# joyecnu/STTODE

Measured on AMD Instinct MI355X. Metric: predicted-trajectories/sec (20-sample best-of-K), higher is better.
Workload: dtype f32

## Files before the change

### include/sttode_hip.h

```cpp
#ifndef STTODE_HIP_H
#define STTODE_HIP_H
#ifdef __cplusplus
extern "C" {
#endif

#define STTODE_ABI_VERSION 15
int sttode_abi_version(void);
const char* sttode_last_error(void);

int sttode_rotate_scene(float* past, float* fut, int n, int Tp, int Tf, float c, float s, void* stream);

int sttode_frontend_scenes(const float* past, const int* scene_ptr, int n, int S, int Tp, int TPX, int vel_from_norm,
                           float* scene_orig, int* agent_scene, float* xpad, float* enc_in, float* cur, float* orig,
                           int* last_flag, void* stream);

int sttode_frontend_nba(const float* past, int n, int N, int Tp, int TPX, float* xpad, float* enc_in, float* cur, float* orig,
                        int* last_flag, void* stream);

int sttode_frontend_future(const float* future, const float* past_last, int n, int Tf, int mode, int nba_N,
                           const float* scene_orig, const int* agent_scene, const int* scene_ptr, float* enc_in, void* stream);

int sttode_embed_qkv(const float* fc1P, const float* fc1b, const float* posP, const float* peb, const float* fc2P,
                     const float* fc2b, const float* fc3P, const float* fc3b, const float* fc3last, const float* inP,
                     const float* inb, const float* enc_in, const int* last_flag, float* g, float* qkv, int n, int Tlen,
// ... 260 lines not shown
                             double* gc_ws, float* gc, void* stream);
int sttode_pmath_matvec_bwd_c(const float* m, const float* x, const float* g, float* mx_ws, float* gmx_ws, float* gxn_ws, float* gx, float* gm,
                              int rows, int d, int O, const float* c_dev, double* gc_ws, float* gc, void* stream);
int sttode_pmath_dist_matrix_bwd_c(const float* x, const float* y, const float* g, float* gx, float* gy, int P, int R, int d,
                                   const float* c_dev, double* gc_ws, float* gc, void* stream);
int sttode_pmath_hsoftmax_bwd_c(const float* X, const float* A, const float* P, const float* g, double* coef_ws, float* gX, float* gA,
                                float* gP, int B, int C, int d, const float* c_dev, double* gc_ws, float* gc, void* stream);
int sttode_oblique_dist(const float* p1, const float* p2, float* out, int nb, int n1, int n2, int d, void* stream);
int sttode_pmath_mean_seg(const float* x, float* yl_ws, float* lam_ws, float* out, float* klein, float* lsum, int outer, int R, int inner,
                          int d, float c, const float* c_dev, void* stream);
int sttode_pmath_mean_bwd(const float* x, const float* g, double* gS_ws, double* gL_ws, float* gx, int outer, int R, int inner, int d, float c,
                          void* stream);
int sttode_pmath_mean_bwd_c(const float* x, const float* g, double* gS_ws, double* gL_ws, float* gx, int outer, int R, int inner, int d,
                            const float* c_dev, double* gc_ws, float* gc, void* stream);
int sttode_oblique_proj_bwd(const float* p, const float* g, float* gp, int rows, int d, void* stream);
int sttode_oblique_dist_bwd(const float* p1, const float* p2, const float* g, float* gp1, float* gp2, int nb, int n1, int n2, int d,
                            void* stream);

enum SttodeManifold { STT_MF_EUCLIDEAN = 0, STT_MF_OBLIQUE, STT_MF_POINCARE, STT_MF_COUNT };
enum SttodeManifoldOp { STT_MOP_PROJ_TAN = 0, STT_MOP_EXPMAP, STT_MOP_PTRANSP, STT_MOP_INNER, STT_MOP_RETR, STT_MOP_RETR_TRANSP, STT_MOP_COUNT };
enum SttodeRiemannianRule { STT_RULE_ADAM = 0, STT_RULE_SGD, STT_RULE_COUNT };
int sttode_manifold_rowop(int op, int manifold, const float* a, const float* b, const float* w, float* out, float* out2, int rows, int d,
                          float c, void* stream);
int sttode_manifold_rowop_bwd(int op, int manifold, const float* a, const float* b, const float* w, const float* g, const float* g2, float* ga,
                              float* gb, float* gw, int rows, int d, float c, void* stream);
#define STTODE_RIEMANNIAN_ITEM_WORDS 10
int sttode_riemannian_step(int rule, const void* table, int nrows_table, long total_slots, double lr, double beta1, double beta2,
                           double eps, double weight_decay, double momentum, long t, void* tstate, void* stream);

int sttode_delta_dist(const float* X, int rows, int d, const int* idx, int T, int n, float* dist, long dist_floats, float* diam, void* stream);
int sttode_delta_workspace(int T, int n, long* floats);
int sttode_delta_hyp(const float* dist, int T, int n, long dist_floats, int symmetric, float* ws, long ws_floats, float* delta, void* stream);

int sttode_reduce_samples(const float* pred, int n, int R, int K_in, int Tf, int K, int iters, int from_frame, int init_mode,
                          const float* init, float* centroids, int* labels, int* counts, void* stream);

int sttode_reduce_scenes(const float* pred, int n, int R, int K_in, int Tf, int K, int iters, int from_frame, int init_mode,
                         const float* init, const int* seg_ptr, int S, float* centroids, int* labels, int* counts, void* stream);
long long int sttode_large_select_ws(int n, int M);
int sttode_large_select(const float* pred, const float* gt, int n, int R, int K_in, int Tf, float scale, float miss_threshold, const int* ks,
                        int nk, const int* seg_ptr, int S, void* ws, long ws_bytes, float* ade, float* fde, int* best_ade_idx,
                        int* best_fde_idx, unsigned char* miss, float* ade_at, float* fde_at, float* seg_jade, float* seg_jfde,
                        int* seg_jade_idx, int* seg_jfde_idx, void* stream);
int sttode_large_kde_nll(const float* pred, const float* gt, int n, int R, int K_in, int Tf, float scale, double* nll, void* stream);
long long int sttode_large_spread_ws(int n, int M);
int sttode_large_spread(const float* pred, const float* gt, int n, int R, int K_in, int Tf, float scale, double div_scale, void* ws,
                        long ws_bytes, double* apd, double* fpd, double* pade, double* dlow, double* es_ade, double* es_fde, void* stream);

typedef struct SttodeModel SttodeModel;

enum SttodeWeight {
    STT_W_FC1P, STT_W_FC1B, STT_W_POSP, STT_W_PEB, STT_W_FC2P, STT_W_FC2B, STT_W_FC3P, STT_W_FC3B, STT_W_FC3LAST, STT_W_INP,
    STT_W_INB, STT_W_OUTP, STT_W_OUTB, STT_W_INFOP, STT_W_INFOB, STT_W_GATEP, STT_W_GATEB, STT_W_LN1W, STT_W_LN1B, STT_W_L1P,
    STT_W_L1B, STT_W_L2P, STT_W_L2B, STT_W_LN2W, STT_W_LN2B,
    STT_W_B0_CONVP, STT_W_B0_CONVB, STT_W_B0_WIHP, STT_W_B0_WHHP, STT_W_B0_GBIAS, STT_W_B0_XWA, STT_W_B0_XB1, STT_W_B0_YWA,
    STT_W_B0_YB1, STT_W_B0_STREAM,
    STT_W_B1_CONVP, STT_W_B1_CONVB, STT_W_B1_WIHP, STT_W_B1_WHHP, STT_W_B1_GBIAS, STT_W_B1_YWA, STT_W_B1_YB1, STT_W_B1_STREAM,
    STT_W_CHAIN_POOL, STT_W_CHAIN_PROG, STT_W_CHAIN_CONSTS, STT_W_G0_POOL, STT_W_G0_PROG, STT_W_G0_CONSTS,
    STT_W_CHAINB3_POOL, STT_W_CHAINB3_PROG,
    STT_W_ROLE32_POOL, STT_W_ROLE32_PROG_SCENES, STT_W_ROLE32_PROG_NBA, STT_W_ROLE32_CONSTS_SCENES,
    STT_W_ROLE32_CONSTS_NBA,
    STT_W_COUNT
};

enum SttodeBuffer {
    STT_B_SCENE_ORIG, STT_B_AGENT_SCENE, STT_B_XPAD, STT_B_ENC_IN, STT_B_CUR, STT_B_ORIG, STT_B_LAST, STT_B_G, STT_B_QKV,
    STT_B_ATTN, STT_B_PF, STT_B_STATE0, STT_B_A0X, STT_B_A0Y, STT_B_A1Y, STT_B_DBUF, STT_B_YBUF, STT_B_STATE1, STT_B_QUEUE, STT_B_FLAGS ,
    STT_B_ODE , STT_B_COUNT
};

enum SttodeStage {
    STT_STAGE_FRONTEND, STT_STAGE_EMBED, STT_STAGE_ATTN, STT_STAGE_POST, STT_STAGE_GRU0, STT_STAGE_LINEAR, STT_STAGE_MLP0,
    STT_STAGE_GRU1, STT_STAGE_MLP1, STT_STAGE_CHAIN, STT_STAGE_AGENTS ,
    STT_STAGE_FUSED , STT_STAGE_COUNT
};

int sttode_model_create(SttodeModel** out, const void* const* weights, int count, int Tp, int Tf, int K, int n_chunks0,
                        int n_chunks1);
int sttode_model_set_weight(SttodeModel* m, int index, const void* ptr);
int sttode_model_destroy(SttodeModel* m);
int sttode_workspace_layout(const SttodeModel* m, int n, int S, long* offsets , long* total_floats);
int sttode_workspace_init(SttodeModel* m, float* workspace, int n, int S, void* stream);
int sttode_set_chain(SttodeModel* m, int mode);
int sttode_set_fused(SttodeModel* m, int mode);
int sttode_set_mfma_mode(SttodeModel* m, int mode);
int sttode_debug_drop_role_flag(SttodeModel* m, int tile);
int sttode_stage_scene(const float* pre, const float* fut, int N, int Tp, int Tf, float* dev, void* stream);
int sttode_stage_rows(const float* a, long na, const float* b, long nb, float* dev, void* stream);
int sttode_async_next_stream(SttodeModel* m, int n, void** stream);
int sttode_async_best_of_k(SttodeModel* m, int slot, const float* pred, const float* gt, int n, int K, int Tf, float scale, float* ade,
                           float* fde);
int sttode_set_scene_launch(SttodeModel* m, int max_tiles);
int sttode_set_ode(SttodeModel* m, int method, int steps);
int sttode_timing_enable(SttodeModel* m, int every);
int sttode_timing_read(SttodeModel* m, double* total_ms , int* launches ,
                       double* busy_ms );

int sttode_inference_scenes(SttodeModel* m, const float* past, const int* scene_ptr, int n, int S, const float* z,
                            float* workspace, float* pred, void* stream);
int sttode_inference_nba(SttodeModel* m, const float* past, int B, int N, const float* z, float* workspace, float* pred,
                         void* stream);
int sttode_inference_nba_groups(SttodeModel* m, const float* past, int G, int B, int N, const float* z, float* workspace, float* pred,
                                void* stream);

int sttode_set_lagged(SttodeModel* m, int streams );
typedef struct SttodeSamplerPlan {
    const float* pool;
    const int* prog;
    int prog_len;
    const float* biases;
    int K;
    int nz;
    int h1;
    int h2;
    int eps_mode;
    const float* eps;
} SttodeSamplerPlan;
typedef struct SttodeAsyncOpts {
    int device_latents;
    unsigned long long zkey;
    const float* metrics_gt;
    float* ade;
    float* fde;
    float metrics_scale;
    int nba_groups;
    const SttodeSamplerPlan* sampler;
} SttodeAsyncOpts;
int sttode_sampler_qnet(const SttodeSamplerPlan* plan, const float* pf, int n, float* z, void* stream);
int sttode_clock_probe(long long* out, void* stream);
int sttode_copy_to_host(void* dst, const void* src, long bytes, int wgs, void* stream);
int sttode_async_enqueue(SttodeModel* m, int slot);
int sttode_async_flush(SttodeModel* m);
int sttode_inference_scenes_async(SttodeModel* m, const float* past, const int* scene_ptr, int n, int S, const float* z,
                                  float* workspace, float* pred, int slot, const SttodeAsyncOpts* opts, void* stream);
int sttode_inference_nba_async(SttodeModel* m, const float* past, int B, int N, const float* z, float* workspace, float* pred,
                               int slot, const SttodeAsyncOpts* opts, void* stream);
int sttode_async_horizon_metrics(SttodeModel* m, int slot, const float* pred, const float* gt, int n, int K, int Tf, float scale, float* out);
int sttode_async_best_of_k_select(SttodeModel* m, int slot, const float* pred, const float* gt, int n, int K, int Tf, float scale,
                                  float miss_threshold, const int* seg_ptr, int S, float* ade, float* fde, int* best_ade_idx, int* best_fde_idx,
                                  unsigned char* miss, float* best, float* seg_ade, float* seg_fde, int* seg_miss);
int sttode_async_joint_select(SttodeModel* m, int slot, const float* pred, const float* gt, int n, int K, int Tf, float scale,
                              const int* seg_ptr, int S, float radius, float* seg_jade, float* seg_jfde, int* seg_jade_idx, int* seg_jfde_idx,
                              int* seg_col, int* seg_gt_col);
int sttode_async_kde_nll(SttodeModel* m, int slot, const float* pred, const float* gt, int n, int K, int Tf, float scale, double* nll);
int sttode_async_sample_spread(SttodeModel* m, int slot, const float* pred, const float* gt, int n, int K, int Tf, float scale,
                               double div_scale, double* apd, double* fpd, double* pade, double* dlow, double* es_ade, double* es_fde,
                               float* ade_at_k, float* fde_at_k);
int sttode_wait(SttodeModel* m, int slot, void* stream);
int sttode_async_is_lagged(SttodeModel* m, int n);
int sttode_wait_host(SttodeModel* m, int slot);
int sttode_timeout_word(SttodeModel* m, const unsigned** word);
int sttode_timeout_clear(SttodeModel* m);
int sttode_check(SttodeModel* m, const float* workspace, int n, int S, void* stream);

#ifdef __cplusplus
}
#endif
#endif
```

### sttode_amd/capi.py

```python
import ctypes
import os

_LIB = None
LIB_PATH = os.environ.get('STTODE_HIP_LIB') or os.path.join(os.path.dirname(os.path.abspath(__file__)), 'lib', 'libsttode_hip.so')

_P, _I, _L, _F, _D = ctypes.c_void_p, ctypes.c_int, ctypes.c_long, ctypes.c_float, ctypes.c_double
ABI_VERSION = 15

SIGNATURES = {
    'sttode_abi_version': [],
    'sttode_rotate_scene': [_P, _P, _I, _I, _I, _F, _F, _P],
    'sttode_frontend_scenes': [_P, _P, _I, _I, _I, _I, _I, _P, _P, _P, _P, _P, _P, _P, _P],
    'sttode_frontend_nba': [_P, _I, _I, _I, _I, _P, _P, _P, _P, _P, _P],
    'sttode_frontend_future': [_P, _P, _I, _I, _I, _I, _P, _P, _P, _P, _P],
    'sttode_embed_qkv': [_P] * 11 + [_P, _P, _P, _P, _I, _I, _P],
    'sttode_mhgsa_attn': [_P, _P, _P, _P, _P, _P, _I, _I, _I] + [_L] * 8 + [_F, _F, _P],
    'sttode_mhgsa_attn_groups': [_P, _P, _P, _P, _I, _L, _L, _L, _L, _I, _I, _I] + [_L] * 8 + [_F, _F, _I, _P],
    'sttode_post_attn': [_P] * 14 + [_P, _P, _I, _P, _I, _F, _P],
    'sttode_post_attn_ode': [_P] * 16 + [_P, _P, _I, _F, _I, _I, _P],
    'sttode_post_attn_rhs': [_P] * 14 + [_P, _P, _I, _P, _I, _P],
    'sttode_ode_state_to_pf': [_P, _P, _P, _I, _P],
    'sttode_gru_cols': [_P, _P, _P, _P, _P, _P, _P, _I, _I, _I, _P],
    'sttode_set_latency_tiles': [_I, _I, _I],
    'sttode_linear_cols': [_P, _I, _I, _P, _I, _I, _P, _P, _P, _I, _I, _I, _I, _P],
# ... 22 lines not shown
    'sttode_sampler_objective_joint': [_P] * 8 + [_I, _I, _I, _I, _I, _F, _P, _L] + [_P] * 6,
    'sttode_sampler_objective_joint_bwd': [_P] * 8 + [_I] + [_P] * 4 + [_I, _I, _I, _I, _F, _P, _L] + [_P] * 4,
    'sttode_tlinear': [_P, _L, _I, _P, _L, _I, _P, _P, _L, _P, _L, _I, _I, _I, _I, _I, _P],
    'sttode_tlinear_tab': [_P, _L, _P, _L, _P, _P, _L, _I, _P, _L, _I, _I, _I, _I, _P],
    'sttode_twgrad': [_P, _L, _P, _L, _I, _P, _L, _P, _I, _I, _I, _P, _L, _P],
    'sttode_twgrad_defer': [_I, _P, _L],
    'sttode_twgrad_flush': [],
    'sttode_tgemm_group': [_I],
    'sttode_tlinear_bwd': [_P, _L, _P, _L, _P, _L, _P, _L, _I, _I, _P, _L, _I, _P, _L, _P, _I, _I, _I, _P, _L, _P],
    'sttode_decoder_inputs': [_P, _P, _L, _P, _L, _P, _P, _I, _I, _I, _I, _P],
    'sttode_rows_copy': [_P, _L, _P, _L, _I, _I, _I, _I, _P],
    'sttode_rows_reduce': [_P, _L, _P, _L, _I, _I, _I, _I, _P],
    'sttode_train_ewise': [_I, _P, _P, _P, _P, _P, _L, _I, _F, _P],
    'sttode_add_ln_fwd': [_P, _P, _P, _P, _P, _P, _P, _I, _I, _P],
    'sttode_ln_bwd': [_P, _P, _P, _P, _P, _P, _P, _I, _I, _P, _L, _P],
    'sttode_gru_cell_fwd': [_P, _L, _P, _P, _P, _P, _I, _P],
    'sttode_gru_cell_bwd': [_P, _P, _P, _P, _L, _P, _P, _I, _P],
    'sttode_gru_seq_fwd': [_P, _P, _P, _P, _P, _P, _L, _I, _I, _P],
    'sttode_gru_seq_bwd': [_P, _L, _P, _P, _P, _P, _P, _I, _I, _P],
    'sttode_conv_fwd': [_P, _I, _P, _P, _P, _P, _P, _I, _I, _P],
    'sttode_conv_bwd': [_P, _P, _P, _P, _P, _P, _I, _I, _P, _L, _P],
    'sttode_mhgsa_attn_bwd': [_P, _P, _P, _I, _I, _I, _P],
    'sttode_mhgsa_attn_rc_bwd': [_P] * 7 + [_I, _I, _I] + [_L] * 8 + [_F, _F, _P],
    'sttode_adam_step': [_P, _I, _L, _P, _D, _D, _D, _D, _D, _L, _P],
    'sttode_grad_norm': [_P, _I, _P, _L, _D, _I, _P, _P],
    'sttode_adam_step_guarded': [_P, _I, _L, _P, _D, _D, _D, _D, _P, _I, _P],
    'sttode_grad_scale': [_P, _I, _L, _P, _P, _P],
    'sttode_loss_sqerr': [_P, _P, _L, _F, _P, _P, _P],
    'sttode_loss_kl': [_P, _P, _I, _I, _I, _F, _F, _P, _P, _P, _P],
    'sttode_loss_diverse': [_P, _P, _P, _P, _I, _I, _I, _P, _P, _P, _P],
    'sttode_ttrunk_fwd': [_P, _I, _I, _I, _L, _F, _I, _P],
    'sttode_ode_combine': [_P, _I, _I, _P],
    'sttode_ttrunk_ode_fwd': [_P, _I, _I, _P, _P, _P, _P, _P, _P, _P],
    'sttode_ode_stage_bwd': [_P, _I, _P],
    'sttode_loss_objective': [_P, _P, _P, _P, _P, _P, _P, _I, _I, _I, _I, _I, _I, _F, _F, _F, _F, _P, _P, _P, _P, _P, _L, _P],
    'sttode_pmath_rowop': [_I, _P, _P, _P, _P, _I, _I, _F, _P],
    'sttode_pmath_scalar': [_I, _P, _P, _L, _P],
    'sttode_pmath_riemannian_grad': [_P, _P, _P, _I, _I, _F, _P],
    'sttode_pmath_matvec': [_P, _P, _P, _P, _P, _I, _I, _I, _F, _P],
    'sttode_pmath_pair': [_I, _P, _P, _P, _P, _I, _I, _I, _F, _P],
    'sttode_pmath_mean': [_P, _P, _P, _P, _I, _I, _F, _P],
    'sttode_oblique_dist': [_P, _P, _P, _I, _I, _I, _I, _P],
    'sttode_pmath_rowop_bwd': [_I, _P, _P, _P, _P, _P, _I, _I, _F, _P],
    'sttode_pmath_matvec_bwd': [_P, _P, _P, _P, _P, _P, _P, _P, _I, _I, _I, _F, _P],
    'sttode_pmath_dist_matrix_bwd': [_P, _P, _P, _P, _P, _I, _I, _I, _F, _P],
    'sttode_pmath_hsoftmax_bwd': [_P, _P, _P, _P, _P, _P, _P, _P, _I, _I, _I, _F, _P],
    'sttode_pmath_clip': [_P, _P, _I, _I, _F, _P],
    'sttode_pmath_clip_bwd': [_P, _P, _P, _I, _I, _F, _P],
    'sttode_pmath_rowop_c': [_I, _P, _P, _P, _P, _I, _I, _P, _P],
    'sttode_pmath_matvec_c': [_P, _P, _P, _P, _P, _I, _I, _I, _P, _P],
    'sttode_pmath_pair_c': [_I, _P, _P, _P, _P, _I, _I, _I, _P, _P],
    'sttode_pmath_rowop_bwd_c': [_I, _P, _P, _P, _P, _P, _I, _I, _P, _P, _P, _P],
    'sttode_pmath_matvec_bwd_c': [_P, _P, _P, _P, _P, _P, _P, _P, _I, _I, _I, _P, _P, _P, _P],
    'sttode_pmath_dist_matrix_bwd_c': [_P, _P, _P, _P, _P, _I, _I, _I, _P, _P, _P, _P],
    'sttode_pmath_hsoftmax_bwd_c': [_P, _P, _P, _P, _P, _P, _P, _P, _I, _I, _I, _P, _P, _P, _P],
    'sttode_manifold_rowop': [_I, _I, _P, _P, _P, _P, _P, _I, _I, _F, _P],
    'sttode_riemannian_step': [_I, _P, _I, _L, _D, _D, _D, _D, _D, _D, _L, _P, _P],
    'sttode_pmath_mean_seg': [_P, _P, _P, _P, _P, _P, _I, _I, _I, _I, _F, _P, _P],
    'sttode_pmath_mean_bwd': [_P, _P, _P, _P, _P, _I, _I, _I, _I, _F, _P],
    'sttode_pmath_mean_bwd_c': [_P, _P, _P, _P, _P, _I, _I, _I, _I, _P, _P, _P, _P],
    'sttode_oblique_proj_bwd': [_P, _P, _P, _I, _I, _P],
    'sttode_oblique_dist_bwd': [_P, _P, _P, _P, _P, _I, _I, _I, _I, _P],
    'sttode_manifold_rowop_bwd': [_I, _I, _P, _P, _P, _P, _P, _P, _P, _P, _I, _I, _F, _P],
    'sttode_delta_dist': [_P, _I, _I, _P, _I, _I, _P, _L, _P, _P],
    'sttode_delta_workspace': [_I, _I, ctypes.POINTER(ctypes.c_long)],
    'sttode_delta_hyp': [_P, _I, _I, _L, _I, _P, _L, _P, _P],
    'sttode_reduce_samples': [_P, _I, _I, _I, _I, _I, _I, _I, _I, _P, _P, _P, _P, _P],
    'sttode_reduce_scenes': [_P, _I, _I, _I, _I, _I, _I, _I, _I, _P, _P, _I, _P, _P, _P, _P],
    'sttode_large_select_ws': [_I, _I],
    'sttode_large_select': [_P, _P, _I, _I, _I, _I, _F, _F, _P, _I, _P, _I, _P, _L] + [_P] * 12,
    'sttode_large_kde_nll': [_P, _P, _I, _I, _I, _I, _F, _P, _P],
    'sttode_large_spread_ws': [_I, _I],
    'sttode_large_spread': [_P, _P, _I, _I, _I, _I, _F, _D, _P, _L] + [_P] * 7,
    'sttode_attn_core': [_P, _P, _P, _P, _L, _P, _P, _P, _P, _I, _I, _I] + [_L] * 8 + [_F, _F, _I, _P],
    'sttode_attn_core_bwd': [_P, _P, _P, _P, _L, _P, _P, _P, _P, _I, _I, _I] + [_L] * 8 + [_F, _F, _I, _P],
    'sttode_model_create': [ctypes.POINTER(ctypes.c_void_p), ctypes.POINTER(ctypes.c_void_p), _I, _I, _I, _I, _I, _I],
    'sttode_model_destroy': [_P],
    'sttode_model_set_weight': [_P, _I, _P],
    'sttode_workspace_layout': [_P, _I, _I, ctypes.POINTER(ctypes.c_long), ctypes.POINTER(ctypes.c_long)],
    'sttode_workspace_init': [_P, _P, _I, _I, _P],
    'sttode_timeout_word': [_P, ctypes.POINTER(ctypes.c_void_p)],
    'sttode_timeout_clear': [_P],
    'sttode_set_chain': [_P, _I],
    'sttode_set_fused': [_P, _I],
    'sttode_set_mfma_mode': [_P, _I],
    'sttode_debug_drop_role_flag': [_P, _I],
    'sttode_set_scene_launch': [_P, _I],
    'sttode_stage_scene': [_P, _P, _I, _I, _I, _P, _P],
    'sttode_stage_rows': [_P, _L, _P, _L, _P, _P],
    'sttode_loss_objective_live': [_P, _P, _P, _P, _P, _P, _P, _I, _I, _I, _I, _I, _I, _F, _F, _F, _F, _P, _P, _P, _P, _P, _P, _L, _P],
    'sttode_loss_objective_joint': [_P, _P, _P, _P, _P, _P, _P, _I, _I, _I, _I, _I, _I, _F, _F, _F, _F, _P, _P, _P, _P, _P, _I, _P, _P, _L, _P],
    'sttode_loss_diverse_joint': [_P, _P, _P, _P, _I, _I, _I, _I, _P, _P, _P, _P, _P],
    'sttode_live_rows_gather': [_P, _I, _P, _I, _I, _P],
    'sttode_publish_values': [_P, _I, _P, _P, _P, _P],
    'sttode_wait_value': [_P, _L, _D],
    'sttode_async_next_stream': [_P, _I, _P],
    'sttode_async_best_of_k': [_P, _I, _P, _P, _I, _I, _I, _F, _P, _P],
    'sttode_set_ode': [_P, _I, _I],
    'sttode_timing_enable': [_P, _I],
    'sttode_timing_read': [_P, ctypes.POINTER(ctypes.c_double), ctypes.POINTER(ctypes.c_int), ctypes.POINTER(ctypes.c_double)],
    'sttode_inference_scenes': [_P, _P, _P, _I, _I, _P, _P, _P, _P],
    'sttode_inference_nba': [_P, _P, _I, _I, _P, _P, _P, _P],
    'sttode_inference_nba_groups': [_P, _P, _I, _I, _I, _P, _P, _P, _P],
    'sttode_inference_scenes_async': [_P, _P, _P, _I, _I, _P, _P, _P, _I, _P, _P],
    'sttode_inference_nba_async': [_P, _P, _I, _I, _P, _P, _P, _I, _P, _P],
    'sttode_async_horizon_metrics': [_P, _I, _P, _P, _I, _I, _I, _F, _P],
    'sttode_async_best_of_k_select': [_P, _I, _P, _P, _I, _I, _I, _F, _F, _P, _I] + [_P] * 9,
    'sttode_async_joint_select': [_P, _I, _P, _P, _I, _I, _I, _F, _P, _I, _F] + [_P] * 6,
    'sttode_async_kde_nll': [_P, _I, _P, _P, _I, _I, _I, _F, _P],
    'sttode_async_sample_spread': [_P, _I, _P, _P, _I, _I, _I, _F, _D] + [_P] * 8,
    'sttode_wait': [_P, _I, _P],
    'sttode_async_is_lagged': [_P, _I],
    'sttode_wait_host': [_P, _I],
    'sttode_set_lagged': [_P, _I],
    'sttode_async_flush': [_P],
    'sttode_clock_probe': [_P, _P],
    'sttode_copy_to_host': [_P, _P, _L, _I, _P],
    'sttode_async_enqueue': [_P, _I],
    'sttode_check': [_P, _P, _I, _I, _P],
}

RESTYPES = {'sttode_sampler_objective_joint_ws': ctypes.c_longlong, 'sttode_large_select_ws': ctypes.c_longlong,
            'sttode_large_spread_ws': ctypes.c_longlong}

WEIGHT_ORDER = ([('past', k) for k in ('fc1P', 'fc1b', 'posP', 'peb', 'fc2P', 'fc2b', 'fc3P', 'fc3b', 'fc3last', 'inP', 'inb', 'outP',
                                       'outb', 'infoP', 'infob', 'gateP', 'gateb', 'ln1w', 'ln1b', 'l1P', 'l1b', 'l2P', 'l2b', 'ln2w',
                                       'ln2b')]
                + [('blk0', k) for k in ('convP', 'convB', 'wihP', 'whhP', 'gbias', 'x_WA', 'x_b1', 'y_WA', 'y_b1', 'stream')]
                + [('blk1', k) for k in ('convP', 'convB', 'wihP', 'whhP', 'gbias', 'y_WA', 'y_b1', 'stream')]
                + [('chain', k) for k in ('pool', 'prog', 'consts')] + [('gru0s', k) for k in ('pool', 'prog', 'consts')]
                + [('chain_b3', k) for k in ('pool', 'prog')]
                + [('role32', k) for k in ('pool', 'prog_scenes', 'prog_nba', 'consts_scenes', 'consts_nba')])
TRUNK_PTRS = ('fc1_w', 'fc1_b', 'pos_w', 'pos_b', 'fc2_w', 'fc2_b', 'fc3_w', 'fc3_b', 'inproj_w', 'inproj_b', 'out_w', 'out_b', 'info_w', 'info_b',
              'gate_w', 'gate_b', 'ln1_w', 'ln1_b', 'l1_w', 'l1_b', 'l2_w', 'l2_b', 'ln2_w', 'ln2_b', 'enc_in', 'last', 'pe', 'drop', 'posin', 'tp',
              'h3in', 'feat', 'xc', 'qkv', 'ao', 'tt', 'ss', 'h', 'xh1', 'rs1', 'f1', 'xh2', 'rs2', 'ode', 'attn')
BUFFERS = ('scene_orig', 'agent_scene', 'xpad', 'enc_in', 'cur', 'orig', 'last', 'g', 'qkv', 'attn', 'pf', 'state0', 'A0x', 'A0y',
           'A1y', 'dbuf', 'ybuf', 'state1', 'queue', 'flags', 'ode')
STAGES = ('frontend', 'embed_qkv', 'mhgsa_attn', 'post_attn', 'gru_cols[block0,agents]', 'agent_preact', 'mlp_block0',
          'gru_cols[block1,trajectories]', 'mlp_block1', 'trajectory_chain', 'agents_fused[encoder+block0 GRU]', 'agents+trajectory_chain[fused launch]')


class AsyncOpts(ctypes.Structure):
    _fields_ = [('device_latents', ctypes.c_int), ('zkey', ctypes.c_ulonglong), ('metrics_gt', ctypes.c_void_p), ('ade', ctypes.c_void_p),
                ('fde', ctypes.c_void_p), ('metrics_scale', ctypes.c_float), ('nba_groups', ctypes.c_int), ('sampler', ctypes.c_void_p)]


class GradGroup(ctypes.Structure):
    _fields_ = [('items', ctypes.c_void_p), ('n', ctypes.c_int), ('chunks', ctypes.c_long), ('gbase', ctypes.c_void_p),
                ('lr', ctypes.c_double), ('beta1', ctypes.c_double), ('beta2', ctypes.c_double), ('step', ctypes.c_long)]


GRAD_MAX_GROUPS = 16
GRAD_STATE_WORDS = 40


MANIFOLDS = dict(euclidean=0, oblique=1, poincare=2)
MANIFOLD_OPS = dict(proj_tan=0, expmap=1, ptransp=2, inner=3, retr=4, retr_transp=5)
RIEMANNIAN_RULES = dict(adam=0, sgd=1)
RIEMANNIAN_ITEM_WORDS = 10


class SamplerPlan(ctypes.Structure):
    _fields_ = [('pool', ctypes.c_void_p), ('prog', ctypes.c_void_p), ('prog_len', ctypes.c_int), ('biases', ctypes.c_void_p),
                ('K', ctypes.c_int), ('nz', ctypes.c_int), ('h1', ctypes.c_int), ('h2', ctypes.c_int), ('eps_mode', ctypes.c_int),
                ('eps', ctypes.c_void_p)]


class NativeModel:

    def __init__(self, packed, Tp, Tf, K):
        self.packed = packed
        tbl = (ctypes.c_void_p * len(WEIGHT_ORDER))(*[(packed[g][k].data_ptr() if g in packed else None) for g, k in WEIGHT_ORDER])
        h = ctypes.c_void_p()
        rc = lib().sttode_model_create(ctypes.byref(h), tbl, len(WEIGHT_ORDER), Tp, Tf, K, int(packed['blk0']['n_chunks']),
                                       int(packed['blk1']['n_chunks']))
        if rc != 0:
            raise SttodeError('sttode_model_create failed: ' + lib().sttode_last_error().decode())
        self.h = h
        self._layouts = {}
        w = ctypes.c_void_p()
        if lib().sttode_timeout_word(h, ctypes.byref(w)) != 0 or not w.value:
            raise SttodeError('sttode_timeout_word failed: ' + lib().sttode_last_error().decode())
        self.timeout_word = ctypes.c_uint.from_address(w.value)

    def raise_if_timed_out(self):
        v = self.timeout_word.value
        if v:
            lib().sttode_timeout_clear(self.h)
            raise SttodeError('a trajectory group of an earlier launch gave up waiting for its per-agent role (time-out word %d): the '
                              'predictions of that call are NaN-poisoned, not valid' % v if v != 2 else
                              'an earlier launch ran on a workspace that was never initialised (sttode_workspace_init): its predictions are NaN')

    def init_workspace(self, buf, n, S):
        call('sttode_workspace_init', self.h, buf, int(n), int(S), stream_ptr())

    def layout(self, n, S):
        key = (n, S)
        if key not in self._layouts:
            off = (ctypes.c_long * len(BUFFERS))()
            tot = ctypes.c_long()
            rc = lib().sttode_workspace_layout(self.h, n, S, off, ctypes.byref(tot))
            if rc != 0:
                raise SttodeError('sttode_workspace_layout failed: ' + lib().sttode_last_error().decode())
            self._layouts[key] = (dict(zip(BUFFERS, list(off))), int(tot.value))
        return self._layouts[key]

    def set_chain(self, mode):
        if lib().sttode_set_chain(self.h, int(mode)) != 0:
            raise SttodeError('sttode_set_chain failed: ' + lib().sttode_last_error().decode())

    def set_scene_launch(self, max_tiles):
        call('sttode_set_scene_launch', self.h, int(max_tiles))

    def set_fused(self, mode):
        if lib().sttode_set_fused(self.h, int(mode)) != 0:
            raise SttodeError('sttode_set_fused failed: ' + lib().sttode_last_error().decode())

    def set_lagged(self, streams):
        call('sttode_set_lagged', self.h, int(streams))
        self._lagged = int(streams)

    def check(self, workspace, n, S):
        call('sttode_check', self.h, workspace, int(n), int(S), stream_ptr())

    def set_weights(self, group, tensors):
        self.packed[group] = tensors
        for i, (g, k) in enumerate(WEIGHT_ORDER):
            if g == group:
                call('sttode_model_set_weight', self.h, i, tensors[k])

    def set_mfma_mode(self, mode):
        if lib().sttode_set_mfma_mode(self.h, int(mode)) != 0:
            raise SttodeError('sttode_set_mfma_mode failed: ' + lib().sttode_last_error().decode())

    def set_ode(self, method, steps):
        if lib().sttode_set_ode(self.h, int(method), int(steps)) != 0:
            raise SttodeError('sttode_set_ode failed: ' + lib().sttode_last_error().decode())

    def timing(self, every):
        lib().sttode_timing_enable(self.h, int(every))

    def read_timing(self):
        ms = (ctypes.c_double * len(STAGES))()
        cnt = (ctypes.c_int * len(STAGES))()
        busy = (ctypes.c_double * len(STAGES))()
        rc = lib().sttode_timing_read(self.h, ms, cnt, busy)
        if rc != 0:
            raise SttodeError('sttode_timing_read failed: ' + lib().sttode_last_error().decode())
        self.busy_ms = {STAGES[i]: busy[i] for i in range(len(STAGES)) if cnt[i]}
        return {STAGES[i]: (ms[i], cnt[i]) for i in range(len(STAGES)) if cnt[i]}

    def __del__(self):
        try:
            if self.h:
                lib().sttode_model_destroy(self.h)
                self.h = None
        except Exception:
            pass



class SttodeError(RuntimeError):
    pass


def lib():
    global _LIB
    if _LIB is None:
        if not os.path.exists(LIB_PATH):
            raise SttodeError(f'{LIB_PATH} not found: build it with `python -c "import __graft_entry__ as g; g.build()"` '
                              f'or `make -C sttode_amd/csrc`. There is no CPU fallback.')
        L = ctypes.CDLL(LIB_PATH)
        L.sttode_last_error.restype = ctypes.c_char_p
        L.sttode_last_error.argtypes = []
        try:
            got = int(L.sttode_abi_version())
        except AttributeError:
            got = None
        if got != ABI_VERSION:
            raise SttodeError(f'{LIB_PATH}: ABI version {got}, this binding needs {ABI_VERSION}; rebuild with `make -C sttode_amd/csrc`')
        for name, args in SIGNATURES.items():
            fn = getattr(L, name)
            fn.argtypes = args
            fn.restype = RESTYPES.get(name, ctypes.c_int)
        _LIB = L
    return _LIB


def _ptr(t):
    if t is None:
        return None
    return t.data_ptr() if hasattr(t, 'data_ptr') else int(t)


TIMING = None


def call(name, *args, tag=None):
    L = lib()
    conv = [(_ptr(a) if (a is None or hasattr(a, 'data_ptr')) else a) for a in args]
    if TIMING is not None:
        import torch
        e0, e1 = torch.cuda.Event(enable_timing=True), torch.cuda.Event(enable_timing=True)
        e0.record()
        rc = getattr(L, name)(*conv)
        e1.record()
        TIMING.append((tag or name, e0, e1))
    else:
        rc = getattr(L, name)(*conv)
    if rc != 0:
        raise SttodeError(f'{name} failed (status {rc}): {L.sttode_last_error().decode()}')


def sampler_joint_ws(n, K, S):
    L = lib()
    b = int(L.sttode_sampler_objective_joint_ws(int(n), int(K), int(S)))
    if b < 0:
        raise SttodeError(f'sttode_sampler_objective_joint_ws failed: {L.sttode_last_error().decode()}')
    return b


def large_set_ws(entry, n, M):
    L = lib()
    b = int(getattr(L, entry + '_ws')(int(n), int(M)))
    if b < 0:
        raise SttodeError(f'{entry}_ws failed: {L.sttode_last_error().decode()}')
    return b


def stream_ptr():
    import torch
    try:
        return torch._C._cuda_getCurrentRawStream(torch._C._cuda_getDevice())
    except AttributeError:
        return torch.cuda.current_stream().cuda_stream
```

### sttode_amd/csrc/api_util.hpp

```cpp
#pragma once
#include <hip/hip_runtime.h>
#include <cstdio>

void stt_set_error(const char* msg);
int stt_refuse(const char* who, const char* why);
int stt_gru_cols_form(const float* xin, const float* convP, const float* convB, const float* wihP, const float* whhP, const float* gbias,
                      float* state, int ncols, int Tp, int TPX, int lat_max_tiles, void* stream);
int stt_agents_fused(const float* const* W, const float* enc_in, const int* last, float* g, float* qkv, float* pf, const float* xpad,
                     float* state0, int n, int Tp, int TPX, float ode_time, void* stream);
bool stt_agents_fused_covers(int Tp, int TPX);
int stt_chain_fused(const float* const* W, float* ws, const long* off, int n, int K, int Tp, int Tf, int prog_len, const float* z, float* pred,
                    float ode_time, const float* attn, int ld_attn, int wgs_per_cu, int b3, int drop_tile,
                    unsigned* tmo_host, void* stream);
bool stt_chain_fused_covers(int Tp);
int stt_scene_lat(const float* const* W, float* ws, const long* off, int n, int K, int Tp, int Tf, int TPX, int NOY, int n_chunks0, int n_chunks1,
                  const float* z, float* pred, float ode_time, const float* past, const int* scene_ptr, int S, int drop_tile, unsigned* tmo_host,
                  void* stream);
static inline int stt_scene_flags_offset(int n) { return 5 * ((n + 15) / 16) + 4; }
int stt_scene_flags_init(float* ws, const long* off, int n, int K, void* stream);
bool stt_scene_lat_covers(int Tp, int TPX, int NOY);
int stt_traj_chain_b3(const float* A0x, const float* A0y, const float* A1y, const float* pool, const int* prog, int prog_len,
                      const float* consts, const float* z, const float* xpad, int ldx, const float* cur, const float* orig,
                      float* pred, int* counter, int ncols, int K, int Tp, int Tf, int wgs_per_cu, void* stream);
int stt_gru_lat_tiles();
int stt_enc_lat_tiles();

#define STT_REQUIRE(cond, msg)      \
    do {                            \
        if (!(cond)) {              \
            stt_set_error(msg);     \
            return 1;               \
        }                           \
    } while (0)

#define STT_HIP(expr)                                                                       \
    do {                                                                                    \
        hipError_t _e = (expr);                                                             \
        if (_e != hipSuccess) {                                                             \
            char _b[512];                                                                   \
            snprintf(_b, sizeof(_b), "%s failed: %s (%s:%d)", #expr, hipGetErrorString(_e), __FILE__, __LINE__); \
            stt_set_error(_b);                                                              \
            return 2;                                                                       \
        }                                                                                   \
    } while (0)

#define STT_ATTR_DEVICES 64
#define STT_SET_LDS_ONCE(kernel, bytes)                                                                         \
    do {                                                                                                        \
        static bool _done[STT_ATTR_DEVICES] = {};                                                               \
        int _dev = 0;                                                                                           \
        STT_HIP(hipGetDevice(&_dev));                                                                           \
        if (_dev < 0 || _dev >= STT_ATTR_DEVICES || !_done[_dev]) {                                             \
            STT_HIP(hipFuncSetAttribute((const void*)(kernel), hipFuncAttributeMaxDynamicSharedMemorySize, (bytes))); \
            if (_dev >= 0 && _dev < STT_ATTR_DEVICES) _done[_dev] = true;                                       \
        }                                                                                                       \
    } while (0)

struct LagRoles {
    float* ws; const long* off; int n;
    const float* attn; int ld_attn; float ode_time;
    float* zgen; unsigned long long zkey;
    const float* past; const int* scene_ptr; int S;
    float* ade; float* fde;
};
struct LagGroups {
    float* ws; const long* off; int n; const float* z; float* pred;
    const float* gt; float* ade; float* fde; float scale;
    int workers;
};
int stt_chain_lagged(const float* const* W, const LagRoles& r, const LagGroups& g, int K, int Tp, int Tf, int prog_len, int b3, void* stream);
bool stt_chain_lagged_covers(int Tp);
struct SttodeSamplerPlan;
const char* stt_sampler_plan_check(const SttodeSamplerPlan* plan, int K);
int stt_sampler_qnet(const SttodeSamplerPlan* plan, const float* pf, int n, float* z, void* stream);
int stt_joint_check(const char* who, const float* pred, const float* gt, int n, int K, int Tf, const int* seg_ptr, int S, float radius,
                    const float* seg_jade, const float* seg_jfde, const int* seg_jade_idx, const int* seg_jfde_idx, const int* seg_col,
                    const int* seg_gt_col);
int stt_kde_check(const char* who, const float* pred, const float* gt, int n, int K, int Tf, const double* nll);
int stt_spread_check(const char* who, const float* pred, const float* gt, int n, int K, int Tf, double div_scale, const double* apd,
                     const double* fpd, const double* pade, const double* dlow, const double* es_ade, const double* es_fde,
                     const float* ade_at_k, const float* fde_at_k);
```

### sttode_amd/csrc/chain32.hip

```cpp
#include "chain.hpp"
#include "latency_bodies.hpp"
#include "frontend_body.hpp"
#include "api_util.hpp"
#include "../../include/sttode_hip.h"
#include <cstdlib>
#include <cstddef>

#ifdef C32_DIAG_TRACE
__shared__ long long g_tr_ph[4];
#define C32_TRACE_BEGIN() long long _tr_t0 = 0, _tr_c0 = 0; if (threadIdx.x == 0 && A.dbg) { _tr_t0 = __builtin_amdgcn_s_memrealtime(); _tr_c0 = __builtin_amdgcn_s_memtime(); }
#define C32_TRACE_END(kind) do { if (threadIdx.x == 0 && A.dbg) { \
        const long long _t1 = __builtin_amdgcn_s_memrealtime(); unsigned _hw, _xcc; \
        asm volatile("s_getreg_b32 %0, hwreg(HW_REG_HW_ID)" : "=s"(_hw)); asm volatile("s_getreg_b32 %0, hwreg(HW_REG_XCC_ID)" : "=s"(_xcc)); \
        const unsigned long long _r = atomicAdd((unsigned long long*)A.dbg, 1ull); if ((long long)_r >= A.dbg[1]) break;  \
        long long* _p = A.dbg + 8 + _r * 12; _p[0] = A.trace_tag; _p[1] = blockIdx.x; _p[2] = (kind); _p[3] = _tr_t0; _p[4] = _t1; _p[5] = _hw; _p[6] = _xcc; \
        _p[8] = g_tr_ph[0]; _p[9] = g_tr_ph[1]; _p[10] = g_tr_ph[2]; _p[7] = __builtin_amdgcn_s_memtime() - _tr_c0; _p[11] = g_tr_ph[3]; } } while (0)
#define C32_TRACE_PHASE(i) do { if (threadIdx.x == 0) g_tr_ph[i] = __builtin_amdgcn_s_memrealtime(); } while (0)
#else
#define C32_TRACE_PHASE(i) do { } while (0)
#define C32_TRACE_BEGIN() do { } while (0)
#define C32_TRACE_END(kind) do { } while (0)
#endif

#include "role_body.hpp"

typedef float f32x16 __attribute__((ext_vector_type(16)));

#ifdef C32_DIAG_NOGATES
#define C32_SIG(x) ((x) * 1e-3f)
#define C32_TANH(x) ((x) * 1e-3f)
#else
#define C32_SIG(x) sigmoid_prescaled(x)
#define C32_TANH(x) tanh_prescaled(x)
#endif

#define C32_TILE 256
#define C32_CMAX 3
#define C32_RING (2 * C32_CMAX * C32_TILE)
#define C32_SLOT 256

struct Role32Args {
    const f32x4* pool; const int2* prog; int prog_len; const float* consts;
    const float* enc_in; const int* last;
    const float* g_in; const float* attn; int ld_attn;
    const float* xpad; int ldx;
    float* pf; float* state0; float* A0x; float* A0y; float* A1y;
    int n, Tp, kte, nwg;
    float ode_time;
    int prio;
    int* counter;
    float* zgen; unsigned zkey0, zkey1; int K;
    const float* past; const int* scene_ptr; int S; float* scene_orig; int* agent_scene;
    float* enc_in_w; float* xpad_w; float* cur_w; float* orig_w; int* last_w;
    float* m_ade; float* m_fde;
};

struct ChainArgs {
    const float* A0x; const float* A0y; const float* A1y;
    const f32x4* pool;
    const int2* prog; int prog_len;
    const float* consts;
    const float* z;
    const float* xpad; int ldx;
    const float* cur; const float* orig;
    float* pred;
    float* park;
    int* counter;
    int ncols, K, Tp, Tf2;
    int persistent;
    const float* m_gt; float* m_ade; float* m_fde; float m_scale;
    int nworkers;
    long long* dbg;
    int trace_tag;
    int xcd_map;
    RoleArgs R;
    Role32Args R32;
};

template <int NY> struct C32Const {
    static constexpr int b2x = 0, b3x = 256, b2y = 288, b3y = 544, gb = 544 + 32 * NY, cb = gb + 384, b2m = cb + 32,
                         b3m = b2m + 256, total = b3m + 32 * NY;
};

__device__ __forceinline__ f32x16 splat16(float v) {
    f32x16 r;
#pragma unroll
    for (int e = 0; e < 16; ++e) r[e] = v;
    return r;
}
__device__ __forceinline__ f32x16 relu16(f32x16 v) {
#pragma unroll
    for (int e = 0; e < 16; ++e) v[e] = fmaxf(v[e], 0.f);
    return v;
}
__device__ __forceinline__ f32x16 ldrows(const float* p, int h) {
    f32x16 r;
#pragma unroll
    for (int a = 0; a < 4; ++a) {
        const f32x4 v = ld4(p + 8 * a + 4 * h);
        r[4 * a + 0] = v[0]; r[4 * a + 1] = v[1]; r[4 * a + 2] = v[2]; r[4 * a + 3] = v[3];
    }
    return r;
}

typedef const __attribute__((address_space(4))) int KProg;

template <int BUF, bool GEN, bool DYN = false>
struct ChainStreamT {
    static constexpr int kBuf = BUF;
    static constexpr int kPieces = (BUF / 64 + 3) / 4, kPairs = (kPieces + 1) / 2;
    const char* pool; KProg* prog; f32x4* ring;
    unsigned ring_addr, loff;
    unsigned qoff, qend;
    int par, lane, wave;
    int2 ld_v, ld_w;
    bool fetched;
    int cnt;
    const char* nsrc[kPairs]; unsigned nm0[kPairs]; int ncnt, npc;
#ifdef C32_DIAG_STAMPS
    long long t_bar, gap_cyc, gap_n, gap_cal;
#endif
    __device__ __forceinline__ int2 entry_at(unsigned off) const {
        const KProg* e = reinterpret_cast<const KProg*>(reinterpret_cast<const __attribute__((address_space(4))) char*>(prog) + off);
        return make_int2(e[0], e[1]);
    }
    __device__ __forceinline__ unsigned next_off(unsigned off) const { return off + 8 >= qend ? 0u : off + 8; }
    __device__ __forceinline__ void stage(int2 ev, int buf) {
        ncnt = __builtin_amdgcn_readfirstlane(ev.y);
        npc = GEN ? (ncnt - wave + 3) >> 2 : ncnt;
        const size_t src = (size_t)(unsigned)__builtin_amdgcn_readfirstlane(ev.x) * (GEN ? 16u : C32_TILE * 16u) + (unsigned)wave * 1024u;
        const unsigned dst = __builtin_amdgcn_readfirstlane(ring_addr + (unsigned)buf * (BUF * 16) + (unsigned)wave * 1024u);
#pragma unroll
        for (int k = 0; k < kPairs; ++k) {
            nsrc[k] = pool + (src + 4096u * (2 * k + 1));
            nm0[k] = dst + 4096u * (2 * k + 1);
            asm volatile("" : "+s"(nsrc[k]), "+s"(nm0[k]));
        }
        asm volatile("" : "+s"(npc));
    }
    __device__ __forceinline__ void issue(int N) {
#ifndef C32_DIAG_NODMA
#pragma unroll
        for (int k = 0; k < kPairs; ++k) {
            if (N > 0 ? 2 * k < N : 2 * k < npc) {
                glds16_sv<-4096>(nsrc[k], loff, nm0[k] - 4096u);
                if (2 * k + 1 < kPieces && (N > 0 ? 2 * k + 1 < N : 2 * k + 1 < npc)) glds16_m0<0>(nsrc[k], loff);
            }
        }
#endif
    }
    __device__ __forceinline__ void init(const f32x4* pool_, const int2* prog_, int len_, f32x4* ring_) {
        pool = reinterpret_cast<const char*>(pool_); prog = (KProg*)prog_; ring = ring_;
        ring_addr = __builtin_amdgcn_readfirstlane(lds_addr(ring_));
        lane = threadIdx.x & 63;
        loff = (unsigned)lane * 16;
        wave = __builtin_amdgcn_readfirstlane(threadIdx.x >> 6);
        par = 0;
        qend = (unsigned)len_ * 8u;
        const int2 e0 = entry_at(0);
        stage(e0, 0);
        issue(0);
        cnt = e0.y;
        qoff = next_off(0);
        stage(entry_at(qoff), 1);
        qoff = next_off(qoff);
        fetched = false;
#ifdef C32_DIAG_STAMPS
        gap_cyc = 0; gap_n = 0;
        const long long c0 = __builtin_amdgcn_s_memtime();
        asm volatile("s_waitcnt lgkmcnt(0)" ::: "memory");
        gap_cal = __builtin_amdgcn_s_memtime() - c0;
        t_bar = 0;
#endif
    }
    __device__ __forceinline__ void fetch() { ld_v = entry_at(qoff); qoff = next_off(qoff); fetched = true; }
// ... 11 lines not shown
        __builtin_amdgcn_sched_barrier(0);
#ifdef C32_DIAG_CHECK
        if (!GEN && N > 0 && ncnt != N) __builtin_trap();
#endif
        cnt = ncnt;
        issue(GEN || DYN ? 0 : N);
        stamp_gap();
        __builtin_amdgcn_sched_barrier(0);
    }
    __device__ __forceinline__ const f32x4* cur() const { return ring + par * BUF + lane; }
    __device__ __forceinline__ void end(bool has_entry = false) {
        __builtin_amdgcn_sched_barrier(0);
#ifdef C32_DIAG_CHECK
        if (has_entry && !fetched) __builtin_trap();
#endif
        if (!has_entry && !fetched) fetch();
        stage(ld_v, par);
        __builtin_amdgcn_sched_barrier(0);
#ifndef C32_DIAG_NOBARRIER
        asm volatile("s_waitcnt vmcnt(0)" ::: "memory");
        __syncthreads();
#endif
#ifdef C32_DIAG_STAMPS
        t_bar = __builtin_amdgcn_s_memtime();
        asm volatile("s_waitcnt lgkmcnt(0)" ::: "memory");
#endif
        par ^= 1;
        fetched = false;
        __builtin_amdgcn_sched_barrier(0);
    }
};
typedef ChainStreamT<C32_CMAX * C32_TILE, false> ChainStream;

__device__ __forceinline__ void tile_mma(f32x16& acc, const f32x4* __restrict__ t, const f32x16& B) {
#pragma unroll
    for (int g = 0; g < 4; ++g) {
        const f32x4 a = t[g * 64];
#pragma unroll
        for (int r = 0; r < 4; ++r) acc = __builtin_amdgcn_mfma_f32_32x32x2f32(a[r], B[4 * g + r], acc, 0, 0, 0);
    }
}

__device__ __forceinline__ void gather_rows(const void* base, unsigned voff, unsigned slot_addr) {
    glds16_sv<0>(base, voff, slot_addr);
    glds16_sv<32>(base, voff, slot_addr + 1024);
    glds16_sv<64>(base, voff, slot_addr + 2048);
    glds16_sv<96>(base, voff, slot_addr + 3072);
}
__device__ __forceinline__ unsigned row_off(int row, int width, int h) { return (unsigned)row * (unsigned)(width * 4) + (unsigned)h * 16; }

struct Frag { f32x4 a[4]; };
__device__ __forceinline__ void ldfrag(Frag& f, const f32x4* __restrict__ t) {
#pragma unroll
    for (int g = 0; g < 4; ++g) f.a[g] = t[g * 64];
}
__device__ __forceinline__ void tile_mma2(f32x16& acc, const Frag& cur, const f32x16& B, Frag& nxt, const f32x4* __restrict__ tn) {
#pragma unroll
    for (int g = 0; g < 4; ++g) {
        if (g == 2 && tn) {
            ldfrag(nxt, tn);
            __builtin_amdgcn_sched_barrier(0);
        }
#pragma unroll
        for (int r = 0; r < 4; ++r) acc = __builtin_amdgcn_mfma_f32_32x32x2f32(cur.a[g][r], B[4 * g + r], acc, 0, 0, 0);
    }
}

template <class ST>
__device__ __forceinline__ void tile_mma2f(ST& st, f32x16& acc, const Frag& cur, const f32x16& B, Frag& nxt, const f32x4* __restrict__ tn, int nf = 1) {
#pragma unroll
    for (int g = 0; g < 4; ++g) {
        if (g == 2) {
            __builtin_amdgcn_sched_barrier(0);
            if (nf >= 1) st.fetch();
            if (nf >= 2) st.fetch_more();
            if (tn) ldfrag(nxt, tn);
            __builtin_amdgcn_sched_barrier(0);
        }
#pragma unroll
        for (int r = 0; r < 4; ++r) acc = __builtin_amdgcn_mfma_f32_32x32x2f32(cur.a[g][r], B[4 * g + r], acc, 0, 0, 0);
    }
}

template <int KH, class ST>
__device__ __forceinline__ void mlp_l12(ST& st, const f32x4* slot, const f32x4* zslot, const f32x16* Bh, const float* tab, unsigned aoff,
                                        const float* tab_next, unsigned aoff_next, f32x16 (&acc2)[8], int lane) {
    const unsigned slot_addr = __builtin_amdgcn_readfirstlane(lds_addr(slot));
    constexpr int KT1 = 1 + KH;
    static_assert((KT1 + 8) % 3 == 0, "hidden tile must be a whole number of chunks");
#pragma unroll
    for (int R = 0; R < 8; ++R) acc2[R] = splat16(0.f);
#pragma unroll 1
    for (int ht = 0; ht < 16; ++ht) {
        f32x16 h1, zb;
#pragma unroll
        for (int a = 0; a < 4; ++a) {
            const f32x4 v = slot[a * 64 + lane];
            h1[4 * a + 0] = v[0]; h1[4 * a + 1] = v[1]; h1[4 * a + 2] = v[2]; h1[4 * a + 3] = v[3];
        }
#pragma unroll
        for (int a = 0; a < 4; ++a) {
            const f32x4 v = zslot[a * 64 + lane];
            zb[4 * a + 0] = v[0]; zb[4 * a + 1] = v[1]; zb[4 * a + 2] = v[2]; zb[4 * a + 3] = v[3];
        }
        asm volatile("s_waitcnt lgkmcnt(0)" ::: "memory");
        __builtin_amdgcn_sched_barrier(0);
        const bool nl = ht + 1 < 16;
        const void* nb = nl ? (const void*)(reinterpret_cast<const char*>(tab) + 128 * (ht + 1)) : (const void*)tab_next;
        const unsigned no = nl ? aoff : aoff_next;
        Frag fr[2];
#pragma unroll
        for (int i = 0; i < KT1 + 8; ++i) {
            if (i % 3 == 0) {
                if (i > 0) st.end();
                ldfrag(fr[i & 1], st.cur());
                st.begin(3);
                if (i == 0) {
#ifndef C32_DIAG_NOGATHER
                    gather_rows(nb, no, slot_addr);
#endif
                    __builtin_amdgcn_sched_barrier(0);
                }
            }
            const f32x4* tn = (i % 3 < 2) ? st.cur() + (i % 3 + 1) * C32_TILE : nullptr;
            if (i == 0) {
                tile_mma2f(st, h1, fr[i & 1], zb, fr[(i + 1) & 1], tn);
            } else if (i < KT1) {
                if (i % 3 == 0) tile_mma2f(st, h1, fr[i & 1], Bh[i - 1], fr[(i + 1) & 1], tn);
                else tile_mma2(h1, fr[i & 1], Bh[i - 1], fr[(i + 1) & 1], tn);
            } else {
                if (i == KT1) h1 = relu16(h1);
                if (i % 3 == 0) tile_mma2f(st, acc2[i - KT1], fr[i & 1], h1, fr[(i + 1) & 1], tn);
                else tile_mma2(acc2[i - KT1], fr[i & 1], h1, fr[(i + 1) & 1], tn);
            }
        }
        st.end();
    }
}

template <int NO, int NEXT = 0, class ST>
__device__ __forceinline__ void mlp_l3(ST& st, f32x16 (&acc2)[8], const float* __restrict__ b2, const float* __restrict__ b3,
                                       f32x16 (&out)[NO], int h) {
#pragma unroll
    for (int R = 0; R < 8; ++R) {
        STT_FENCE();
        const f32x16 b = ldrows(b2 + 32 * R, h);
        acc2[R] = relu16(acc2[R] + b);
        asm volatile("" : "+v"(acc2[R]));
    }
    STT_FENCE();
#pragma unroll
    for (int o = 0; o < NO; ++o) out[o] = ldrows(b3 + 32 * o, h);
    Frag fr[2];
#pragma unroll
    for (int i = 0; i < 8 * NO; ++i) {
        if (i % 3 == 0) {
            if (i > 0) st.end();
            ldfrag(fr[i & 1], st.cur());
            const int left = 8 * NO - (i + 3);
            st.begin(left >= 3 ? 3 : left > 0 ? left : NEXT);
        }
        const f32x4* tn = (i % 3 < 2 && i + 1 < 8 * NO) ? st.cur() + (i % 3 + 1) * C32_TILE : nullptr;
        if (i % 3 == 0) tile_mma2f(st, out[i / 8], fr[i & 1], acc2[i % 8], fr[(i + 1) & 1], tn);
        else tile_mma2(out[i / 8], fr[i & 1], acc2[i % 8], fr[(i + 1) & 1], tn);
    }
    st.end();
}

typedef __bf16 bf16x8 __attribute__((ext_vector_type(8)));
typedef __bf16 bf16x2 __attribute__((ext_vector_type(2)));
typedef float f32x2v __attribute__((ext_vector_type(2)));
typedef unsigned u32x4v __attribute__((ext_vector_type(4)));
#define C32_TILE_B3 384
#define C32_BUF_B3 (C32_CMAX * C32_TILE_B3)
struct B3 { bf16x8 p[3][2]; };
__device__ __forceinline__ float bf_lo(unsigned u) { return __uint_as_float(u << 16); }
__device__ __forceinline__ float bf_hi(unsigned u) { return __uint_as_float(u & 0xffff0000u); }
__device__ __forceinline__ void split3(const f32x16& x, B3& o) {
#pragma unroll
    for (int kb = 0; kb < 2; ++kb) {
        unsigned hi[4], mi[4], lo[4];
#pragma unroll
        for (int q = 0; q < 4; ++q) {
            const float x0 = x[8 * kb + 2 * q], x1 = x[8 * kb + 2 * q + 1];
            const f32x2v v = {x0, x1};
            hi[q] = __builtin_bit_cast(unsigned, __builtin_convertvector(v, bf16x2));
            const float r0 = x0 - bf_lo(hi[q]), r1 = x1 - bf_hi(hi[q]);
            const f32x2v rv = {r0, r1};
            mi[q] = __builtin_bit_cast(unsigned, __builtin_convertvector(rv, bf16x2));
            const f32x2v qv = {r0 - bf_lo(mi[q]), r1 - bf_hi(mi[q])};
            lo[q] = __builtin_bit_cast(unsigned, __builtin_convertvector(qv, bf16x2));
        }
        const u32x4v H = {hi[0], hi[1], hi[2], hi[3]}, M = {mi[0], mi[1], mi[2], mi[3]}, L = {lo[0], lo[1], lo[2], lo[3]};
        o.p[0][kb] = __builtin_bit_cast(bf16x8, H);
        o.p[1][kb] = __builtin_bit_cast(bf16x8, M);
        o.p[2][kb] = __builtin_bit_cast(bf16x8, L);
    }
}
struct Frag6 { f32x4 a[6]; };
__device__ __forceinline__ void ldfrag6(Frag6& f, const f32x4* __restrict__ t) {
#pragma unroll
    for (int i = 0; i < 6; ++i) f.a[i] = t[i * 64];
}
__device__ __forceinline__ void tile_mma_b3(f32x16& acc, const Frag6& cur, const B3& B, Frag6& nxt, const f32x4* __restrict__ tn) {
#pragma unroll
    for (int kb = 0; kb < 2; ++kb) {
        if (kb == 1 && tn) {
            ldfrag6(nxt, tn);
            __builtin_amdgcn_sched_barrier(0);
        }
        const bf16x8 ah = __builtin_bit_cast(bf16x8, cur.a[kb * 3 + 0]), am = __builtin_bit_cast(bf16x8, cur.a[kb * 3 + 1]),
                     al = __builtin_bit_cast(bf16x8, cur.a[kb * 3 + 2]);
        acc = __builtin_amdgcn_mfma_f32_32x32x16_bf16(al, B.p[0][kb], acc, 0, 0, 0);
        acc = __builtin_amdgcn_mfma_f32_32x32x16_bf16(ah, B.p[2][kb], acc, 0, 0, 0);
        acc = __builtin_amdgcn_mfma_f32_32x32x16_bf16(am, B.p[1][kb], acc, 0, 0, 0);
        acc = __builtin_amdgcn_mfma_f32_32x32x16_bf16(am, B.p[0][kb], acc, 0, 0, 0);
        acc = __builtin_amdgcn_mfma_f32_32x32x16_bf16(ah, B.p[1][kb], acc, 0, 0, 0);
        acc = __builtin_amdgcn_mfma_f32_32x32x16_bf16(ah, B.p[0][kb], acc, 0, 0, 0);
    }
}
__device__ __forceinline__ void tile_mma_b3n(f32x16& acc, const f32x4* __restrict__ t, const B3& B) {
    Frag6 f, dummy;
    ldfrag6(f, t);
    tile_mma_b3(acc, f, B, dummy, nullptr);
}
template <int KH, bool PRE, class ST>
__device__ __forceinline__ void mlp_l12_b3(ST& st, const f32x4* slot, const f32x4* zslot, const f32x16* Bh, const float* tab, unsigned aoff,
                                           const float* tab_next, unsigned aoff_next, f32x16 (&acc2)[8], int lane) {
    const unsigned slot_addr = __builtin_amdgcn_readfirstlane(lds_addr(slot));
    constexpr int KT1 = 1 + KH;
// ... 94 lines not shown

__device__ __forceinline__ f32x16 b3_to_f32(const B3& b) {
    f32x16 r;
#pragma unroll
    for (int kb = 0; kb < 2; ++kb) {
        const u32x4v H = __builtin_bit_cast(u32x4v, b.p[0][kb]), M = __builtin_bit_cast(u32x4v, b.p[1][kb]), L = __builtin_bit_cast(u32x4v, b.p[2][kb]);
#pragma unroll
        for (int q = 0; q < 4; ++q) {
            r[8 * kb + 2 * q] = (bf_lo(H[q]) + bf_lo(M[q])) + bf_lo(L[q]);
            r[8 * kb + 2 * q + 1] = (bf_hi(H[q]) + bf_hi(M[q])) + bf_hi(L[q]);
        }
    }
    return r;
}
template <class ST>
__device__ __forceinline__ void gru32_steps_b3(ST& st, const float* gb, const float* cb, const f32x16& d, f32x16 (&hs)[3], int Tp, int h) {
    B3 dB, hB[3];
    split3(d, dB);
#pragma unroll
    for (int j = 0; j < 3; ++j) split3(hs[j], hB[j]);
    constexpr int T = C32_TILE_B3;
#pragma unroll 1
    for (int t = 0; t < Tp; ++t) {
        B3 eB;
        {
            f32x16 e = ldrows(cb, h);
            st.begin();
            tile_mma_b3n(e, st.cur(), dB);
            e = relu16(e);
            st.end();
            split3(e, eB);
        }
        f32x16 hn[3];
#pragma unroll
        for (int j = 0; j < 3; ++j) {
            STT_FENCE();
            f32x16 ar = ldrows(gb + 0 * 96 + 32 * j, h);
            st.begin();
            tile_mma_b3n(ar, st.cur(), eB);
            tile_mma_b3n(ar, st.cur() + T, hB[0]);
            tile_mma_b3n(ar, st.cur() + 2 * T, hB[1]);
            st.end(); st.begin();
            tile_mma_b3n(ar, st.cur(), hB[2]);
#pragma unroll
            for (int r = 0; r < 16; ++r) ar[r] = C32_SIG(ar[r]);
            STT_FENCE();
            f32x16 az = ldrows(gb + 1 * 96 + 32 * j, h);
            tile_mma_b3n(az, st.cur() + T, eB);
            tile_mma_b3n(az, st.cur() + 2 * T, hB[0]);
            st.end(); st.begin();
            tile_mma_b3n(az, st.cur(), hB[1]);
            tile_mma_b3n(az, st.cur() + T, hB[2]);
#pragma unroll
            for (int r = 0; r < 16; ++r) az[r] = C32_SIG(az[r]);
            STT_FENCE();
            f32x16 an = ldrows(gb + 3 * 96 + 32 * j, h);
            tile_mma_b3n(an, st.cur() + 2 * T, hB[0]);
            st.end(); st.begin();
            tile_mma_b3n(an, st.cur(), hB[1]);
            tile_mma_b3n(an, st.cur() + T, hB[2]);
            {
                const f32x16 bi = ldrows(gb + 2 * 96 + 32 * j, h);
#pragma unroll
                for (int r = 0; r < 16; ++r) an[r] = fmaf(ar[r], an[r], bi[r]);
            }
            STT_FENCE();
            tile_mma_b3n(an, st.cur() + 2 * T, eB);
            st.end();
            const f32x16 hp = b3_to_f32(hB[j]);
#pragma unroll
            for (int r = 0; r < 16; ++r) {
                const float ng = C32_TANH(an[r]);
                hn[j][r] = fmaf(az[r], hp[r] - ng, ng);
            }
        }
#pragma unroll
        for (int j = 0; j < 3; ++j) {
            hs[j] = hn[j];
            split3(hn[j], hB[j]);
        }
    }
}

template <bool ZS, class ST>
__device__ __forceinline__ f32x16 gru32_conv(ST& st, const float* cb, const f32x16& d, int t, int Tp, int h, bool pre) {
    f32x16 e = ldrows(cb, h);
    Frag fa, fb;
    if (ZS) {
        const int k0 = 2 * t - 2, k1 = 2 * t + 3;
        const int g0 = (k0 > 0 ? k0 : 0) >> 3, g1 = (k1 < 2 * Tp - 1 ? k1 : 2 * Tp - 1) >> 3;
        const f32x4* tc = st.cur();
#pragma unroll
        for (int g = 0; g < 4; ++g)
            if (g >= g0 && g <= g1) fa.a[g] = tc[g * 64];
        st.begin(3);
#pragma unroll
        for (int g = 0; g < 4; ++g)
            if (g >= g0 && g <= g1)
#pragma unroll
                for (int r = 0; r < 4; ++r) e = __builtin_amdgcn_mfma_f32_32x32x2f32(fa.a[g][r], d[4 * g + r], e, 0, 0, 0);
        __builtin_amdgcn_sched_barrier(0);
        if (pre) st.take_prefetched();
        else st.fetch();
    } else {
        ldfrag(fa, st.cur());
        st.begin(3);
        tile_mma2f(st, e, fa, d, fb, nullptr, pre ? 0 : 1);
        if (pre) st.take_prefetched();
    }
    e = relu16(e);
    st.end();
    return e;
}

template <bool ZS, class ST>
__device__ __forceinline__ void gru32_steps(ST& st, const float* gb, const float* cb, const f32x16& d, f32x16 (&hs)[3], int Tp, int h) {
    if (ZS) {
        const f32x16 e = gru32_conv<ZS>(st, cb, d, 0, Tp, h, false);
        Frag fa, fb;
#pragma unroll
        for (int j = 0; j < 3; ++j) {
            STT_FENCE();
            f32x16 ar = ldrows(gb + 0 * 96 + 32 * j, h);
            ldfrag(fa, st.cur()); st.begin(3);
            tile_mma2f(st, ar, fa, e, fb, nullptr);
            st.end(); ldfrag(fa, st.cur() + 1 * C32_TILE); st.begin(3);
#pragma unroll
            for (int r = 0; r < 16; ++r) ar[r] = C32_SIG(ar[r]);
            STT_FENCE();
            f32x16 az = ldrows(gb + 1 * 96 + 32 * j, h);
            tile_mma2f(st, az, fa, e, fb, nullptr, 2);
            st.end(); st.begin(3);
            st.take_prefetched();
#pragma unroll
            for (int r = 0; r < 16; ++r) az[r] = C32_SIG(az[r]);
            STT_FENCE();
            f32x16 an = ldrows(gb + 3 * 96 + 32 * j, h);
            {
                const f32x16 bi = ldrows(gb + 2 * 96 + 32 * j, h);
#pragma unroll
                for (int r = 0; r < 16; ++r) an[r] = fmaf(ar[r], an[r], bi[r]);
            }
            st.end(); ldfrag(fa, st.cur() + 2 * C32_TILE);
            if (j < 2) st.begin(3); else st.begin();
            STT_FENCE();
            tile_mma2f(st, an, fa, e, fb, nullptr, (j == 2 && 1 < Tp) ? 2 : 1);
            st.end();
#pragma unroll
            for (int r = 0; r < 16; ++r) {
                const float ng = C32_TANH(an[r]);
                hs[j][r] = fmaf(az[r], 0.f - ng, ng);
            }
        }
    }
#pragma unroll 1
    for (int t = ZS ? 1 : 0; t < Tp; ++t) {
        const f32x16 e = gru32_conv<ZS>(st, cb, d, t, Tp, h, ZS);
        Frag fa, fb;
        f32x16 hn[3];
#pragma unroll
        for (int j = 0; j < 3; ++j) {
            STT_FENCE();
            f32x16 ar = ldrows(gb + 0 * 96 + 32 * j, h);
            ldfrag(fa, st.cur()); st.begin(3);
            tile_mma2f(st, ar, fa, e, fb, st.cur() + 1 * C32_TILE);
            tile_mma2(ar, fb, hs[0], fa, st.cur() + 2 * C32_TILE);
            tile_mma2(ar, fa, hs[1], fb, nullptr);
            st.end(); ldfrag(fa, st.cur()); st.begin(3);
            tile_mma2f(st, ar, fa, hs[2], fb, st.cur() + 1 * C32_TILE);
#pragma unroll
            for (int r = 0; r < 16; ++r) ar[r] = C32_SIG(ar[r]);
            STT_FENCE();
            f32x16 az = ldrows(gb + 1 * 96 + 32 * j, h);
            tile_mma2(az, fb, e, fa, st.cur() + 2 * C32_TILE);
            tile_mma2(az, fa, hs[0], fb, nullptr);
            st.end(); ldfrag(fa, st.cur()); st.begin(3);
            tile_mma2f(st, az, fa, hs[1], fb, st.cur() + 1 * C32_TILE);
            tile_mma2(az, fb, hs[2], fa, st.cur() + 2 * C32_TILE);
#pragma unroll
            for (int r = 0; r < 16; ++r) az[r] = C32_SIG(az[r]);
            STT_FENCE();
            f32x16 an = ldrows(gb + 3 * 96 + 32 * j, h);
            tile_mma2(an, fa, hs[0], fb, nullptr);
            st.end(); ldfrag(fa, st.cur());
            if (j < 2) st.begin(3); else st.begin();
            tile_mma2f(st, an, fa, hs[1], fb, st.cur() + 1 * C32_TILE, (ZS && j == 2 && t + 1 < Tp) ? 2 : 1);
            tile_mma2(an, fb, hs[2], fa, st.cur() + 2 * C32_TILE);
            {
                const f32x16 bi = ldrows(gb + 2 * 96 + 32 * j, h);
#pragma unroll
                for (int r = 0; r < 16; ++r) an[r] = fmaf(ar[r], an[r], bi[r]);
            }
            STT_FENCE();
            tile_mma2(an, fa, e, fb, nullptr);
            st.end();
#pragma unroll
            for (int r = 0; r < 16; ++r) {
                const float ng = C32_TANH(an[r]);
                hn[j][r] = fmaf(az[r], hs[j][r] - ng, ng);
            }
        }
#pragma unroll
        for (int j = 0; j < 3; ++j) hs[j] = hn[j];
    }

}

#include "role32.hpp"

__device__ __forceinline__ int opaque(int v) { asm volatile("" : "+v"(v)); return v; }

#ifdef C32_DIAG_STAMPS
#define C32_STAMP(k) do { if (threadIdx.x == 0 && A.dbg && gi < 4) { A.dbg[((size_t)blockIdx.x * 4 + gi) * 16 + 2 * (k)] = __builtin_amdgcn_s_memtime(); \
                                                                    A.dbg[((size_t)blockIdx.x * 4 + gi) * 16 + 2 * (k) + 1] = __builtin_amdgcn_s_memrealtime(); } } while (0)
#else
#define C32_STAMP(k) do { } while (0)
#endif


__host__ __device__ __forceinline__ int xcd_group(int b, int G) {
    const int x = b & 7, i = b >> 3, q = G >> 3, r = G & 7;
    return x * q + (x < r ? x : r) + i;
}

template <int NY, int FUSE, bool B3M, bool ZS>
__global__ __launch_bounds__(256, 2) void traj_chain_kernel(ChainArgs A) {
    constexpr bool kDynCount = !B3M && ((NY == 1 && FUSE == 2 && !ZS) || (NY == 2 && FUSE == 1 && ZS));
    typedef ChainStreamT<B3M ? C32_BUF_B3 : C32_CMAX * C32_TILE, B3M, kDynCount> Stream;
    extern __shared__ __attribute__((aligned(16))) char smem[];
    f32x4* ring = reinterpret_cast<f32x4*>(smem);
    f32x4* slots = ring + 2 * Stream::kBuf;
    f32x4* zslots = slots + 4 * C32_SLOT;
    float* cst = reinterpret_cast<float*>(zslots + 4 * C32_SLOT);
    int* sq = reinterpret_cast<int*>(cst + C32Const<NY>::total);
    typedef C32Const<NY> CO;

    const int lane = threadIdx.x & 63, c = lane & 31, h = lane >> 5;
    const int wave = __builtin_amdgcn_readfirstlane(threadIdx.x >> 6);
    const f32x4* slot = slots + wave * C32_SLOT;
    const f32x4* zslot = zslots + wave * C32_SLOT;
    const unsigned slot_addr = __builtin_amdgcn_readfirstlane(lds_addr(slot));
    const unsigned zslot_addr = __builtin_amdgcn_readfirstlane(lds_addr(zslot));
    const int ngroups = (A.ncols + 127) >> 7;

    C32_TRACE_BEGIN();
    if (FUSE == 2 && (int)blockIdx.x < A.R32.nwg) {
        role32_body<ZS>(*(KRole32Args*)((const __attribute__((address_space(4))) char*)__builtin_amdgcn_kernarg_segment_ptr() + offsetof(ChainArgs, R32)),
                    blockIdx.x, smem);
        C32_TRACE_END(1);
        return;
    }
    int fb = FUSE == 0 ? (int)blockIdx.x : (int)blockIdx.x - (FUSE == 2 ? A.R32.nwg : A.R.ntiles);
    if (FUSE && A.xcd_map && fb >= 0) fb = xcd_group(fb, ngroups);
    if (FUSE == 1 && fb < 0) {
        agent_role(A.R, (A.ncols + A.K - 1) / A.K, A.Tp, A.ldx, A.xpad, A.R.ntiles + fb, smem);
        C32_TRACE_END(1);
        return;
    }
    for (int i = threadIdx.x; i < CO::total; i += blockDim.x) cst[i] = A.consts[i];
    if (threadIdx.x == 0) sq[0] = FUSE == 2 ? fb : (FUSE == 0 && A.persistent) ? atomicAdd(A.counter, 1) : FUSE ? fb : (int)blockIdx.x;
    if (FUSE == 1) {
        const int g0 = fb;
        const int c_lo = g0 * 128, c_hi = (c_lo + 127 < A.ncols ? c_lo + 127 : A.ncols - 1);
        const int t_lo = (c_lo / A.K) >> 4, t_hi = (c_hi / A.K) >> 4;
        if (wave == 0) {
            const bool ok = wait_tiles(A.R.flags, t_lo, t_hi, A.R.flags + A.R.ntiles, lane, A.R.tmo_host);
            if (!ok && lane == 0) sq[0] = -1;
        }
    }
    __syncthreads();
    C32_TRACE_PHASE(3);
    int g = sq[0];
    if (FUSE == 1 && g < 0) {
        for (int i = threadIdx.x; i < 128 * A.Tf2; i += blockDim.x) {
            const size_t o = (size_t)fb * 128 * A.Tf2 + i;
            if (o < (size_t)A.ncols * A.Tf2) A.pred[o] = __builtin_nanf("");
        }
        return;
    }
    if (g >= ngroups) return;
    Stream st;
    st.init(A.pool, A.prog, A.prog_len, ring);

    auto col_of = [&](int gg) { int col = gg * 128 + wave * 32 + c; return col < A.ncols ? col : A.ncols - 1; };
    {
        const int c0 = col_of(g);
        gather_rows(A.A0x, row_off(c0 / A.K, 512, h), slot_addr);
        gather_rows(A.z, row_off(c0, 32, h), zslot_addr);
    }
    asm volatile("s_waitcnt vmcnt(0)" ::: "memory");
    __syncthreads();

    int gi = 0;
    (void)gi;
    while (true) {
        C32_STAMP(0);
        const int col = g * 128 + wave * 32 + c;
        int colc = col < A.ncols ? col : A.ncols - 1;
        int agent = colc / A.K;
        const bool live = col < A.ncols;
        __syncthreads();
        if (threadIdx.x == 0)
            sq[1] = (FUSE == 2 && A.persistent && ngroups > A.nworkers) ? A.nworkers + atomicAdd(A.counter, 1)
                    : (FUSE == 0 && A.persistent) ? atomicAdd(A.counter, 1) : ngroups;

        f32x16 acc2[8];
        f32x16 d;
        {
            agent = opaque(agent);
            f32x16 xo[1];
            const unsigned ao = row_off(agent, 512, h);
            if (B3M) {
                mlp_l12_b3<0, true>(st, slot, zslot, nullptr, A.A0x, ao, A.A0y, ao, acc2, lane);
                mlp_l3_b3<1>(st, acc2, cst + CO::b2x, cst + CO::b3x, xo, h);
            } else {
                mlp_l12<0>(st, slot, zslot, nullptr, A.A0x, ao, A.A0y, ao, acc2, lane);
                mlp_l3<1, 3>(st, acc2, cst + CO::b2x, cst + CO::b3x, xo, h);
            }
            agent = opaque(agent);
            const float* xp = A.xpad + (size_t)agent * A.ldx;
#pragma unroll
            for (int a = 0; a < 4; ++a) {
                f32x4 v = splat4(0.f);
                if (8 * a + 4 * h < A.ldx) v = ld4(xp + 8 * a + 4 * h);
#pragma unroll
                for (int b = 0; b < 4; ++b) d[4 * a + b] = v[b] - xo[0][4 * a + b];
            }
        }
        STT_FENCE();
        C32_STAMP(1);
        {
            agent = opaque(agent);
            f32x16 yo[NY];
            const unsigned ao = row_off(agent, 512, h);
            if (B3M) {
                mlp_l12_b3<0, true>(st, slot, zslot, nullptr, A.A0y, ao, A.A1y, ao, acc2, lane);
                mlp_l3_b3<NY>(st, acc2, cst + CO::b2y, cst + CO::b3y, yo, h);
            } else {
                mlp_l12<0>(st, slot, zslot, nullptr, A.A0y, ao, A.A1y, ao, acc2, lane);
                mlp_l3<NY, 1>(st, acc2, cst + CO::b2y, cst + CO::b3y, yo, h);
            }
            if (live) {
                float* prow = A.park + (size_t)opaque(col) * A.Tf2;
#pragma unroll
                for (int o = 0; o < NY; ++o)
#pragma unroll
                    for (int a = 0; a < 4; ++a) {
                        const int row0 = 32 * o + 8 * a + 4 * h;
                        float* p = prow + row0;
                        if (row0 + 3 < A.Tf2 && (A.Tf2 & 3) == 0) {
                            f32x4 v = {yo[o][4 * a], yo[o][4 * a + 1], yo[o][4 * a + 2], yo[o][4 * a + 3]};
                            st4(p, v);
                        } else {
#pragma unroll
                            for (int b = 0; b < 4; ++b)
                                if (row0 + b < A.Tf2) p[b] = yo[o][4 * a + b];
                        }
                    }
            }
        }
        STT_FENCE();
        C32_STAMP(2);
        f32x16 hs[3];
        {
#pragma unroll
            for (int j = 0; j < 3; ++j) hs[j] = splat16(0.f);
            if (B3M) gru32_steps_b3(st, cst + CO::gb, cst + CO::cb, d, hs, A.Tp, h);
            else gru32_steps<ZS>(st, cst + CO::gb, cst + CO::cb, d, hs, A.Tp, h);
        }
        STT_FENCE();
        C32_STAMP(3);
        const int gnext = sq[1];
        {
            agent = opaque(agent);
            const int cnx = col_of(gnext < ngroups ? gnext : g);
            const unsigned ao = row_off(agent, 512, h), an = row_off(cnx / A.K, 512, h);
            if (B3M) mlp_l12_b3<3, false>(st, slot, zslot, hs, A.A1y, ao, A.A0x, an, acc2, lane);
            else mlp_l12<3>(st, slot, zslot, hs, A.A1y, ao, A.A0x, an, acc2, lane);
            gather_rows(A.z, row_off(opaque(cnx), 32, h), zslot_addr);
            f32x16 yo[NY];
            if (B3M) mlp_l3_b3<NY>(st, acc2, cst + CO::b2m, cst + CO::b3m, yo, h);
            else mlp_l3<NY, 3>(st, acc2, cst + CO::b2m, cst + CO::b3m, yo, h);
            {
                agent = opaque(agent);
                const float cx = A.cur[2 * agent], cy = A.cur[2 * agent + 1];
                const float ox = A.orig[2 * agent], oy = A.orig[2 * agent + 1];
                const bool vec = (A.Tf2 & 3) == 0;
                const float* yrow = A.park + (size_t)opaque(colc) * A.Tf2;
                float* prow = A.pred + (size_t)opaque(col) * A.Tf2;
                const float* grow = FUSE == 2 && A.m_gt ? A.m_gt + (size_t)agent * A.Tf2 : nullptr;
                float dd[NY][4][2];
#pragma unroll
                for (int o = 0; o < NY; ++o)
#pragma unroll
                    for (int a = 0; a < 4; ++a) {
                        const int row0 = 32 * o + 8 * a + 4 * h;
                        const bool whole = vec && row0 + 3 < A.Tf2;
                        f32x4 y0 = splat4(0.f);
                        if (whole) y0 = ld4(yrow + row0);
                        else {
#pragma unroll
                            for (int b = 0; b < 4; ++b)
                                if (row0 + b < A.Tf2) y0[b] = yrow[row0 + b];
                        }
                        f32x4 v;
                        v[0] = ((y0[0] + yo[o][4 * a + 0]) + cx) + ox;
                        v[1] = ((y0[1] + yo[o][4 * a + 1]) + cy) + oy;
                        v[2] = ((y0[2] + yo[o][4 * a + 2]) + cx) + ox;
                        v[3] = ((y0[3] + yo[o][4 * a + 3]) + cy) + oy;
                        if (live) {
                            if (whole) st4(prow + row0, v);
                            else {
#pragma unroll
                                for (int b = 0; b < 4; ++b)
                                    if (row0 + b < A.Tf2) prow[row0 + b] = v[b];
                            }
                        }
                        dd[o][a][0] = dd[o][a][1] = 0.f;
                        if (FUSE == 2 && grow) {
                            if (row0 < A.Tf2) { const float2 g = *reinterpret_cast<const float2*>(grow + row0); dd[o][a][0] = bok_dist(v[0], v[1], g.x, g.y, A.m_scale); }
                            if (row0 + 2 < A.Tf2) { const float2 g = *reinterpret_cast<const float2*>(grow + row0 + 2); dd[o][a][1] = bok_dist(v[2], v[3], g.x, g.y, A.m_scale); }
                        }
                    }
                if (FUSE == 2 && grow) {
                    const int Tf = A.Tf2 >> 1;
                    float acc = 0.f, fdl = -1.f;
#pragma unroll
                    for (int o = 0; o < NY; ++o)
#pragma unroll
                        for (int a = 0; a < 4; ++a) {
                            const int t0 = (32 * o + 8 * a + 4 * h) >> 1;
                            float mine = acc;
                            if (h == 0) { if (t0 < Tf) mine += dd[o][a][0]; if (t0 + 1 < Tf) mine += dd[o][a][1]; }
                            float mine1 = __shfl(mine, c, 64);
                            if (h == 1) { if (t0 < Tf) mine1 += dd[o][a][0]; if (t0 + 1 < Tf) mine1 += dd[o][a][1]; }
                            acc = __shfl(mine1, c + 32, 64);
                            if (t0 == Tf - 1) fdl = dd[o][a][0];
                            if (t0 + 1 == Tf - 1) fdl = dd[o][a][1];
                        }
                    fdl = fmaxf(fdl, __shfl_xor(fdl, 32, 64));
                    const float adev = acc / (float)Tf;
                    if (live && h == 0) {
                        atomicMin(reinterpret_cast<unsigned*>(A.m_ade) + agent, __float_as_uint(adev));
                        atomicMin(reinterpret_cast<unsigned*>(A.m_fde) + agent, __float_as_uint(fdl));
                    }
                }
            }
        }
        C32_STAMP(4);
#ifdef C32_DIAG_STAMPS
        if (threadIdx.x == 0 && A.dbg && gi < 4) {
            long long* o = A.dbg + ((size_t)blockIdx.x * 4 + gi) * 16 + 10;
            o[0] = st.gap_cyc; o[1] = st.gap_n; o[2] = st.gap_cal;
        }
        st.gap_cyc = 0; st.gap_n = 0;
#endif
        ++gi;
        g = gnext;
        if (g >= ngroups) break;
    }
    C32_TRACE_END(0);
}

struct Gru32Args {
    const float* xin; int ldx;
    const f32x4* pool; const int2* prog; int prog_len;
    const float* consts;
    float* state;
    int ncols, Tp;
};
template <bool ZS>
__global__ __launch_bounds__(256, 2) void gru32_kernel(Gru32Args A) {
    extern __shared__ __attribute__((aligned(16))) char smem[];
    f32x4* ring = reinterpret_cast<f32x4*>(smem);
    float* cst = reinterpret_cast<float*>(ring + C32_RING);
    const int lane = threadIdx.x & 63, c = lane & 31, h = lane >> 5;
    const int wave = __builtin_amdgcn_readfirstlane(threadIdx.x >> 6);
    for (int i = threadIdx.x; i < 416; i += blockDim.x) cst[i] = A.consts[i];
    __syncthreads();
    ChainStream st;
    st.init(A.pool, A.prog, A.prog_len, ring);
    const int col = blockIdx.x * 128 + wave * 32 + c;
    const int colc = col < A.ncols ? col : A.ncols - 1;
    f32x16 d;
    {
        const float* xp = A.xin + (size_t)colc * A.ldx;
#pragma unroll
        for (int a = 0; a < 4; ++a) {
            f32x4 v = splat4(0.f);
            if (8 * a + 4 * h < A.ldx) v = ld4(xp + 8 * a + 4 * h);
#pragma unroll
            for (int b = 0; b < 4; ++b) d[4 * a + b] = v[b];
        }
    }
    asm volatile("s_waitcnt vmcnt(0)" ::: "memory");
    __syncthreads();
    f32x16 hs[3];
#pragma unroll
    for (int j = 0; j < 3; ++j) hs[j] = splat16(0.f);
    gru32_steps<ZS>(st, cst, cst + 384, d, hs, A.Tp, h);
    if (col < A.ncols) {
#pragma unroll
        for (int j = 0; j < 3; ++j)
#pragma unroll
            for (int a = 0; a < 4; ++a) {
                const f32x4 v = {hs[j][4 * a], hs[j][4 * a + 1], hs[j][4 * a + 2], hs[j][4 * a + 3]};
                st4(A.state + (size_t)col * 96 + 32 * j + 8 * a + 4 * h, v);
            }
    }
}

static int chain_cus() {
    static int n = 0;
    if (!n) {
        int dev = 0;
        hipDeviceProp_t p;
        if (hipGetDevice(&dev) == hipSuccess && hipGetDeviceProperties(&p, dev) == hipSuccess) n = p.multiProcessorCount;
        if (n <= 0) n = 256;
    }
    return n;
}
static int gru_zero_skip() {
    static const int v = getenv("STTODE_GRU_ZERO_SKIP") ? atoi(getenv("STTODE_GRU_ZERO_SKIP")) != 0 : 1;
    return v;
}
static int chain_lds(int NY, bool b3 = false) { return ((b3 ? 2 * C32_BUF_B3 : C32_RING) + 8 * C32_SLOT) * 16 + (1216 + 64 * NY) * 4 + 16; }

static int role_lds(int Tp) {
    const int e = (Tp * 256 + 512) * 16, g = (2 * 6 * 64 + 2 * 24 * 64 + 2 * 4 * 64) * 16;
    return e > g ? e : g;
}

static int role32_lds() { return C32_RING * 16 + R32C::total * 4; }

template <int NY, int FUSE, bool B3M = false> static int chain_launch(ChainArgs a, int wgs_per_cu, hipStream_t s) {
    void (*kern)(ChainArgs) = gru_zero_skip() ? traj_chain_kernel<NY, FUSE, B3M, true> : traj_chain_kernel<NY, FUSE, B3M, false>;
    STT_SET_LDS_ONCE(kern, 96 * 1024);
    const int ngroups = (a.ncols + 127) / 128;
    int grid = ngroups;
    if (FUSE == 1) grid = a.R.ntiles + ngroups;
    else if (FUSE == 2) {
        int workers = ngroups;
        if (a.persistent && workers > 2 * chain_cus()) workers = 2 * chain_cus();
        grid = a.R32.nwg + (a.ncols > 0 ? workers : 0);
        a.nworkers = workers;
        if (workers < ngroups) a.xcd_map = 0;
    }
    int lds = chain_lds(NY, B3M);
    if (FUSE == 1 && lds < role_lds(a.Tp)) lds = role_lds(a.Tp);
    if (FUSE == 2 && a.R32.nwg > 0 && lds < role32_lds()) lds = role32_lds();
    if (wgs_per_cu == 1 && lds < 84 * 1024) lds = 84 * 1024;
    STT_REQUIRE(lds <= 96 * 1024, "sttode_traj_chain: dynamic LDS beyond the 96 KiB the kernel is registered for");
    STT_REQUIRE((long)a.ncols * 128 <= 0xffffffffL && (long)((a.ncols + a.K - 1) / a.K) * 2048 <= 0xffffffffL,
                "sttode_traj_chain: z / per-agent table rows beyond the 32-bit byte offsets of the gathers");
    if (FUSE == 1) STT_HIP(hipMemsetAsync(a.R.flags, 0, (((size_t)a.R.ntiles + 1) * 4 + 15) / 16 * 16, s));
    hipLaunchKernelGGL(kern, dim3(grid), dim3(256), lds, s, a);
    STT_HIP(hipGetLastError());
    return 0;
}

extern "C" int sttode_gru_cols32(const float* xin, int ldx, const float* pool, const int* prog, int prog_len, const float* consts,
                                 float* state, int ncols, int Tp, void* stream) {
    STT_REQUIRE(xin && pool && prog && consts && state, "sttode_gru_cols32: null pointer");
    STT_REQUIRE(ncols > 0 && Tp >= 1 && (ldx == 16 || ldx == 32) && 2 * Tp <= ldx, "sttode_gru_cols32: bad ncols/Tp/ldx");
    STT_REQUIRE(prog_len == 13 * Tp, "sttode_gru_cols32: chunk program must hold 13 entries per step");
    Gru32Args a;
    a.xin = xin; a.ldx = ldx; a.pool = (const f32x4*)pool; a.prog = (const int2*)prog; a.prog_len = prog_len; a.consts = consts;
    a.state = state; a.ncols = ncols; a.Tp = Tp;
    const int lds = C32_RING * 16 + 416 * 4;
    hipLaunchKernelGGL(gru_zero_skip() ? gru32_kernel<true> : gru32_kernel<false>, dim3((ncols + 127) / 128), dim3(256), lds, (hipStream_t)stream, a);
    STT_HIP(hipGetLastError());
    return 0;
}

__global__ __launch_bounds__(256, 2) void sampler_qnet32_kernel(QNet32Args Q) {
    extern __shared__ __attribute__((aligned(16))) char smem[];
    f32x4* ring = reinterpret_cast<f32x4*>(smem);
    const int lane = threadIdx.x & 63, c = lane & 31, h = lane >> 5;
    const int wave = __builtin_amdgcn_readfirstlane(threadIdx.x >> 6);
    ChainStream st;
    st.init(Q.pool, Q.prog, Q.prog_len, ring);
    const int col = blockIdx.x * 128 + wave * 32 + c;
    const bool live = col < Q.n;
    const int colc = live ? col : Q.n - 1;
    f32x16 P[4];
#pragma unroll
    for (int kt = 0; kt < 4; ++kt) P[kt] = ldrows(Q.pf + (size_t)colc * 128 + 32 * kt, h);
    asm volatile("s_waitcnt vmcnt(0)" ::: "memory");
    __syncthreads();
    TileFeed<ChainStream> fd(st);
    fd.open();
    qnet32(fd, Q, P, col, colc, live, h);
    fd.close();
}

static long sampler_tiles(const SttodeSamplerPlan* p) {
    const long h1t = p->h1 / 32, h2t = p->h2 / 32;
    return 8 + h1t * (2 + h2t) + (long)p->K * h2t * (p->eps_mode ? 2 : 1);
}
const char* stt_sampler_plan_check(const SttodeSamplerPlan* p, int K) {
    if (!p || !p->pool || !p->prog || !p->biases) return "sampler plan: null pool / program / biases";
    if (p->nz != 32) return "sampler plan: nz must be 32 (one MFMA tile of rows per sample)";
    if (p->K <= 0 || (K > 0 && p->K != K)) return "sampler plan: K must be positive and equal the model's sample_k";
    if (p->h1 <= 0 || p->h1 % 32 || p->h2 <= 0 || p->h2 % 32 || p->h2 > 256) return "sampler plan: hidden widths must be multiples of 32, h2 <= 256";
    if (p->eps_mode < 0 || p->eps_mode > 2 || (p->eps_mode != 0 && !p->eps)) return "sampler plan: eps_mode 0 (mean) | 1 (shared [nz]) | 2 (per agent [n][nz]); eps required unless 0";
    if (p->prog_len <= 0 || p->prog_len > 4096) return "sampler plan: prog_len must be in [1, 4096]";
    if (3L * p->prog_len < sampler_tiles(p)) return "sampler plan: chunk program too short for the widths (<= 3 tiles per chunk)";
    return nullptr;
}
int stt_sampler_qnet(const SttodeSamplerPlan* p, const float* pf, int n, float* z, void* stream) {
    QNet32Args q;
    q.pool = (const f32x4*)p->pool; q.prog = (const int2*)p->prog; q.prog_len = p->prog_len; q.bias = p->biases;
    q.pf = pf; q.z = z; q.eps = p->eps; q.n = n; q.K = p->K; q.h1t = p->h1 / 32; q.h2t = p->h2 / 32; q.eps_mode = p->eps_mode;
    const int lds = C32_RING * 16;
    hipLaunchKernelGGL(sampler_qnet32_kernel, dim3((n + 127) / 128), dim3(256), lds, (hipStream_t)stream, q);
    STT_HIP(hipGetLastError());
    return 0;
}
extern "C" int sttode_sampler_qnet(const SttodeSamplerPlan* plan, const float* pf, int n, float* z, void* stream) {
    STT_REQUIRE(plan && pf && z, "sttode_sampler_qnet: null pointer");
    STT_REQUIRE(n > 0 && (long)n * plan->K <= 0x7fffffffL / 32, "sttode_sampler_qnet: n must be positive (and n K 32 within int range)");
    if (const char* why = stt_sampler_plan_check(plan, 0)) {
        char b[256];
        snprintf(b, sizeof(b), "sttode_sampler_qnet: %s", why);
        stt_set_error(b);
        return 1;
    }
    return stt_sampler_qnet(plan, pf, n, z, stream);
}

#if defined(C32_DIAG_STAMPS) || defined(C32_DIAG_TRACE)
static long long* g_chain_dbg = nullptr;
static int g_trace_tag = 0;
extern "C" int sttode_chain_debug_buffer(void* p) { g_chain_dbg = (long long*)p; return 0; }
#endif

extern "C" int sttode_chain_prog_len(int Tp, int Tf) {
    const int NY = (2 * Tf + 31) / 32;
    const int l3y = (8 * NY + 2) / 3;
    return (48 + 3) + (48 + l3y) + 13 * Tp + (64 + l3y);
}

static int traj_chain_impl(const float* A0x, const float* A0y, const float* A1y, const float* pool, const int* prog, int prog_len,
                           const float* consts, const float* z, const float* xpad, int ldx, const float* cur, const float* orig,
                           float* pred, int* counter, int ncols, int K, int Tp, int Tf, int wgs_per_cu, bool b3, void* stream) {
    STT_REQUIRE(A0x && A0y && A1y && pool && prog && consts && z && xpad && cur && orig && pred && counter, "sttode_traj_chain: null pointer");
    STT_REQUIRE(ncols > 0 && K > 0 && Tp >= 1 && 2 * Tp <= 32 && Tf >= 1, "sttode_traj_chain: bad ncols/K/Tp/Tf");
    STT_REQUIRE(ldx == 16 || ldx == 32, "sttode_traj_chain: ldx must be 16 or 32");
    STT_REQUIRE(wgs_per_cu == 1 || wgs_per_cu == 2, "sttode_traj_chain: wgs_per_cu must be 1 or 2");
    STT_REQUIRE(2 * Tp <= ldx, "sttode_traj_chain: xpad rows shorter than 2*Tp");
    STT_REQUIRE(prog_len == sttode_chain_prog_len(Tp, Tf), "sttode_traj_chain: chunk program length does not match (Tp, Tf)");
    ChainArgs a;
    a.A0x = A0x; a.A0y = A0y; a.A1y = A1y; a.pool = (const f32x4*)pool; a.prog = (const int2*)prog; a.prog_len = prog_len;
    a.consts = consts; a.z = z; a.xpad = xpad; a.ldx = ldx; a.cur = cur; a.orig = orig; a.pred = pred; a.park = pred; a.counter = counter;
    a.ncols = ncols; a.K = K; a.Tp = Tp; a.Tf2 = 2 * Tf;
    a.dbg = nullptr; a.trace_tag = 0; a.xcd_map = 0; a.nworkers = 0; a.m_gt = nullptr; a.m_ade = a.m_fde = nullptr; a.m_scale = 1.0f;
    a.R = RoleArgs();
    a.persistent = 0;
#if defined(C32_DIAG_STAMPS) || defined(C32_DIAG_TRACE)
    a.dbg = g_chain_dbg;
    a.trace_tag = g_trace_tag++;
#endif
    const int NY = (2 * Tf + 31) / 32;
    hipStream_t s = (hipStream_t)stream;
    if (b3) {
        switch (NY) {
            case 1: return chain_launch<1, 0, true>(a, wgs_per_cu, s);
            case 2: return chain_launch<2, 0, true>(a, wgs_per_cu, s);
            case 3: return chain_launch<3, 0, true>(a, wgs_per_cu, s);
            default: STT_REQUIRE(false, "sttode_traj_chain: future length beyond the built instantiations (2*Tf <= 96)");
        }
    }
    switch (NY) {
        case 1: return chain_launch<1, 0>(a, wgs_per_cu, s);
        case 2: return chain_launch<2, 0>(a, wgs_per_cu, s);
        case 3: return chain_launch<3, 0>(a, wgs_per_cu, s);
        default: STT_REQUIRE(false, "sttode_traj_chain: future length beyond the built instantiations (2*Tf <= 96)");
    }
    return 0;
}
extern "C" int sttode_traj_chain(const float* A0x, const float* A0y, const float* A1y, const float* pool, const int* prog, int prog_len,
                                 const float* consts, const float* z, const float* xpad, int ldx, const float* cur, const float* orig,
                                 float* pred, int* counter, int ncols, int K, int Tp, int Tf, int wgs_per_cu, void* stream) {
    return traj_chain_impl(A0x, A0y, A1y, pool, prog, prog_len, consts, z, xpad, ldx, cur, orig, pred, counter, ncols, K, Tp, Tf, wgs_per_cu, false, stream);
}
int stt_traj_chain_b3(const float* A0x, const float* A0y, const float* A1y, const float* pool, const int* prog, int prog_len,
                      const float* consts, const float* z, const float* xpad, int ldx, const float* cur, const float* orig,
                      float* pred, int* counter, int ncols, int K, int Tp, int Tf, int wgs_per_cu, void* stream) {
    return traj_chain_impl(A0x, A0y, A1y, pool, prog, prog_len, consts, z, xpad, ldx, cur, orig, pred, counter, ncols, K, Tp, Tf, wgs_per_cu, true, stream);
}

bool stt_chain_fused_covers(int Tp) { return Tp >= 2 && 2 * Tp <= 32 && role_lds(Tp) <= 80 * 1024; }
int stt_chain_fused(const float* const* W, float* ws, const long* off, int n, int K, int Tp, int Tf, int prog_len, const float* z, float* pred,
                    float ode_time, const float* attn, int ld_attn, int wgs_per_cu, int b3, int drop_tile, unsigned* tmo_host, void* stream) {
    STT_REQUIRE(W && ws && off && z && pred, "stt_chain_fused: null pointer");
    STT_REQUIRE(n > 0 && K > 0 && stt_chain_fused_covers(Tp) && Tf >= 1, "stt_chain_fused: shape outside the fused launch");
    STT_REQUIRE(!attn || (ld_attn >= 64 && ld_attn % 4 == 0), "stt_chain_fused: bad attention leading dimension");
    STT_REQUIRE(prog_len == sttode_chain_prog_len(Tp, Tf), "stt_chain_fused: chunk program length does not match (Tp, Tf)");
    STT_REQUIRE((long)n * K <= 0x7fffffffL, "stt_chain_fused: too many trajectories");
    ChainArgs a;
    a.A0x = ws + off[STT_B_A0X]; a.A0y = ws + off[STT_B_A0Y]; a.A1y = ws + off[STT_B_A1Y];
    a.pool = (const f32x4*)W[b3 ? STT_W_CHAINB3_POOL : STT_W_CHAIN_POOL]; a.prog = (const int2*)W[b3 ? STT_W_CHAINB3_PROG : STT_W_CHAIN_PROG];
    a.prog_len = prog_len;
    a.consts = W[STT_W_CHAIN_CONSTS]; a.z = z; a.xpad = ws + off[STT_B_XPAD]; a.ldx = 2 * Tp <= 16 ? 16 : 32; a.cur = ws + off[STT_B_CUR];
    a.orig = ws + off[STT_B_ORIG]; a.pred = pred; a.park = pred; a.counter = (int*)(ws + off[STT_B_QUEUE]);
    a.ncols = n * K; a.K = K; a.Tp = Tp; a.Tf2 = 2 * Tf; a.persistent = 0; a.dbg = nullptr; a.trace_tag = 0; a.xcd_map = 0; a.nworkers = 0;
    a.m_gt = nullptr; a.m_ade = a.m_fde = nullptr; a.m_scale = 1.0f;
#if defined(C32_DIAG_STAMPS) || defined(C32_DIAG_TRACE)
    a.dbg = g_chain_dbg;
    a.trace_tag = g_trace_tag++;
#endif
    RoleArgs& r = a.R;
    role_args_fill(r, W, ws, off);
    r.attn = attn; r.ld_attn = ld_attn;
    r.past = nullptr; r.scene_ptr = nullptr; r.S = 0;
    r.flags = (unsigned*)(ws + off[STT_B_FLAGS]); r.ntiles = (n + 15) / 16; r.ode_time = ode_time;
    r.tmo_host = tmo_host;
    a.xcd_map = 1;
    r.drop_tile = drop_tile;
    const int NY = (2 * Tf + 31) / 32;
    hipStream_t s = (hipStream_t)stream;
    switch (NY) {
        case 1: return b3 ? chain_launch<1, 1, true>(a, wgs_per_cu, s) : chain_launch<1, 1>(a, wgs_per_cu, s);
        case 2: return b3 ? chain_launch<2, 1, true>(a, wgs_per_cu, s) : chain_launch<2, 1>(a, wgs_per_cu, s);
        case 3: return b3 ? chain_launch<3, 1, true>(a, wgs_per_cu, s) : chain_launch<3, 1>(a, wgs_per_cu, s);
        default: STT_REQUIRE(false, "stt_chain_fused: future length beyond the built instantiations (2*Tf <= 96)");
    }
    return 0;
}

bool stt_chain_lagged_covers(int Tp) { return Tp >= 2 && 2 * Tp <= 32; }
int stt_chain_lagged(const float* const* W, const LagRoles& lr, const LagGroups& lg, int K, int Tp, int Tf, int prog_len, int b3, void* stream) {
    float* ws_r = lr.ws; const long* off_r = lr.off; const int n_r = lr.n; const float* attn = lr.attn; const int ld_attn = lr.ld_attn;
    const float ode_time = lr.ode_time; float* zgen = lr.zgen; const unsigned long long zkey = lr.zkey; const float* past = lr.past;
    const int* scene_ptr = lr.scene_ptr; const int S = lr.S; float* r_ade = lr.ade; float* r_fde = lr.fde;
    float* ws_g = lg.ws; const long* off_g = lg.off; const int n_g = lg.n; const float* z = lg.z; float* pred = lg.pred;
    const float* g_gt = lg.gt; float* g_ade = lg.ade; float* g_fde = lg.fde; const float g_scale = lg.scale; const int lag_workers_ok = lg.workers;
    STT_REQUIRE(W && (ws_r || ws_g), "stt_chain_lagged: nothing to launch");
    STT_REQUIRE(K > 0 && stt_chain_lagged_covers(Tp) && Tf >= 1, "stt_chain_lagged: shape outside the lagged launch");
    ChainArgs a;
    a.R = RoleArgs();
    a.R32 = Role32Args();
    a.dbg = nullptr; a.trace_tag = 0; a.xcd_map = 0; a.persistent = 0; a.counter = nullptr; a.nworkers = 0;
    a.K = K; a.Tp = Tp; a.Tf2 = 2 * Tf; a.ldx = 2 * Tp <= 16 ? 16 : 32; a.ncols = 0;
    a.pool = (const f32x4*)W[b3 ? STT_W_CHAINB3_POOL : STT_W_CHAIN_POOL]; a.prog = (const int2*)W[b3 ? STT_W_CHAINB3_PROG : STT_W_CHAIN_PROG];
    a.prog_len = prog_len; a.consts = W[STT_W_CHAIN_CONSTS];
    a.A0x = a.A0y = a.A1y = nullptr; a.z = nullptr; a.xpad = nullptr; a.cur = a.orig = nullptr; a.pred = nullptr; a.park = nullptr;
    a.m_gt = nullptr; a.m_ade = a.m_fde = nullptr; a.m_scale = 1.0f;
    if (ws_g && g_gt) {
        STT_REQUIRE(g_ade && g_fde, "stt_chain_lagged: fused metrics need ade and fde");
        a.m_gt = g_gt; a.m_ade = g_ade; a.m_fde = g_fde; a.m_scale = g_scale;
    }
    if (ws_g) {
        STT_REQUIRE(off_g && z && pred && n_g > 0 && (long)n_g * K <= 0x7fffffffL, "stt_chain_lagged: bad group arguments");
        STT_REQUIRE(prog_len == sttode_chain_prog_len(Tp, Tf), "stt_chain_lagged: chunk program length does not match (Tp, Tf)");
        a.A0x = ws_g + off_g[STT_B_A0X]; a.A0y = ws_g + off_g[STT_B_A0Y]; a.A1y = ws_g + off_g[STT_B_A1Y];
        a.z = z; a.xpad = ws_g + off_g[STT_B_XPAD]; a.cur = ws_g + off_g[STT_B_CUR]; a.orig = ws_g + off_g[STT_B_ORIG]; a.pred = pred;
        a.park = ws_g + off_g[STT_B_YBUF];
        a.ncols = n_g * K;
        a.persistent = lag_workers_ok ? 1 : 0;
        a.counter = (int*)(ws_g + off_g[STT_B_QUEUE]);
        a.xcd_map = 1;
    }
    if (ws_r) {
        STT_REQUIRE(off_r && n_r > 0, "stt_chain_lagged: bad role arguments");
        STT_REQUIRE(!attn || (ld_attn >= 64 && ld_attn % 4 == 0), "stt_chain_lagged: bad attention leading dimension");
        Role32Args& r = a.R32;
        r.pool = (const f32x4*)W[STT_W_ROLE32_POOL];
        r.prog = (const int2*)W[attn ? STT_W_ROLE32_PROG_NBA : STT_W_ROLE32_PROG_SCENES];
        r.consts = W[attn ? STT_W_ROLE32_CONSTS_NBA : STT_W_ROLE32_CONSTS_SCENES];
        r.kte = (4 * Tp + 31) / 32;
        const int e = attn ? 8 : 2 * r.kte + 8;
        r.prog_len = attn ? 13 * Tp + (e + 2) / 3 + (128 + 288 + 2) / 3 : 13 * Tp + (e + 128 + 288 + 2) / 3;
        r.enc_in = ws_r + off_r[STT_B_ENC_IN]; r.last = (const int*)(ws_r + off_r[STT_B_LAST]);
        r.g_in = ws_r + off_r[STT_B_G]; r.attn = attn; r.ld_attn = ld_attn;
        r.xpad = ws_r + off_r[STT_B_XPAD]; r.ldx = a.ldx;
        r.pf = ws_r + off_r[STT_B_PF]; r.state0 = ws_r + off_r[STT_B_STATE0];
        r.A0x = ws_r + off_r[STT_B_A0X]; r.A0y = ws_r + off_r[STT_B_A0Y]; r.A1y = ws_r + off_r[STT_B_A1Y];
        r.n = n_r; r.Tp = Tp; r.nwg = (n_r + 127) / 128; r.ode_time = ode_time;
        r.prio = 3;
        r.counter = (int*)(ws_r + off_r[STT_B_QUEUE]);
        r.zgen = zgen; r.zkey0 = (unsigned)zkey; r.zkey1 = (unsigned)(zkey >> 32); r.K = K;
        STT_REQUIRE(!past || (scene_ptr && S > 0 && !attn), "stt_chain_lagged: the in-role front-end needs scene_ptr, S > 0 and attention length 1");
        r.past = past; r.scene_ptr = scene_ptr; r.S = S;
        r.scene_orig = ws_r + off_r[STT_B_SCENE_ORIG]; r.agent_scene = (int*)(ws_r + off_r[STT_B_AGENT_SCENE]);
        r.enc_in_w = ws_r + off_r[STT_B_ENC_IN]; r.xpad_w = ws_r + off_r[STT_B_XPAD]; r.cur_w = ws_r + off_r[STT_B_CUR];
        r.orig_w = ws_r + off_r[STT_B_ORIG]; r.last_w = (int*)(ws_r + off_r[STT_B_LAST]);
        r.m_ade = r_ade; r.m_fde = r_fde;
    }
#if defined(C32_DIAG_STAMPS) || defined(C32_DIAG_TRACE)
    a.dbg = g_chain_dbg;
    a.trace_tag = g_trace_tag++;
#endif
    const int NY = (2 * Tf + 31) / 32;
    hipStream_t s = (hipStream_t)stream;
    switch (NY) {
        case 1: return b3 ? chain_launch<1, 2, true>(a, 2, s) : chain_launch<1, 2>(a, 2, s);
        case 2: return b3 ? chain_launch<2, 2, true>(a, 2, s) : chain_launch<2, 2>(a, 2, s);
        case 3: return b3 ? chain_launch<3, 2, true>(a, 2, s) : chain_launch<3, 2>(a, 2, s);
        default: STT_REQUIRE(false, "stt_chain_lagged: future length beyond the built instantiations (2*Tf <= 96)");
    }
    return 0;
}
```

### sttode_amd/csrc/pipeline.hip

```cpp
#include "api_util.hpp"
#include "../../include/sttode_hip.h"
#include <vector>
#include <algorithm>
#include <utility>
#include <cstring>
#include <mutex>
#include <cstdlib>

#define STT_MAX_DEVICES 64
#define STT_MAX_SLOTS 8
#define STT_GRU0_LAT_TILES 4096
struct TimRec { int stage; hipEvent_t e0, e1; };

struct LagPending { bool valid; float* ws; long off[STT_B_COUNT]; int n; const float* z; float* pred; hipStream_t s; int si;
                    const float* gt; float* ade; float* fde; float scale;
                    int one_launch; };

struct SttodeModel {
    int Tp, Tf, TPX, NOY, K;
    const float* w[STT_W_COUNT];
    int n_chunks0, n_chunks1;
    hipStream_t side;
    hipEvent_t ev_fork, ev_join;
    int chain_mode;
    int fused_mode;
    hipStream_t slot_stream[STT_MAX_SLOTS];
    int scene_launch;
    int drop_tile;
    int b3;
    int ode_method, ode_steps;
    int prog_len;
    hipStream_t sA, sB, sB2;
    std::mutex mu;
    unsigned* tmo_host;
    int lag_streams;
    long lag_calls;
    LagPending lag[STT_MAX_SLOTS];
    int lag_q[4][STT_MAX_SLOTS]; int lag_qn[4];
    hipStream_t sLag4;
    long acalls;
    hipEvent_t ev_call, evA_done[STT_MAX_SLOTS], evB_done[STT_MAX_SLOTS];
    bool timing;
    int timing_every;
    long calls;
    std::vector<TimRec> recs;
    std::vector<hipEvent_t> pool;
};

bool stt_embed_qkv_fe_covers(int n, int Tlen);
int stt_embed_qkv_fe(const float* const* W, const float* past, int n, int N, int Tlen, int TPX, float* xpad, float* enc_in, float* cur,
                     float* orig, int* last, float* g, float* qkv, void* stream);

int stt_post_attn_stage(const float* const* W, const float* state, const float* attn, int ld_attn, const float* base, const float* kA, float cA,
                        const float* kB, float cB, const float* kC, float cC, float cN, float* kout, float* out, float* qkv, const float* g,
                        float* pf, int n, void* stream);

static std::mutex g_stream_mu;

#define STT_TMO_WORDS 4096
static unsigned* g_tmo_pool = nullptr;
static std::vector<int> g_tmo_free;
static unsigned* tmo_word_take() {
    std::lock_guard<std::mutex> lk(g_stream_mu);
    if (!g_tmo_pool) {
        if (hipHostMalloc((void**)&g_tmo_pool, STT_TMO_WORDS * sizeof(unsigned), hipHostMallocDefault) != hipSuccess) { g_tmo_pool = nullptr; return nullptr; }
        memset(g_tmo_pool, 0, STT_TMO_WORDS * sizeof(unsigned));
        for (int i = STT_TMO_WORDS - 1; i >= 0; --i) g_tmo_free.push_back(i);
    }
    if (g_tmo_free.empty()) return nullptr;
    const int i = g_tmo_free.back();
    g_tmo_free.pop_back();
    g_tmo_pool[i] = 0u;
    return g_tmo_pool + i;
}
static void tmo_word_give(unsigned* w) {
    if (!w || !g_tmo_pool) return;
    std::lock_guard<std::mutex> lk(g_stream_mu);
    g_tmo_free.push_back((int)(w - g_tmo_pool));
}

static inline size_t al(size_t x) { return (x + 63) & ~(size_t)63; }

extern "C" int sttode_model_create(SttodeModel** out, const void* const* weights, int count, int Tp, int Tf, int K,
                                   int n_chunks0, int n_chunks1) {
    STT_REQUIRE(out && weights, "sttode_model_create: null pointer");
    STT_REQUIRE(count == STT_W_COUNT, "sttode_model_create: weight table must have STT_W_COUNT entries");
    STT_REQUIRE(Tp >= 2 && 2 * Tp <= 32 && Tf >= 1 && K >= 1, "sttode_model_create: bad Tp/Tf/K");
    for (int i = 0; i < count; ++i)
        STT_REQUIRE(weights[i] != nullptr || i == STT_W_CHAINB3_POOL || i == STT_W_CHAINB3_PROG, "sttode_model_create: null weight pointer");
    SttodeModel* m = new SttodeModel();
    m->Tp = Tp; m->Tf = Tf; m->K = K;
    m->TPX = (2 * Tp <= 16) ? 1 : 2;
    m->NOY = (2 * Tf + 15) / 16;
    for (int i = 0; i < count; ++i) m->w[i] = (const float*)weights[i];
    m->n_chunks0 = n_chunks0; m->n_chunks1 = n_chunks1;
    m->timing = false;
    m->timing_every = 0;
    m->calls = 0;
    m->acalls = 0;
    m->chain_mode = -1;
    m->ode_method = 0; m->ode_steps = 1;
    m->fused_mode = 1;
    m->b3 = 0;
    m->drop_tile = -1;
    for (int p = 0; p < STT_MAX_SLOTS; ++p) { m->slot_stream[p] = nullptr; m->lag[p].valid = false; }
    m->lag_streams = 3;
    m->lag_calls = 0;
    m->tmo_host = nullptr;
    for (int i = 0; i < 4; ++i) m->lag_qn[i] = 0;
    if (const char* e = getenv("STTODE_LAGGED")) m->lag_streams = atoi(e) >= 2 && atoi(e) <= 4 ? atoi(e) : 0;
    m->scene_launch = 128;
    m->prog_len = sttode_chain_prog_len(Tp, Tf);
    m->side = nullptr;
    bool ok = hipEventCreateWithFlags(&m->ev_fork, hipEventDisableTiming) == hipSuccess &&
              hipEventCreateWithFlags(&m->ev_join, hipEventDisableTiming) == hipSuccess;
    static hipStream_t g_sA[STT_MAX_DEVICES] = {}, g_sB[STT_MAX_DEVICES] = {}, g_sB2[STT_MAX_DEVICES] = {};
    static hipStream_t g_sLag4[STT_MAX_DEVICES] = {};
    int dev = 0;
    ok = ok && hipGetDevice(&dev) == hipSuccess && dev >= 0 && dev < STT_MAX_DEVICES;
    if (ok) {
        std::lock_guard<std::mutex> lk(g_stream_mu);
        if (!g_sA[dev]) {
            ok = hipStreamCreateWithFlags(&g_sA[dev], hipStreamNonBlocking) == hipSuccess &&
                 hipStreamCreateWithFlags(&g_sB[dev], hipStreamNonBlocking) == hipSuccess &&
                 hipStreamCreateWithFlags(&g_sB2[dev], hipStreamNonBlocking) == hipSuccess;
            if (!ok) g_sA[dev] = nullptr;
        }
        if (ok) { m->sA = g_sA[dev]; m->sB = g_sB[dev]; m->sB2 = g_sB2[dev]; }
        if (ok && !g_sLag4[dev]) ok = hipStreamCreateWithFlags(&g_sLag4[dev], hipStreamNonBlocking) == hipSuccess;
        m->sLag4 = g_sLag4[dev];
    }
    ok = ok && hipEventCreateWithFlags(&m->ev_call, hipEventDisableTiming) == hipSuccess;
    if (ok) { m->tmo_host = tmo_word_take(); ok = m->tmo_host != nullptr; }
    for (int p = 0; p < STT_MAX_SLOTS && ok; ++p)
        ok = hipEventCreateWithFlags(&m->evA_done[p], hipEventDisableTiming) == hipSuccess &&
             hipEventCreateWithFlags(&m->evB_done[p], hipEventDisableTiming) == hipSuccess;
    if (!ok) {
        tmo_word_give(m->tmo_host);
        delete m;
        stt_set_error("sttode_model_create: could not create streams / events");
        return 2;
    }
    *out = m;
    return 0;
}

extern "C" int sttode_model_set_weight(SttodeModel* m, int index, const void* ptr) {
    STT_REQUIRE(m && ptr && index >= 0 && index < STT_W_COUNT, "sttode_model_set_weight: bad arguments");
    m->w[index] = (const float*)ptr;
    return 0;
}

extern "C" int sttode_model_destroy(SttodeModel* m) {
    if (!m) return 0;
    hipStreamCaptureMode mode = hipStreamCaptureModeRelaxed;
    const bool exchanged = hipThreadExchangeStreamCaptureMode(&mode) == hipSuccess;
    if (!exchanged) (void)hipGetLastError();
    for (auto& r : m->recs) { (void)hipEventDestroy(r.e0); (void)hipEventDestroy(r.e1); }
    for (auto e : m->pool) (void)hipEventDestroy(e);
    (void)hipEventDestroy(m->ev_fork); (void)hipEventDestroy(m->ev_join);
    (void)hipEventDestroy(m->ev_call);
    for (int p = 0; p < STT_MAX_SLOTS; ++p) { (void)hipEventDestroy(m->evA_done[p]); (void)hipEventDestroy(m->evB_done[p]); }
    tmo_word_give(m->tmo_host);
    delete m;
    if (exchanged) (void)hipThreadExchangeStreamCaptureMode(&mode);
    return 0;
}

extern "C" int sttode_workspace_layout(const SttodeModel* m, int n, int S, long* offsets, long* total_floats) {
    STT_REQUIRE(m && offsets && total_floats, "sttode_workspace_layout: null pointer");
    STT_REQUIRE(n > 0 && S >= 0, "sttode_workspace_layout: bad n/S");
    const size_t mm = (size_t)n * m->K;
    size_t o = 0;
    auto put = [&](int id, size_t cnt) { offsets[id] = (long)o; o += al(cnt); };
    put(STT_B_SCENE_ORIG, (size_t)(S > 0 ? S : 1) * 2);
    put(STT_B_AGENT_SCENE, n);
    put(STT_B_XPAD, (size_t)n * 16 * m->TPX);
    put(STT_B_ENC_IN, (size_t)n * m->Tp * 4);
    put(STT_B_CUR, (size_t)n * 2);
    put(STT_B_ORIG, (size_t)n * 2);
    put(STT_B_LAST, n);
    put(STT_B_G, (size_t)n * 64);
    put(STT_B_QKV, (size_t)n * 192);
    put(STT_B_ATTN, (size_t)n * 64);
    put(STT_B_PF, (size_t)n * 128);
    put(STT_B_STATE0, (size_t)n * 96);
    put(STT_B_A0X, (size_t)n * 512);
    put(STT_B_A0Y, (size_t)n * 512);
    put(STT_B_A1Y, (size_t)n * 512);
    put(STT_B_DBUF, mm * 16 * m->TPX);
    put(STT_B_YBUF, mm * 16 * m->NOY);
    put(STT_B_STATE1, mm * 96);
    put(STT_B_QUEUE, 64);
    put(STT_B_FLAGS, (size_t)8 * ((n + 15) / 16) + 8 + (mm + 15) / 16);
    put(STT_B_ODE, (size_t)6 * n * 64);
    *total_floats = (long)o;
    return 0;
}

extern "C" int sttode_set_chain(SttodeModel* m, int mode) {
    STT_REQUIRE(m, "sttode_set_chain: null model");
    STT_REQUIRE(mode >= -1 && mode <= 1, "sttode_set_chain: mode must be -1 (auto), 0 or 1");
    m->chain_mode = mode;
    return 0;
}

extern "C" int sttode_set_fused(SttodeModel* m, int mode) {
    STT_REQUIRE(m, "sttode_set_fused: null model");
    STT_REQUIRE(mode == 0 || mode == 1, "sttode_set_fused: mode must be 0 or 1 (modes 2-4 were retired)");
    m->fused_mode = mode;
    return 0;
}

static int lag_flush_all(SttodeModel* m);
extern "C" int sttode_set_lagged(SttodeModel* m, int streams) {
    STT_REQUIRE(m, "sttode_set_lagged: null model");
    STT_REQUIRE(streams == 0 || (streams >= 2 && streams <= 4), "sttode_set_lagged: streams must be 0 (off), 2, 3 or 4");
    std::lock_guard<std::mutex> lk(m->mu);
    if (int rc = lag_flush_all(m)) return rc;
    m->lag_streams = streams;
    m->lag_calls = 0;
    return 0;
}

extern "C" int sttode_debug_drop_role_flag(SttodeModel* m, int tile) {
    STT_REQUIRE(m && tile >= -1, "sttode_debug_drop_role_flag: bad arguments");
    m->drop_tile = tile;
    return 0;
}

extern "C" int sttode_set_scene_launch(SttodeModel* m, int max_tiles) {
    STT_REQUIRE(m, "sttode_set_scene_launch: null model");
    STT_REQUIRE(max_tiles >= -1, "sttode_set_scene_launch: max_tiles must be -1 (default), 0 (off) or a tile count");
    m->scene_launch = max_tiles < 0 ? 128 : max_tiles;
    return 0;
}

extern "C" int sttode_set_mfma_mode(SttodeModel* m, int mode) {
    STT_REQUIRE(m, "sttode_set_mfma_mode: null model");
    STT_REQUIRE(mode == 0 || mode == 1, "sttode_set_mfma_mode: mode must be 0 (fp32) or 1 (three-way bf16 split, exploratory)");
    STT_REQUIRE(mode == 0 || (m->w[STT_W_CHAINB3_POOL] && m->w[STT_W_CHAINB3_PROG]),
                "sttode_set_mfma_mode: the bf16-split weight stream has not been handed over (sttode_model_set_weight)");
    m->b3 = mode;
    return 0;
}

extern "C" int sttode_set_ode(SttodeModel* m, int method, int steps) {
    STT_REQUIRE(m, "sttode_set_ode: null model");
    STT_REQUIRE(method >= 0 && method <= 2 && steps >= 1 && steps <= 1024, "sttode_set_ode: method in {0,1,2}, 1 <= steps <= 1024");
    m->ode_method = method; m->ode_steps = steps;
    return 0;
}

extern "C" int sttode_timing_enable(SttodeModel* m, int every) {
    STT_REQUIRE(m && every >= 0, "sttode_timing_enable: bad arguments");
    m->timing_every = every;
    m->timing = false;
    m->calls = 0;
    return 0;
}

static hipEvent_t get_event(SttodeModel* m) {
    if (!m->pool.empty()) { hipEvent_t e = m->pool.back(); m->pool.pop_back(); return e; }
    hipEvent_t e = nullptr;
    (void)hipEventCreate(&e);
    return e;
}

extern "C" int sttode_timing_read(SttodeModel* m, double* total_ms, int* launches, double* busy_ms) {
    STT_REQUIRE(m && total_ms && launches, "sttode_timing_read: null pointer");
    for (int i = 0; i < STT_STAGE_COUNT; ++i) { total_ms[i] = 0.0; launches[i] = 0; if (busy_ms) busy_ms[i] = 0.0; }
    std::vector<std::pair<double, double>> iv[STT_STAGE_COUNT];
    hipEvent_t ref = m->recs.empty() ? nullptr : m->recs.front().e0;
    for (auto& r : m->recs) {
        STT_HIP(hipEventSynchronize(r.e1));
        float ms = 0.f, t0 = 0.f;
        STT_HIP(hipEventElapsedTime(&ms, r.e0, r.e1));
        total_ms[r.stage] += ms;
        launches[r.stage] += 1;
        if (busy_ms && r.e0 != ref) {
            STT_HIP(hipEventSynchronize(r.e0));
            STT_HIP(hipEventElapsedTime(&t0, ref, r.e0));
        }
        iv[r.stage].push_back({(double)t0, (double)t0 + (double)ms});
    }
    if (busy_ms)
        for (int st = 0; st < STT_STAGE_COUNT; ++st) {
            std::sort(iv[st].begin(), iv[st].end());
            double cur0 = 0, cur1 = 0;
            bool open = false;
            for (auto& p : iv[st]) {
                if (!open) { cur0 = p.first; cur1 = p.second; open = true; }
                else if (p.first <= cur1) { if (p.second > cur1) cur1 = p.second; }
                else { busy_ms[st] += cur1 - cur0; cur0 = p.first; cur1 = p.second; }
            }
            if (open) busy_ms[st] += cur1 - cur0;
        }
    for (auto& r : m->recs) { m->pool.push_back(r.e0); m->pool.push_back(r.e1); }
    m->recs.clear();
    return 0;
}

struct StageTimer {
    SttodeModel* m; int stage; hipStream_t s; hipEvent_t e0 = nullptr, e1 = nullptr; bool on = false;
    StageTimer(SttodeModel* m_, int st, hipStream_t s_) : m(m_), stage(st), s(s_) {
        on = m->timing || (m->timing_every > 0 && ((stage >= STT_STAGE_MLP0 && stage <= STT_STAGE_CHAIN) || stage == STT_STAGE_FUSED));
        if (on) { e0 = get_event(m); e1 = get_event(m); (void)hipEventRecord(e0, s); }
    }
    ~StageTimer() {
        if (on) { (void)hipEventRecord(e1, s); m->recs.push_back({stage, e0, e1}); }
    }
};

#define RUN(stage, s, call)                         \
    do {                                            \
        StageTimer _t(m, stage, s);                 \
        int _rc = (call);                           \
        if (_rc) return _rc;                        \
    } while (0)

static int attention(float* qkv, float* attn, int groups, int attn_len, int attn_slots, hipStream_t s) {
    const long st_seq = (long)attn_slots * 192, gq = (long)attn_len * st_seq, go = (long)attn_len * attn_slots * 64;
    return sttode_mhgsa_attn_groups(qkv + 64, qkv, qkv + 128, attn, groups, gq, gq, gq, go, attn_len, attn_len, attn_slots, st_seq, 192, st_seq, 192,
                                    st_seq, 192, (long)attn_slots * 64, 64, 1.0f, 0.35355339059327373f, 8, s);
}

static int stage_agents(SttodeModel* m, float* ws, const long* off, int n, int groups, int attn_len, int attn_slots, hipStream_t s, bool use_side) {
    const float* const* W = m->w;
    const int Tp = m->Tp, TPX = m->TPX;
    float* xpad = ws + off[STT_B_XPAD];
    float* g = ws + off[STT_B_G];
    float* qkv = ws + off[STT_B_QKV];
    float* attn = ws + off[STT_B_ATTN];
    float* pf = ws + off[STT_B_PF];
    float* state0 = ws + off[STT_B_STATE0];
    float *A0x = ws + off[STT_B_A0X], *A0y = ws + off[STT_B_A0Y], *A1y = ws + off[STT_B_A1Y];

    const int ntiles = (n + 15) / 16;
    if (attn_len == 1 && m->ode_method == 0 && m->ode_steps == 1 && stt_agents_fused_covers(Tp, TPX) &&
        ntiles <= (use_side ? stt_gru_lat_tiles() : STT_GRU0_LAT_TILES) && ntiles <= stt_enc_lat_tiles()) {
        RUN(STT_STAGE_AGENTS, s,
            stt_agents_fused(W, ws + off[STT_B_ENC_IN], (const int*)(ws + off[STT_B_LAST]), g, qkv, pf, xpad, state0, n, Tp, TPX, 12.0f, s));
        RUN(STT_STAGE_LINEAR, s,
            sttode_agent_preact(pf, state0, W[STT_W_B0_XWA], W[STT_W_B0_XB1], W[STT_W_B0_YWA], W[STT_W_B0_YB1], W[STT_W_B1_YWA], W[STT_W_B1_YB1],
                                A0x, A0y, A1y, n, s));
        return 0;
    }
    if (use_side && !m->side) {
        static hipStream_t g_side[STT_MAX_DEVICES] = {};
        int dev = 0;
        STT_HIP(hipGetDevice(&dev));
        STT_REQUIRE(dev >= 0 && dev < STT_MAX_DEVICES, "sttode_inference_*: device index beyond STT_MAX_DEVICES");
        {
            std::lock_guard<std::mutex> lk(g_stream_mu);
            if (!g_side[dev]) STT_HIP(hipStreamCreateWithFlags(&g_side[dev], hipStreamNonBlocking));
            m->side = g_side[dev];
        }
    }
    hipStream_t gs = use_side ? m->side : s;
    if (use_side) {
        STT_HIP(hipEventRecord(m->ev_fork, s));
        STT_HIP(hipStreamWaitEvent(m->side, m->ev_fork, 0));
    }
    if (TPX == 2) {
        RUN(STT_STAGE_GRU0, gs,
            sttode_gru_cols32(xpad, 16 * TPX, W[STT_W_G0_POOL], (const int*)W[STT_W_G0_PROG], 13 * Tp, W[STT_W_G0_CONSTS], state0, n, Tp, gs));
    } else
        RUN(STT_STAGE_GRU0, gs,
            stt_gru_cols_form(xpad, W[STT_W_B0_CONVP], W[STT_W_B0_CONVB], W[STT_W_B0_WIHP], W[STT_W_B0_WHHP], W[STT_W_B0_GBIAS], state0, n,
                              Tp, TPX, use_side ? 0 : STT_GRU0_LAT_TILES, gs));
    if (use_side) STT_HIP(hipEventRecord(m->ev_join, m->side));

    RUN(STT_STAGE_EMBED, s,
        sttode_embed_qkv(W[STT_W_FC1P], W[STT_W_FC1B], W[STT_W_POSP], W[STT_W_PEB], W[STT_W_FC2P], W[STT_W_FC2B], W[STT_W_FC3P],
                         W[STT_W_FC3B], W[STT_W_FC3LAST], W[STT_W_INP], W[STT_W_INB], ws + off[STT_B_ENC_IN],
                         (const int*)(ws + off[STT_B_LAST]), g, qkv, n, Tp, s));
    const float* attn_src = qkv + 128;
    int ld_attn = 192;
    if (attn_len > 1) {
        RUN(STT_STAGE_ATTN, s, attention(qkv, attn, groups, attn_len, attn_slots, s));
        attn_src = attn;
        ld_attn = 64;
    }
    if ((m->ode_method != 0 || m->ode_steps != 1) && attn_len > 1) {
        float* ob = ws + off[STT_B_ODE];
        const size_t nf = (size_t)n * 64;
        float *y = ob, *k1 = ob + nf, *k2 = ob + 2 * nf, *k3 = ob + 3 * nf, *t = ob + 5 * nf;
        auto attention_of_state = [&]() -> int {
            RUN(STT_STAGE_ATTN, s, attention(qkv, attn, groups, attn_len, attn_slots, s));
            return 0;
        };
        auto stage = [&](const float* state, const float* base, const float* kA, double cA, const float* kB, double cB, const float* kC, double cC,
                         double cN, float* kout, float* out, bool last) -> int {
            RUN(STT_STAGE_POST, s,
                stt_post_attn_stage(W, state, attn, 64, base, kA, (float)cA, kB, (float)cB, kC, (float)cC, (float)cN, kout, out, last ? nullptr : qkv,
                                    g, last ? pf : nullptr, n, s));
            return last ? 0 : attention_of_state();
        };
#define ODE_DO(call) do { if (int _rc = (call)) return _rc; } while (0)
        const double h = 12.0 / (double)m->ode_steps;
        for (int st = 0; st < m->ode_steps; ++st) {
            const bool fin = st + 1 == m->ode_steps;
            const float* y0 = st == 0 ? g : y;
            if (m->ode_method == 0) { ODE_DO(stage(y0, y0, nullptr, 0, nullptr, 0, nullptr, 0, h, nullptr, y, fin)); continue; }
            if (m->ode_method == 1) {
                ODE_DO(stage(y0, y0, nullptr, 0, nullptr, 0, nullptr, 0, h / 3, k1, t, false));
                ODE_DO(stage(t, y0, k1, -h / 3, nullptr, 0, nullptr, 0, h, k2, t, false));
                ODE_DO(stage(t, y0, k1, h, k2, -h, nullptr, 0, h, k3, t, false));
                ODE_DO(stage(t, y0, k1, h / 8, k2, 3 * h / 8, k3, 3 * h / 8, h / 8, nullptr, y, fin));
            } else {
                ODE_DO(stage(y0, y0, nullptr, 0, nullptr, 0, nullptr, 0, h / 2, k1, t, false));
                ODE_DO(stage(t, y0, nullptr, 0, nullptr, 0, nullptr, 0, h / 2, k2, t, false));
                ODE_DO(stage(t, y0, nullptr, 0, nullptr, 0, nullptr, 0, h, k3, t, false));
                ODE_DO(stage(t, y0, k1, h / 6, k2, h / 3, k3, h / 3, h / 6, nullptr, y, fin));
            }
        }
#undef ODE_DO
    } else if (m->ode_method != 0 || m->ode_steps != 1) {
        RUN(STT_STAGE_POST, s,
            sttode_post_attn_ode(W[STT_W_OUTP], W[STT_W_OUTB], W[STT_W_INFOP], W[STT_W_INFOB], W[STT_W_GATEP], W[STT_W_GATEB], W[STT_W_LN1W],
                                 W[STT_W_LN1B], W[STT_W_L1P], W[STT_W_L1B], W[STT_W_L2P], W[STT_W_L2B], W[STT_W_LN2W], W[STT_W_LN2B],
                                 W[STT_W_INP], W[STT_W_INB], g, pf, n, 12.0f, m->ode_method, m->ode_steps, s));
    } else
    RUN(STT_STAGE_POST, s,
        sttode_post_attn(W[STT_W_OUTP], W[STT_W_OUTB], W[STT_W_INFOP], W[STT_W_INFOB], W[STT_W_GATEP], W[STT_W_GATEB], W[STT_W_LN1W],
                         W[STT_W_LN1B], W[STT_W_L1P], W[STT_W_L1B], W[STT_W_L2P], W[STT_W_L2B], W[STT_W_LN2W], W[STT_W_LN2B], g,
                         attn_src, ld_attn, pf, n, 12.0f, s));
    if (use_side) STT_HIP(hipStreamWaitEvent(s, m->ev_join, 0));
    RUN(STT_STAGE_LINEAR, s,
        sttode_agent_preact(pf, state0, W[STT_W_B0_XWA], W[STT_W_B0_XB1], W[STT_W_B0_YWA], W[STT_W_B0_YB1], W[STT_W_B1_YWA], W[STT_W_B1_YB1],
                            A0x, A0y, A1y, n, s));
    return 0;
}

static int stage_trajectories(SttodeModel* m, float* ws, const long* off, int n, const float* z, float* pred, hipStream_t s, bool pipelined) {
    const float* const* W = m->w;
    const int K = m->K, Tp = m->Tp, Tf = m->Tf, TPX = m->TPX, NOY = m->NOY;
    const float* xpad = ws + off[STT_B_XPAD];
    const float *A0x = ws + off[STT_B_A0X], *A0y = ws + off[STT_B_A0Y], *A1y = ws + off[STT_B_A1Y];
    float *dbuf = ws + off[STT_B_DBUF], *ybuf = ws + off[STT_B_YBUF], *state1 = ws + off[STT_B_STATE1];
    const long ncols_all = (long)n * K;
    const bool fused = m->chain_mode == 1 || (m->chain_mode < 0 && ncols_all >= 16384);
    if (fused) {
        if (m->b3) {
            RUN(STT_STAGE_CHAIN, s,
                stt_traj_chain_b3(A0x, A0y, A1y, W[STT_W_CHAINB3_POOL], (const int*)W[STT_W_CHAINB3_PROG], m->prog_len, W[STT_W_CHAIN_CONSTS], z,
                                  xpad, 16 * TPX, ws + off[STT_B_CUR], ws + off[STT_B_ORIG], pred, (int*)(ws + off[STT_B_QUEUE]), (int)ncols_all, K,
                                  Tp, Tf, pipelined ? 1 : 2, s));
            return 0;
// ... 392 lines not shown
```

### sttode_amd/csrc/role32.hpp

```cpp
#pragma once

struct R32C {
    static constexpr int bc = 0, wlast = 64, bi = 128, bg = 192, ln1w = 256, ln1b = 320, l1b = 384, l2b = 1408, ln2w = 1472, ln2b = 1536,
                         gb = 1600, cb = 1984, b1x = 2016, b1y = 2528, b11 = 3040, total = 3552;
};

typedef const __attribute__((address_space(4))) Role32Args KRole32Args;

template <class ST> struct TileFeed {
    ST& st; int t, cnt; bool pre;
    Frag cur, nxt;
    __device__ __forceinline__ explicit TileFeed(ST& s) : st(s), t(0), cnt(0), pre(false) {}
    __device__ __forceinline__ void open() {
        cnt = st.cnt;
        t = 0;
        ldfrag(cur, st.cur());
        st.begin();
        pre = false;
    }
    __device__ __forceinline__ void mma(f32x16& acc, const f32x16& B) {
        if (t == cnt) { st.end(true); open(); }
        else if (pre) cur = nxt;
        const f32x4* tn = t + 1 < cnt ? st.cur() + (t + 1) * C32_TILE : nullptr;
        tile_mma2f(st, acc, cur, B, nxt, tn, t == 0 ? 1 : 0);
// ... 18 lines not shown
#pragma unroll
        for (int r = 0; r < 16; ++r) { const float dd = x[j][r] - mean; v += dd * dd; }
    const float rstd = 1.0f / sqrtf(halfsum32(v) * (1.0f / 64.0f) + 1e-5f);
#pragma unroll
    for (int j = 0; j < 2; ++j) {
        const f32x16 g = ldrows(gamma + 32 * j, h), b = ldrows(beta + 32 * j, h);
#pragma unroll
        for (int r = 0; r < 16; ++r) x[j][r] = (x[j][r] - mean) * rstd * g[r] + b[r];
    }
}

__device__ __forceinline__ void strows(float* p, const f32x16& v, int h) {
#pragma unroll
    for (int a = 0; a < 4; ++a) {
        const f32x4 w = {v[4 * a], v[4 * a + 1], v[4 * a + 2], v[4 * a + 3]};
        st4(p + 8 * a + 4 * h, w);
    }
}

template <int KT, class FD>
__device__ __forceinline__ void table32(FD& fd, const float* bias, float* out, const f32x16 (&B)[7], int col, bool live, int h) {
#pragma unroll 1
    for (int rt = 0; rt < 16; ++rt) {
        f32x16 acc = ldrows(bias + 32 * rt, h);
#pragma unroll
        for (int kt = 0; kt < KT; ++kt) fd.mma(acc, B[kt]);
        if (live) strows(out + (size_t)col * 512 + 32 * rt, acc, h);
    }
}

__device__ __forceinline__ void philox4x32_10(unsigned (&c)[4], unsigned k0, unsigned k1) {
#pragma unroll
    for (int r = 0; r < 10; ++r) {
        const unsigned long long p0 = (unsigned long long)0xD2511F53u * c[0], p1 = (unsigned long long)0xCD9E8D57u * c[2];
        const unsigned n0 = (unsigned)(p1 >> 32) ^ c[1] ^ k0, n2 = (unsigned)(p0 >> 32) ^ c[3] ^ k1;
        c[0] = n0; c[1] = (unsigned)p1; c[2] = n2; c[3] = (unsigned)p0;
        k0 += 0x9E3779B9u; k1 += 0xBB67AE85u;
    }
}
__device__ __forceinline__ void latents32(float* z, unsigned k0, unsigned k1, int wg, int n, int K) {
    const int a0 = wg * 128, na = n - a0 < 128 ? n - a0 : 128;
    const long first4 = (long)a0 * K * 8;
    const int count4 = na * K * 8;
    for (int i = threadIdx.x; i < count4; i += blockDim.x) {
        const unsigned long long g4 = (unsigned long long)(first4 + i);
        unsigned c[4] = {(unsigned)g4, (unsigned)(g4 >> 32), 0u, 0u};
        philox4x32_10(c, k0, k1);
        f32x4 v;
#pragma unroll
        for (int p = 0; p < 2; ++p) {
            const float u1 = (float)(c[2 * p] >> 8) * 5.9604644775390625e-8f + 2.98023223876953125e-8f;
            const float u2 = (float)(c[2 * p + 1] >> 8) * 5.9604644775390625e-8f + 2.98023223876953125e-8f;
            const float rad = sqrtf(-2.0f * __logf(u1));
            float sn, cs;
            __sincosf(6.283185307179586f * u2, &sn, &cs);
            v[2 * p] = rad * cs; v[2 * p + 1] = rad * sn;
        }
        st4(z + (first4 + i) * 4, v);
    }
}

__device__ __forceinline__ void frontend32(KRole32Args& R, int wg) {
    const int a = wg * 128 + (int)threadIdx.x;
    if (threadIdx.x < 128 && a < R.n) {
        int lo = 0, hi = R.S - 1;
        while (lo < hi) {
            const int mid = (lo + hi + 1) >> 1;
            if (R.scene_ptr[mid] <= a) lo = mid; else hi = mid - 1;
        }
        const int a0 = R.scene_ptr[lo], a1 = R.scene_ptr[lo + 1];
        float sx = 0.f, sy = 0.f;
        for (int aa = a0; aa < a1; ++aa) {
            sx += R.past[((size_t)aa * R.Tp + (R.Tp - 1)) * 2 + 0];
            sy += R.past[((size_t)aa * R.Tp + (R.Tp - 1)) * 2 + 1];
        }
        const float inv = (float)(a1 - a0);
        const float ox = sx / inv, oy = sy / inv;
        if (a == a0) { R.scene_orig[2 * lo] = ox; R.scene_orig[2 * lo + 1] = oy; }
        R.agent_scene[a] = lo;
        agent_inputs_core<false, 16>(a, R.past, R.Tp, R.ldx / 16, 1, ox, oy, a == a1 - 1, nullptr, R.xpad_w, R.enc_in_w, R.cur_w, R.orig_w, R.last_w);
    }
}

template <bool ZS>
__device__ __forceinline__ void role32_body(KRole32Args& R, int wg, char* smem) {
    f32x4* ring = reinterpret_cast<f32x4*>(smem);
    float* cst = reinterpret_cast<float*>(ring + C32_RING);
    const int lane = threadIdx.x & 63, c = lane & 31, h = lane >> 5;
    const int wave = __builtin_amdgcn_readfirstlane(threadIdx.x >> 6);
    if (R.prio > 0) __builtin_amdgcn_s_setprio(3);
    if (wg == 0 && threadIdx.x == 0) *R.counter = 0;
    if (R.m_ade && threadIdx.x < 128 && wg * 128 + (int)threadIdx.x < R.n) {
        R.m_ade[wg * 128 + threadIdx.x] = INFINITY;
        R.m_fde[wg * 128 + threadIdx.x] = INFINITY;
    }
    if (R.past) frontend32(R, wg);
    if (R.zgen) latents32(R.zgen, R.zkey0, R.zkey1, wg, R.n, R.K);
    if (R.past) {
        __builtin_amdgcn_fence(__ATOMIC_RELEASE, "workgroup");
        __syncthreads();
        __builtin_amdgcn_fence(__ATOMIC_ACQUIRE, "workgroup");
    }
    for (int i = threadIdx.x; i < R32C::total; i += blockDim.x) cst[i] = R.consts[i];
    __syncthreads();
    ChainStream st;
    st.init(R.pool, R.prog, R.prog_len, ring);
    const int col = wg * 128 + wave * 32 + c;
    const bool live = col < R.n;
    const int colc = live ? col : R.n - 1;
    f32x16 d;
    {
        const float* xp = R.xpad + (size_t)colc * R.ldx;
#pragma unroll
        for (int a = 0; a < 4; ++a) {
            f32x4 v = splat4(0.f);
            if (8 * a + 4 * h < R.ldx) v = ld4(xp + 8 * a + 4 * h);
#pragma unroll
            for (int b = 0; b < 4; ++b) d[4 * a + b] = v[b];
        }
    }
    int Tp = R.Tp;
    asm volatile("" : "+s"(Tp));
    asm volatile("s_waitcnt vmcnt(0)" ::: "memory");
    __syncthreads();
    f32x16 hs[3];
#pragma unroll
    for (int j = 0; j < 3; ++j) hs[j] = splat16(0.f);
    gru32_steps<ZS>(st, cst + R32C::gb, cst + R32C::cb, d, hs, Tp, h);
    if (live) {
#pragma unroll
        for (int j = 0; j < 3; ++j) strows(R.state0 + (size_t)col * 96 + 32 * j, hs[j], h);
    }
    STT_FENCE();
    TileFeed<ChainStream> fd(st);
    fd.open();
    f32x16 G[2], S[2];
    if (R.attn == nullptr) {
        f32x16 X[2];
        const float* ep = R.enc_in + (size_t)colc * (4 * R.Tp);
#pragma unroll
        for (int kt = 0; kt < 2; ++kt)
#pragma unroll
            for (int a = 0; a < 4; ++a) {
                f32x4 v = splat4(0.f);
                if (32 * kt + 8 * a + 4 * h < 4 * R.Tp) v = ld4(ep + 32 * kt + 8 * a + 4 * h);
#pragma unroll
                for (int b = 0; b < 4; ++b) X[kt][4 * a + b] = v[b];
            }
        const float lastf = R.last[colc] ? 1.0f : 0.0f;
#pragma unroll
        for (int j = 0; j < 2; ++j) {
            const f32x16 b = ldrows(cst + R32C::bc + 32 * j, h), wl = ldrows(cst + R32C::wlast + 32 * j, h);
#pragma unroll
            for (int r = 0; r < 16; ++r) G[j][r] = fmaf(wl[r], lastf, b[r]);
            fd.mma(G[j], X[0]);
            if (R.kte > 1) fd.mma(G[j], X[1]);
        }
        S[0] = G[0]; S[1] = G[1];
    } else {
#pragma unroll
        for (int j = 0; j < 2; ++j) {
            G[j] = ldrows(R.g_in + (size_t)colc * 64 + 32 * j, h);
            S[j] = ldrows(R.attn + (size_t)colc * R.ld_attn + 32 * j, h);
        }
    }
    f32x16 XR[2];
#pragma unroll
    for (int j = 0; j < 2; ++j) {
        f32x16 vi = ldrows(cst + R32C::bi + 32 * j, h);
        fd.mma(vi, S[0]);
        fd.mma(vi, S[1]);
        f32x16 vg = ldrows(cst + R32C::bg + 32 * j, h);
        fd.mma(vg, S[0]);
        fd.mma(vg, S[1]);
#pragma unroll
        for (int r = 0; r < 16; ++r) XR[j][r] = G[j][r] + tanhf(vi[r]) * sigmoidf_(vg[r]);
    }
    layernorm64_c32(XR, cst + R32C::ln1w, cst + R32C::ln1b, h);
    {
        f32x16 FF[2];
        FF[0] = splat16(0.f); FF[1] = splat16(0.f);
#pragma unroll 1
        for (int ht = 0; ht < 32; ++ht) {
            f32x16 hid = ldrows(cst + R32C::l1b + 32 * ht, h);
            fd.mma(hid, XR[0]);
            fd.mma(hid, XR[1]);
            hid = relu16(hid);
            fd.mma(FF[0], hid);
            fd.mma(FF[1], hid);
        }
#pragma unroll
        for (int j = 0; j < 2; ++j) {
            const f32x16 b = ldrows(cst + R32C::l2b + 32 * j, h);
            XR[j] = XR[j] + (FF[j] + b);
        }
    }
    layernorm64_c32(XR, cst + R32C::ln2w, cst + R32C::ln2b, h);
    f32x16 B7[7];
#pragma unroll
    for (int j = 0; j < 2; ++j) {
        B7[j] = G[j];
        B7[2 + j] = relu16(G[j] + XR[j] * R.ode_time);
    }
#pragma unroll
    for (int j = 0; j < 3; ++j) B7[4 + j] = hs[j];
    if (live) {
#pragma unroll
        for (int j = 0; j < 4; ++j) strows(R.pf + (size_t)col * 128 + 32 * j, B7[j], h);
    }
    table32<7>(fd, cst + R32C::b1x, R.A0x, B7, col, live, h);
    table32<7>(fd, cst + R32C::b1y, R.A0y, B7, col, live, h);
    table32<4>(fd, cst + R32C::b11, R.A1y, B7, col, live, h);
    fd.close();
}

struct QNet32Args {
    const f32x4* pool; const int2* prog; int prog_len; const float* bias;
    const float* pf; float* z; const float* eps;
    int n, K, h1t, h2t, eps_mode;
};

__device__ __forceinline__ f32x16 tanh16(f32x16 v) {
#pragma unroll
    for (int e = 0; e < 16; ++e) v[e] = tanhf(v[e]);
    return v;
}

template <class FD>
__device__ __forceinline__ void qnet32(FD& fd, const QNet32Args& Q, const f32x16 (&P)[4], int col, int colc, bool live, int h) {
    const float* bl = Q.bias;
    const float* b1 = bl + 64;
    const float* b2 = b1 + 32 * Q.h1t;
    const float* bb = b2 + 32 * Q.h2t;
    const float* bA = bb + 32 * Q.K;
    f32x16 H0[2];
#pragma unroll
    for (int j = 0; j < 2; ++j) {
        H0[j] = ldrows(bl + 32 * j, h);
#pragma unroll
        for (int kt = 0; kt < 4; ++kt) fd.mma(H0[j], P[kt]);
    }
    f32x16 H2[8];
#pragma unroll
    for (int j = 0; j < 8; ++j) H2[j] = splat16(0.f);
#pragma unroll 1
    for (int ht = 0; ht < Q.h1t; ++ht) {
        f32x16 hid = ldrows(b1 + 32 * ht, h);
        fd.mma(hid, H0[0]);
        fd.mma(hid, H0[1]);
        hid = tanh16(hid);
#pragma unroll
        for (int j = 0; j < 8; ++j)
            if (j < Q.h2t) fd.mma(H2[j], hid);
    }
#pragma unroll
    for (int j = 0; j < 8; ++j)
        if (j < Q.h2t) H2[j] = tanh16(H2[j] + ldrows(b2 + 32 * j, h));
    f32x16 E = splat16(0.f);
    if (Q.eps_mode == 1) E = ldrows(Q.eps, h);
    else if (Q.eps_mode == 2) E = ldrows(Q.eps + (size_t)colc * 32, h);
#pragma unroll 1
    for (int k = 0; k < Q.K; ++k) {
        f32x16 zb = ldrows(bb + 32 * k, h);
#pragma unroll
        for (int j = 0; j < 8; ++j)
            if (j < Q.h2t) fd.mma(zb, H2[j]);
        if (Q.eps_mode != 0) {
            f32x16 za = ldrows(bA + 32 * k, h);
#pragma unroll
            for (int j = 0; j < 8; ++j)
                if (j < Q.h2t) fd.mma(za, H2[j]);
#pragma unroll
            for (int r = 0; r < 16; ++r) zb[r] = fmaf(za[r], E[r], zb[r]);
        }
        if (live) strows(Q.z + ((size_t)col * Q.K + k) * 32, zb, h);
    }
}
```

### sttode_amd/model.py

```python
import os
import operator

import numpy as np
import torch
from torch import nn

from .dist import Normal
from . import capi, packing
from .weights import sinusoid_table_np

_DEBUG = os.environ.get('STTODE_DEBUG', '0') not in ('', '0')


class _HypMHSA(nn.Module):

    def __init__(self, d, h):
        super().__init__()
        self.embed_dim, self.num_heads = d, h
        self.in_proj_weight = nn.Parameter(torch.empty(3 * d, d))
        self.in_proj_bias = nn.Parameter(torch.zeros(3 * d))
        self.out_proj = nn.Linear(d, d)
        nn.init.xavier_uniform_(self.in_proj_weight)
        nn.init.zeros_(self.out_proj.bias)

# ... 129 lines not shown
        self.max_train_agent = args.max_train_agent
        self.rand_rot_scene = args.rand_rot_scene
        self.discrete_rot = args.discrete_rot
        scale_num = 2 + len(args.hyper_scales)
        self.past_encoder = _Trunk(args, args.past_length)
        self.pz_layer = nn.Linear(scale_num * args.hidden_dim, 2 * args.zdim)
        self.future_encoder = _Trunk(args, args.future_length, future=True)
        self.decoder = _Decoder(args)
        self.param_annealers = nn.ModuleList()
        self._packed = None
        self._packed_key = None
        self._mode = None
        self._async_calls = 0
        self.ode_method, self.ode_steps = 'euler', 1
        self.mfma_mode = 'bf16x3' if os.environ.get('STTODE_BF16X3', '0') not in ('', '0') else 'f32'
        self.diverse_mode = getattr(args, 'diverse_mode', 'marginal')
        self._diverse_joint()
        self._host_futures = {}
        self.async_depth = 6
        self.device_latents = os.environ.get('STTODE_DEVICE_LATENTS', '1') != '0'
        self._async_bufs = {}
        self._async_metrics = {}
        self._ext_streams = {}
        self._ptr_cache = {}
        self._pf = self._pf_thunk = None
        self.to(self.device)

    DIVERSE_MODES = ('marginal', 'joint')

    def _diverse_joint(self):
        if self.diverse_mode not in self.DIVERSE_MODES:
            raise ValueError(f"diverse_mode must be 'marginal' or 'joint', got {self.diverse_mode!r}")
        return self.diverse_mode == 'joint'

    def _joint_seg_len(self, n):
        return int(self._N) if self._mode == 'nba' else int(n)

    @property
    def past_feature(self):
        if self._pf is None and self._pf_thunk is not None:
            self._pf, self._pf_thunk = self._pf_thunk(), None
        return self._pf

    @past_feature.setter
    def past_feature(self, value):
        self._pf, self._pf_thunk = value, None

    _PLAIN = frozenset(('_past', '_future', '_scene_ptr', '_mode', 'batch_size', 'agent_num', '_S', '_N', '_G', 'pre_motion_mask', 'fut_motion_mask',
                        'scene_orig', '_pf', '_pf_thunk', '_ws', '_dbg', 'diverse_pred', '_plist'))

    def __setattr__(self, name, value):
        if name in STTODENet._PLAIN:
            self.__dict__[name] = value
        else:
            super().__setattr__(name, value)

    def set_device(self, device):
        self.device = torch.device(device)
        self.to(self.device)

    def step_annealer(self):
        for anl in self.param_annealers:
            anl.step()

    def _weights_key(self):
        if getattr(self, '_plist', None) is None:
            self._plist = list(self.parameters()) + list(self.buffers())
        return (self.device.index, tuple(map(_DATA_PTR, self._plist)), tuple(map(_VERSION, self._plist)))

    def _apply(self, fn, *a, **k):
        self._plist = None
        return super()._apply(fn, *a, **k)

    def packed(self):
        if self._generic:
            return {}
        key = self._weights_key()
        if self._packed is None or key != self._packed_key:
            if getattr(self, '_native', None) is not None:
                capi.call('sttode_async_flush', self._native.h)
                torch.cuda.synchronize(self.device)
            sd = {k: v.detach().cpu().numpy() for k, v in self.state_dict().items()}
            a = self.args
            host = {'past': packing.pack_trunk(sd, 'past_encoder.', a.past_length),
                    'blk0': packing.pack_block(sd, 0, a.past_length, a.future_length, first=True),
                    'blk1': packing.pack_block(sd, 1, a.past_length, a.future_length, first=False),
                    'future': packing.pack_trunk(sd, 'future_encoder.', a.future_length),
                    'post': packing.pack_posterior(sd),
                    'chain': packing.chain_stream(sd, a.past_length, a.future_length),
                    'gru0s': packing.gru32_stream(sd, 0, a.past_length),
                    'role32': packing.role_stream(sd, a.past_length)}
            self._packed = {g: {k: (torch.from_numpy(np.ascontiguousarray(v)).to(self.device) if isinstance(v, np.ndarray) else v)
                                for k, v in d.items()} for g, d in host.items()}
            self._packed_key = key
            self._native = capi.NativeModel(self._packed, a.past_length, a.future_length, a.sample_k) if self.device.type == 'cuda' else None
            self._wscache = {}
            self._async_bufs = {}
        return self._packed

    def release_native(self):
        if self.device.type == 'cuda':
            if getattr(self, '_native', None) is not None:
                capi.call('sttode_async_flush', self._native.h)
            torch.cuda.synchronize(self.device)
        self._native, self._packed, self._packed_key = None, None, None
        self._wscache, self._async_bufs = {}, {}

    def native(self, check_weights=True):
        if self._generic:
            raise capi.SttodeError('the native pipeline (fused launches, packed weight streams) is built for the reference widths hidden_dim 64, '
                                   'zdim 32, num_decompose 2, 2 Tp <= 32, 2 Tf <= 96; this model runs the generic form (sttode_amd/generic.py)')
        if check_weights or self._packed is None or self._native is None:
            self.packed()
        ode = (self.ODE_METHODS[self.ode_method], int(self.ode_steps))
        if self._native is not None and getattr(self._native, '_ode', (0, 1)) != ode:
            self._native.set_ode(*ode)
            self._native._ode = ode
        if self._native is not None and getattr(self._native, '_mfma', None) != self.mfma_mode:
            if self.mfma_mode not in ('f32', 'bf16x3'):
                raise ValueError("mfma_mode must be 'f32' or 'bf16x3'")
            if self.mfma_mode == 'bf16x3' and 'chain_b3' not in self._packed:
                sd = {k: v.detach().cpu().numpy() for k, v in self.state_dict().items()}
                b3 = packing.chain_stream_b3(sd, self.args.past_length, self.args.future_length)
                self._native.set_weights('chain_b3', {k: (torch.from_numpy(np.ascontiguousarray(v)).to(self.device) if isinstance(v, np.ndarray) else v)
                                                      for k, v in b3.items()})
            self._native.set_mfma_mode(1 if self.mfma_mode == 'bf16x3' else 0)
            self._native._mfma = self.mfma_mode
        return self._native

    def _workspace(self, n, S):
        key = (n, S)
        if key not in self._wscache:
            if len(self._wscache) > 8:
                self._wscache.clear()
            off, tot = self._native.layout(n, S)
            buf = torch.empty(tot, dtype=torch.float32, device=self.device)
            self._native.init_workspace(buf, n, S)
            self._wscache[key] = (buf, off)
        return self._wscache[key]

    def _view(self, buf, off, name, *shape, dtype=torch.float32):
        cnt = int(np.prod(shape))
        v = buf[off[name]: off[name] + cnt]
        if dtype != torch.float32:
            v = v.view(dtype)
        return v.view(*shape)

    def _require_gpu(self):
        if self.device.type != 'cuda':
            raise capi.SttodeError('STTODENet compute runs only on a HIP device (no CPU fallback); got device=%s' % self.device)

    def set_data(self, batch, pre_motion, fut_motion, pre_motion_mask=None, fut_motion_mask=None, theta=None):
        dev = self.device
        if (not self.training and theta is None and type(pre_motion) is torch.Tensor and type(fut_motion) is torch.Tensor
                and pre_motion.dtype is torch.float32 and fut_motion.dtype is torch.float32 and not pre_motion.is_cuda and not fut_motion.is_cuda
                and dev.type == 'cuda' and pre_motion.dim() == 3 and pre_motion.shape[1] == 2 and pre_motion.shape[2] == self.args.past_length
                and pre_motion.shape[0] > 0 and fut_motion.shape == (pre_motion.shape[0], 2, self.args.future_length)):
            N = pre_motion.shape[0]
            past, fut = self._stage_scene(pre_motion, fut_motion)
            ptr = self._ptr_cache.get(N)
            if ptr is None or not _on(ptr, dev):
                ptr = self._ptr_cache[N] = torch.tensor([0, N], dtype=torch.int32).to(dev)
            d = self.__dict__
            d['_past'], d['_future'], d['_scene_ptr'], d['_mode'], d['batch_size'], d['agent_num'], d['_S'], d['_N'] = past, fut, ptr, 'scenes', 1, N, 1, 0
            d['_G'] = 1
            d['pre_motion_mask'], d['fut_motion_mask'] = pre_motion_mask, fut_motion_mask
            return

        def to_dev(x):
            x = torch.as_tensor(x, dtype=torch.float32)
            return x.permute(0, 2, 1).contiguous().to(dev)
        pre_motion = torch.as_tensor(pre_motion, dtype=torch.float32)
        fut_motion = torch.as_tensor(fut_motion, dtype=torch.float32) if fut_motion is not None else None
        if torch.device(dev).type == 'cuda' and not pre_motion.is_cuda and (fut_motion is None or not fut_motion.is_cuda):
            past, fut = self._stage_scene(pre_motion, fut_motion)
        else:
            past = to_dev(pre_motion)
            fut = to_dev(fut_motion) if fut_motion is not None else None
        if self.training and past.shape[0] > self.max_train_agent:
            ind = torch.tensor(np.random.choice(past.shape[0], self.max_train_agent).tolist(), device=dev)
            past = past.index_select(0, ind).contiguous()
            fut = fut.index_select(0, ind).contiguous() if fut is not None else None
            pre_motion_mask = pre_motion_mask.to(dev).index_select(0, ind) if pre_motion_mask is not None else None
            fut_motion_mask = fut_motion_mask.to(dev).index_select(0, ind) if fut_motion_mask is not None else None
        if (self.training and self.rand_rot_scene) or theta is not None:
            if theta is None:
                theta = (torch.randint(high=24, size=(1,)) * (np.pi / 12)) if self.discrete_rot else torch.rand(1) * np.pi * 2
            th = float(theta)
            c, s_ = float(np.cos(np.float32(th))), float(np.sin(np.float32(th)))
            if past.is_cuda:
                past = past.contiguous()
                fut = fut.contiguous() if fut is not None else None
                capi.call('sttode_rotate_scene', past, fut, past.shape[0], past.shape[1], fut.shape[1] if fut is not None else 0, c, s_,
                          capi.stream_ptr())
            else:
# ... 738 lines not shown
```

### sttode_amd/packing.py

```python
import numpy as np


def _pad16(n):
    return (n + 15) // 16 * 16


def pk16(W):
    W = np.asarray(W, np.float32)
    N, K = W.shape
    Np, Kp = _pad16(N), _pad16(K)
    Wp = np.zeros((Np, Kp), np.float32)
    Wp[:N, :K] = W
    X = Wp.reshape(Np // 16, 16, Kp // 16, 4, 4)
    X = X.transpose(0, 2, 3, 1, 4)
    return np.ascontiguousarray(X.reshape(Np // 16, Kp // 16, 64, 4))


def pk4(W):
    W = np.asarray(W, np.float32)
    N = W.shape[0]
    assert W.shape[1] == 4 and N % 16 == 0
    return np.ascontiguousarray(W.reshape(N // 16, 16, 4).transpose(0, 2, 1).reshape(N // 16, 64))


# ... 234 lines not shown
    assert len(prog) == f['prog_len']
    return {'pool': np.ascontiguousarray(np.concatenate(words)), 'prog': np.ascontiguousarray(np.asarray(prog, np.int32)),
            'consts': f['consts'], 'prog_len': len(prog)}


def chain_stream(sd, Tp, Tf):
    NY = tiles_y32(Tf)
    g = lambda k: np.asarray(sd[k], np.float32)
    tiles, prog = [], []

    def add(ts):
        base = len(tiles)
        tiles.extend(ts)
        for o in range(0, len(ts), 3):
            prog.append((base + o, min(3, len(ts) - o)))

    def mlp(prefix, kcols, NO, n_out):
        W1, W2, W3 = g(prefix + 'layers.0.weight'), g(prefix + 'layers.1.weight'), g(prefix + 'layers.2.weight')
        P1 = pk32_tiles(W1[:, kcols])
        P2 = pk32_tiles(W2)
        W3p = np.zeros((32 * NO, 256), np.float32)
        W3p[:n_out] = W3
        P3 = pk32_tiles(W3p)
        for ht in range(16):
            add(list(P1[ht]) + [P2[R, ht] for R in range(8)])
        add([P3[o, T] for o in range(NO) for T in range(8)])
        b3 = np.zeros(32 * NO, np.float32)
        b3[:n_out] = g(prefix + 'layers.2.bias')
        return g(prefix + 'layers.1.bias'), b3

    b2x, b3x = mlp('decoder.decompose.0.decoder_x.', slice(128, 160), 1, 2 * Tp)
    b2y, b3y = mlp('decoder.decompose.0.decoder_y.', slice(128, 160), NY, 2 * Tf)
    p = 'decoder.decompose.1.'
    L2E = np.float32(1.4426950408889634)
    sc = np.concatenate([np.full(192, -L2E, np.float32), np.full(96, 2 * L2E, np.float32)])
    wih = g(p + 'encoder_past.weight_ih_l0') * sc[:, None]
    whh = g(p + 'encoder_past.weight_hh_l0') * sc[:, None]
    bih, bhh = g(p + 'encoder_past.bias_ih_l0'), g(p + 'encoder_past.bias_hh_l0')
    Pih, Phh = pk32_tiles(wih), pk32_tiles(whh)
    gru = []
    for j in range(3):
        gru += [Pih[j, 0], Phh[j, 0], Phh[j, 1], Phh[j, 2], Pih[3 + j, 0], Phh[3 + j, 0], Phh[3 + j, 1], Phh[3 + j, 2],
                Phh[6 + j, 0], Phh[6 + j, 1], Phh[6 + j, 2], Pih[6 + j, 0]]
    conv = pk32_tiles(toeplitz_conv(g(p + 'conv_past.weight'), Tp, 2))
    gru_base, conv_base = len(tiles), len(tiles) + 36
    tiles.extend(gru)
    tiles.extend(conv[t, 0] for t in range(Tp))
    for t in range(Tp):
        prog.append((conv_base + t, 1))
        prog.extend((gru_base + 3 * c, 3) for c in range(12))
    gbias = np.concatenate([(bih[:96] + bhh[:96]) * -L2E, (bih[96:192] + bhh[96:192]) * -L2E, bih[192:] * (2 * L2E), bhh[192:] * (2 * L2E)])
    b2m, b3m = mlp(p + 'decoder_y.', slice(128, 256), NY, 2 * Tf)
    consts = np.concatenate([b2x, b3x, b2y, b3y, gbias, g(p + 'conv_past.bias'), b2m, b3m]).astype(np.float32)
    assert consts.size == 1216 + 64 * NY and len(prog) == chain_prog_len(Tp, Tf), (consts.size, len(prog))
    return {'pool': np.ascontiguousarray(np.stack(tiles)), 'prog': np.ascontiguousarray(np.asarray(prog, np.int32)),
            'consts': np.ascontiguousarray(consts), 'prog_len': len(prog)}


def gru32_stream(sd, block, Tp):
    p = f'decoder.decompose.{block}.'
    g = lambda k: np.asarray(sd[p + k], np.float32)
    L2E = np.float32(1.4426950408889634)
    sc = np.concatenate([np.full(192, -L2E, np.float32), np.full(96, 2 * L2E, np.float32)])
    wih, whh = g('encoder_past.weight_ih_l0') * sc[:, None], g('encoder_past.weight_hh_l0') * sc[:, None]
    bih, bhh = g('encoder_past.bias_ih_l0'), g('encoder_past.bias_hh_l0')
    Pih, Phh = pk32_tiles(wih), pk32_tiles(whh)
    tiles = []
    for j in range(3):
        tiles += [Pih[j, 0], Phh[j, 0], Phh[j, 1], Phh[j, 2], Pih[3 + j, 0], Phh[3 + j, 0], Phh[3 + j, 1], Phh[3 + j, 2],
                  Phh[6 + j, 0], Phh[6 + j, 1], Phh[6 + j, 2], Pih[6 + j, 0]]
    conv = pk32_tiles(toeplitz_conv(g('conv_past.weight'), Tp, 2))
    tiles.extend(conv[t, 0] for t in range(Tp))
    prog = []
    for t in range(Tp):
        prog.append((36 + t, 1))
        prog.extend((3 * c, 3) for c in range(12))
    gbias = np.concatenate([(bih[:96] + bhh[:96]) * -L2E, (bih[96:192] + bhh[96:192]) * -L2E, bih[192:] * (2 * L2E), bhh[192:] * (2 * L2E)])
    consts = np.concatenate([gbias, g('conv_past.bias')]).astype(np.float32)
    assert consts.size == 416 and len(prog) == 13 * Tp
    return {'pool': np.ascontiguousarray(np.stack(tiles)), 'prog': np.ascontiguousarray(np.asarray(prog, np.int32)),
            'consts': np.ascontiguousarray(consts), 'prog_len': len(prog)}


R32_CONSTS = dict(bc=0, wlast=64, bi=128, bg=192, ln1w=256, ln1b=320, l1b=384, l2b=1408, ln2w=1472, ln2b=1536, gbias=1600, convb=1984,
                  b1x=2016, b1y=2528, b11=3040, total=3552)


def role_fold(sd, Tp):
    f64 = lambda k: np.asarray(sd[k], np.float64)
    pe_ = 'past_encoder.'
    att = pe_ + 'ODE_Encoder.odeblock.odefunc.layers.0.self_attn.'
    W1, b1 = f64(pe_ + 'input_fc.weight'), f64(pe_ + 'input_fc.bias')
    Wpos, bpos, pe = f64(pe_ + 'pos_encoder.fc.weight'), f64(pe_ + 'pos_encoder.fc.bias'), f64(pe_ + 'pos_encoder.pe')
    W2, b2 = f64(pe_ + 'input_fc2.weight'), f64(pe_ + 'input_fc2.bias')
    W3, b3 = f64(pe_ + 'input_fc3.weight'), f64(pe_ + 'input_fc3.bias')
    W3a = W3[:, :64]
    kte = (4 * Tp + 31) // 32
    Wc = np.zeros((64, 32 * kte))
    acc = b2.copy()
    for t in range(Tp):
        W2t = W2[:, 64 * t:64 * t + 64]
        Wc[:, 4 * t:4 * t + 4] = W3a @ W2t @ Wpos[:, :64] @ W1
        acc = acc + W2t @ (Wpos[:, :64] @ b1 + Wpos[:, 64:] @ pe[t] + bpos)
    Win, bin_ = f64(att + 'temporal_attention_before.in_proj_weight'), f64(att + 'temporal_attention_before.in_proj_bias')
    Wo, bo = f64(att + 'temporal_attention_before.out_proj.weight'), f64(att + 'temporal_attention_before.out_proj.bias')
    Wi, bi = f64(att + 'temporal_info.weight'), f64(att + 'temporal_info.bias')
    Wg, bg = f64(att + 'temporal_gate.weight'), f64(att + 'temporal_gate.bias')
    WoWv, boc = Wo @ Win[128:192], Wo @ bin_[128:192] + bo
    return {'kte': kte, 'Wc': Wc, 'bc': W3a @ acc + b3, 'wlast': W3[:, 66],
            'Ki_scenes': Wi @ WoWv, 'Kg_scenes': Wg @ WoWv, 'bi_scenes': Wi @ boc + bi, 'bg_scenes': Wg @ boc + bg,
            'Ki_nba': Wi @ Wo, 'Kg_nba': Wg @ Wo, 'bi_nba': Wi @ bo + bi, 'bg_nba': Wg @ bo + bg}


def role_stream(sd, Tp):
    f64 = lambda k: np.asarray(sd[k], np.float64)
    att = 'past_encoder.ODE_Encoder.odeblock.odefunc.layers.0.'
    F = role_fold(sd, Tp)
    kte = F['kte']
    gs = gru32_stream(sd, 0, Tp)
    tiles = list(gs['pool'])
    gru_prog = [tuple(int(v) for v in e) for e in gs['prog']]

    def chunks(first, count):
        return [(first + o, min(3, count - o)) for o in range(0, count, 3)]

    def e_tiles(v):
        Pi, Pg = pk32_tiles(F['Ki_' + v]), pk32_tiles(F['Kg_' + v])
        ts = []
        if v == 'scenes':
            P = pk32_tiles(F['Wc'])
            ts += [P[j, kt] for j in range(2) for kt in range(kte)]
        for j in range(2):
            ts += [Pi[j, 0], Pi[j, 1], Pg[j, 0], Pg[j, 1]]
        return ts

    P1, P2 = pk32_tiles(f64(att + 'linear1.weight')), pk32_tiles(f64(att + 'linear2.weight'))
    rest = []
    for ht in range(32):
        rest += [P1[ht, 0], P1[ht, 1], P2[0, ht], P2[1, ht]]
    for blk, nm, with_state in ((0, 'x', True), (0, 'y', True), (1, 'y', False)):
        Wl = f64(f'decoder.decompose.{blk}.decoder_{nm}.layers.0.weight')
        P = pk32_tiles(np.concatenate([Wl[:, :128], Wl[:, 160:256]], axis=1) if with_state else Wl[:, :128])
        rest += [P[rt, kt] for rt in range(16) for kt in range(P.shape[1])]
    es, en = e_tiles('scenes'), e_tiles('nba')
    base_s = len(tiles)
    tiles += es + rest
    base_n = len(tiles)
    tiles += en
    progs = {'scenes': gru_prog + chunks(base_s, len(es) + len(rest)),
             'nba': gru_prog + chunks(base_n, len(en)) + chunks(base_s + len(es), len(rest))}
    out = {'kte': kte, 'pool': np.ascontiguousarray(np.stack([np.asarray(t, np.float32) for t in tiles]))}
    C = R32_CONSTS
    for v in ('scenes', 'nba'):
        c = np.zeros(C['total'], np.float64)
        c[C['bc']:C['bc'] + 64], c[C['wlast']:C['wlast'] + 64] = F['bc'], F['wlast']
        c[C['bi']:C['bi'] + 64], c[C['bg']:C['bg'] + 64] = F['bi_' + v], F['bg_' + v]
        c[C['ln1w']:C['ln1w'] + 64], c[C['ln1b']:C['ln1b'] + 64] = f64(att + 'norm1.weight'), f64(att + 'norm1.bias')
        c[C['l1b']:C['l1b'] + 1024], c[C['l2b']:C['l2b'] + 64] = f64(att + 'linear1.bias'), f64(att + 'linear2.bias')
        c[C['ln2w']:C['ln2w'] + 64], c[C['ln2b']:C['ln2b'] + 64] = f64(att + 'norm2.weight'), f64(att + 'norm2.bias')
        c[C['gbias']:C['gbias'] + 416] = gs['consts']
        for nm, blk, key in (('x', 0, 'b1x'), ('y', 0, 'b1y'), ('y', 1, 'b11')):
            c[C[key]:C[key] + 512] = f64(f'decoder.decompose.{blk}.decoder_{nm}.layers.0.bias')
        out['consts_' + v] = np.ascontiguousarray(c.astype(np.float32))
        out['prog_' + v] = np.ascontiguousarray(np.asarray(progs[v], np.int32))
        out['prog_len_' + v] = len(progs[v])
        assert len(progs[v]) == role_prog_len(Tp, v == 'nba')
# ... 55 lines not shown
```

Before: 86.81 million.

## Add lean GRU weight program with LDS-resident conv blocks and trimmed step-0 tiles

Adds a 'lean' packed weight program for the GRU section of the chain, gru32 and role kernels. The nonzero conv Toeplitz fragments are packed into a compact block that is copied into LDS once per workgroup, so the conv tiles no longer go through the streamed ring. Step 0 is trimmed to only the input-gate tiles, since the hidden state starts at zero. It also swaps relu to an integer max form and adjusts stream prefetch begin counts. The cost is extra LDS per block and a new kernel variant, enabled by default when the conv block is small and the mode is fp32.

```diff
diff --git a/include/sttode_hip.h b/include/sttode_hip.h
--- a/include/sttode_hip.h
+++ b/include/sttode_hip.h
@@ -366,6 +366,7 @@
 int sttode_workspace_layout(const SttodeModel* m, int n, int S, long* offsets , long* total_floats);
 int sttode_workspace_init(SttodeModel* m, float* workspace, int n, int S, void* stream);
 int sttode_set_chain(SttodeModel* m, int mode);
+int sttode_set_chain_program(SttodeModel* m, int lean);
 int sttode_set_fused(SttodeModel* m, int mode);
 int sttode_set_mfma_mode(SttodeModel* m, int mode);
 int sttode_debug_drop_role_flag(SttodeModel* m, int tile);
diff --git a/sttode_amd/capi.py b/sttode_amd/capi.py
--- a/sttode_amd/capi.py
+++ b/sttode_amd/capi.py
@@ -128,6 +128,7 @@
     'sttode_timeout_word': [_P, ctypes.POINTER(ctypes.c_void_p)],
     'sttode_timeout_clear': [_P],
     'sttode_set_chain': [_P, _I],
+    'sttode_set_chain_program': [_P, _I],
     'sttode_set_fused': [_P, _I],
     'sttode_set_mfma_mode': [_P, _I],
     'sttode_debug_drop_role_flag': [_P, _I],
@@ -166,6 +167,13 @@
     'sttode_check': [_P, _P, _I, _I, _P],
 }
 
+OPTIONAL = {'sttode_set_chain_program'}
+
+
+def has_lean_program():
+    return hasattr(lib(), 'sttode_set_chain_program')
+
+
 RESTYPES = {'sttode_sampler_objective_joint_ws': ctypes.c_longlong, 'sttode_large_select_ws': ctypes.c_longlong,
             'sttode_large_spread_ws': ctypes.c_longlong}
 
@@ -214,7 +222,7 @@
 
 class NativeModel:
 
-    def __init__(self, packed, Tp, Tf, K):
+    def __init__(self, packed, Tp, Tf, K, lean=False):
         self.packed = packed
         tbl = (ctypes.c_void_p * len(WEIGHT_ORDER))(*[(packed[g][k].data_ptr() if g in packed else None) for g, k in WEIGHT_ORDER])
         h = ctypes.c_void_p()
@@ -224,6 +232,9 @@
             raise SttodeError('sttode_model_create failed: ' + lib().sttode_last_error().decode())
         self.h = h
         self._layouts = {}
+        self.lean = bool(lean)
+        if lean:
+            call('sttode_set_chain_program', h, 1)
         w = ctypes.c_void_p()
         if lib().sttode_timeout_word(h, ctypes.byref(w)) != 0 or not w.value:
             raise SttodeError('sttode_timeout_word failed: ' + lib().sttode_last_error().decode())
@@ -326,6 +337,8 @@
         if got != ABI_VERSION:
             raise SttodeError(f'{LIB_PATH}: ABI version {got}, this binding needs {ABI_VERSION}; rebuild with `make -C sttode_amd/csrc`')
         for name, args in SIGNATURES.items():
+            if name in OPTIONAL and not hasattr(L, name):
+                continue
             fn = getattr(L, name)
             fn.argtypes = args
             fn.restype = RESTYPES.get(name, ctypes.c_int)
diff --git a/sttode_amd/csrc/api_util.hpp b/sttode_amd/csrc/api_util.hpp
--- a/sttode_amd/csrc/api_util.hpp
+++ b/sttode_amd/csrc/api_util.hpp
@@ -70,6 +70,8 @@
 };
 int stt_chain_lagged(const float* const* W, const LagRoles& r, const LagGroups& g, int K, int Tp, int Tf, int prog_len, int b3, void* stream);
 bool stt_chain_lagged_covers(int Tp);
+inline int stt_lean_gru_len(int Tp) { return 3 + 12 * (Tp - 1); }
+bool stt_chain_lean_available();
 struct SttodeSamplerPlan;
 const char* stt_sampler_plan_check(const SttodeSamplerPlan* plan, int K);
 int stt_sampler_qnet(const SttodeSamplerPlan* plan, const float* pf, int n, float* z, void* stream);
diff --git a/sttode_amd/csrc/chain32.hip b/sttode_amd/csrc/chain32.hip
--- a/sttode_amd/csrc/chain32.hip
+++ b/sttode_amd/csrc/chain32.hip
@@ -88,9 +88,13 @@
     for (int e = 0; e < 16; ++e) r[e] = v;
     return r;
 }
+template <bool ONE = false>
 __device__ __forceinline__ f32x16 relu16(f32x16 v) {
 #pragma unroll
-    for (int e = 0; e < 16; ++e) v[e] = fmaxf(v[e], 0.f);
+    for (int e = 0; e < 16; ++e) {
+        if (ONE) { const int b = __float_as_int(v[e]); v[e] = __int_as_float(b > 0 ? b : 0); }
+        else v[e] = fmaxf(v[e], 0.f);
+    }
     return v;
 }
 __device__ __forceinline__ f32x16 ldrows(const float* p, int h) {
@@ -268,7 +272,7 @@
     }
 }
 
-template <int KH, class ST>
+template <int KH, bool R1 = false, class ST>
 __device__ __forceinline__ void mlp_l12(ST& st, const f32x4* slot, const f32x4* zslot, const f32x16* Bh, const float* tab, unsigned aoff,
                                         const float* tab_next, unsigned aoff_next, f32x16 (&acc2)[8], int lane) {
     const unsigned slot_addr = __builtin_amdgcn_readfirstlane(lds_addr(slot));
@@ -315,7 +319,7 @@
                 if (i % 3 == 0) tile_mma2f(st, h1, fr[i & 1], Bh[i - 1], fr[(i + 1) & 1], tn);
                 else tile_mma2(h1, fr[i & 1], Bh[i - 1], fr[(i + 1) & 1], tn);
             } else {
-                if (i == KT1) h1 = relu16(h1);
+                if (i == KT1) h1 = relu16<R1>(h1);
                 if (i % 3 == 0) tile_mma2f(st, acc2[i - KT1], fr[i & 1], h1, fr[(i + 1) & 1], tn);
                 else tile_mma2(acc2[i - KT1], fr[i & 1], h1, fr[(i + 1) & 1], tn);
             }
@@ -324,14 +328,14 @@
     }
 }
 
-template <int NO, int NEXT = 0, class ST>
+template <int NO, int NEXT = 0, bool R1 = false, class ST>
 __device__ __forceinline__ void mlp_l3(ST& st, f32x16 (&acc2)[8], const float* __restrict__ b2, const float* __restrict__ b3,
                                        f32x16 (&out)[NO], int h) {
 #pragma unroll
     for (int R = 0; R < 8; ++R) {
         STT_FENCE();
         const f32x16 b = ldrows(b2 + 32 * R, h);
-        acc2[R] = relu16(acc2[R] + b);
+        acc2[R] = relu16<R1>(acc2[R] + b);
         asm volatile("" : "+v"(acc2[R]));
     }
     STT_FENCE();
@@ -592,10 +596,36 @@
     }
 }
 
-template <bool ZS, class ST>
-__device__ __forceinline__ f32x16 gru32_conv(ST& st, const float* cb, const f32x16& d, int t, int Tp, int h, bool pre) {
+__host__ __device__ __forceinline__ int conv_groups_of(int t, int Tp) {
+    const int k0 = 2 * t - 2, k1 = 2 * t + 3;
+    return ((k1 < 2 * Tp - 1 ? k1 : 2 * Tp - 1) >> 3) - ((k0 > 0 ? k0 : 0) >> 3) + 1;
+}
+__host__ __device__ __forceinline__ int conv_block_groups(int t, int Tp) {
+    int n = 0;
+    for (int s = 0; s < t; ++s) n += conv_groups_of(s, Tp);
+    return n;
+}
+template <bool ZS, bool LEAN = false, class ST>
+__device__ __forceinline__ f32x16 gru32_conv(ST& st, const float* cb, const f32x16& d, int t, int Tp, int h, bool pre,
+                                             const f32x4* cblk = nullptr, int* cpos = nullptr) {
     f32x16 e = ldrows(cb, h);
     Frag fa, fb;
+    if (LEAN) {
+        static_assert(!LEAN || ZS, "the lean program has no tiles for the zero products");
+        const int k0 = 2 * t - 2, k1 = 2 * t + 3;
+        const int g0 = (k0 > 0 ? k0 : 0) >> 3, g1 = (k1 < 2 * Tp - 1 ? k1 : 2 * Tp - 1) >> 3;
+        const f32x4* tc = cblk + (*cpos - g0) * 64;
+#pragma unroll
+        for (int g = 0; g < 4; ++g)
+            if (g >= g0 && g <= g1) fa.a[g] = tc[g * 64];
+#pragma unroll
+        for (int g = 0; g < 4; ++g)
+            if (g >= g0 && g <= g1)
+#pragma unroll
+                for (int r = 0; r < 4; ++r) e = __builtin_amdgcn_mfma_f32_32x32x2f32(fa.a[g][r], d[4 * g + r], e, 0, 0, 0);
+        *cpos += g1 - g0 + 1;
+        return relu16<true>(e);
+    }
     if (ZS) {
         const int k0 = 2 * t - 2, k1 = 2 * t + 3;
         const int g0 = (k0 > 0 ? k0 : 0) >> 3, g1 = (k1 < 2 * Tp - 1 ? k1 : 2 * Tp - 1) >> 3;
@@ -623,9 +653,44 @@
     return e;
 }
 
-template <bool ZS, class ST>
-__device__ __forceinline__ void gru32_steps(ST& st, const float* gb, const float* cb, const f32x16& d, f32x16 (&hs)[3], int Tp, int h) {
-    if (ZS) {
+template <bool ZS, bool LEAN = false, class ST>
+__device__ __forceinline__ void gru32_steps(ST& st, const float* gb, const float* cb, const f32x16& d, f32x16 (&hs)[3], int Tp, int h,
+                                            const f32x4* cblk = nullptr) {
+    int cpos = 0;
+    if (LEAN) {
+        const f32x16 e = gru32_conv<ZS, LEAN>(st, cb, d, 0, Tp, h, false, cblk, &cpos);
+        Frag fa, fb;
+#pragma unroll
+        for (int j = 0; j < 3; ++j) {
+            STT_FENCE();
+            f32x16 ar = ldrows(gb + 0 * 96 + 32 * j, h);
+            ldfrag(fa, st.cur());
+            if (j < 2 || 1 < Tp) st.begin(3); else st.begin();
+            tile_mma2f(st, ar, fa, e, fb, st.cur() + 1 * C32_TILE);
+#pragma unroll
+            for (int r = 0; r < 16; ++r) ar[r] = C32_SIG(ar[r]);
+            STT_FENCE();
+            f32x16 az = ldrows(gb + 1 * 96 + 32 * j, h);
+            tile_mma2(az, fb, e, fa, st.cur() + 2 * C32_TILE);
+#pragma unroll
+            for (int r = 0; r < 16; ++r) az[r] = C32_SIG(az[r]);
+            STT_FENCE();
+            f32x16 an = ldrows(gb + 3 * 96 + 32 * j, h);
+            {
+                const f32x16 bi = ldrows(gb + 2 * 96 + 32 * j, h);
+#pragma unroll
+                for (int r = 0; r < 16; ++r) an[r] = fmaf(ar[r], an[r], bi[r]);
+            }
+            STT_FENCE();
+            tile_mma2(an, fa, e, fb, nullptr);
+            st.end();
+#pragma unroll
+            for (int r = 0; r < 16; ++r) {
+                const float ng = C32_TANH(an[r]);
+                hs[j][r] = fmaf(az[r], 0.f - ng, ng);
+            }
+        }
+    } else if (ZS) {
         const f32x16 e = gru32_conv<ZS>(st, cb, d, 0, Tp, h, false);
         Frag fa, fb;
 #pragma unroll
@@ -665,7 +730,7 @@
     }
 #pragma unroll 1
     for (int t = ZS ? 1 : 0; t < Tp; ++t) {
-        const f32x16 e = gru32_conv<ZS>(st, cb, d, t, Tp, h, ZS);
+        const f32x16 e = gru32_conv<ZS, LEAN>(st, cb, d, t, Tp, h, ZS, cblk, &cpos);
         Frag fa, fb;
         f32x16 hn[3];
 #pragma unroll
@@ -693,8 +758,8 @@
             f32x16 an = ldrows(gb + 3 * 96 + 32 * j, h);
             tile_mma2(an, fa, hs[0], fb, nullptr);
             st.end(); ldfrag(fa, st.cur());
-            if (j < 2) st.begin(3); else st.begin();
-            tile_mma2f(st, an, fa, hs[1], fb, st.cur() + 1 * C32_TILE, (ZS && j == 2 && t + 1 < Tp) ? 2 : 1);
+            if (j < 2 || (LEAN && t + 1 < Tp)) st.begin(3); else st.begin();
+            tile_mma2f(st, an, fa, hs[1], fb, st.cur() + 1 * C32_TILE, (ZS && !LEAN && j == 2 && t + 1 < Tp) ? 2 : 1);
             tile_mma2(an, fb, hs[2], fa, st.cur() + 2 * C32_TILE);
             {
                 const f32x16 bi = ldrows(gb + 2 * 96 + 32 * j, h);
@@ -733,9 +798,10 @@
     return x * q + (x < r ? x : r) + i;
 }
 
-template <int NY, int FUSE, bool B3M, bool ZS>
-__global__ __launch_bounds__(256, 2) void traj_chain_kernel(ChainArgs A) {
-    constexpr bool kDynCount = !B3M && ((NY == 1 && FUSE == 2 && !ZS) || (NY == 2 && FUSE == 1 && ZS));
+template <int NY, int FUSE, bool B3M, bool ZS, bool LEAN>
+__device__ __forceinline__ void traj_chain_body(const ChainArgs& A) {
+    static_assert(!LEAN || (ZS && !B3M), "the lean program: fp32 tiles, zero products skipped");
+    constexpr bool kDynCount = !B3M && !LEAN && ((NY == 1 && FUSE == 2 && !ZS) || (NY == 2 && FUSE == 1 && ZS));
     typedef ChainStreamT<B3M ? C32_BUF_B3 : C32_CMAX * C32_TILE, B3M, kDynCount> Stream;
     extern __shared__ __attribute__((aligned(16))) char smem[];
     f32x4* ring = reinterpret_cast<f32x4*>(smem);
@@ -743,6 +809,7 @@
     f32x4* zslots = slots + 4 * C32_SLOT;
     float* cst = reinterpret_cast<float*>(zslots + 4 * C32_SLOT);
     int* sq = reinterpret_cast<int*>(cst + C32Const<NY>::total);
+    f32x4* cblk = reinterpret_cast<f32x4*>(sq + 4);
     typedef C32Const<NY> CO;
 
     const int lane = threadIdx.x & 63, c = lane & 31, h = lane >> 5;
@@ -755,7 +822,7 @@
 
     C32_TRACE_BEGIN();
     if (FUSE == 2 && (int)blockIdx.x < A.R32.nwg) {
-        role32_body<ZS>(*(KRole32Args*)((const __attribute__((address_space(4))) char*)__builtin_amdgcn_kernarg_segment_ptr() + offsetof(ChainArgs, R32)),
+        role32_body<ZS, LEAN>(*(KRole32Args*)((const __attribute__((address_space(4))) char*)__builtin_amdgcn_kernarg_segment_ptr() + offsetof(ChainArgs, R32)),
                     blockIdx.x, smem);
         C32_TRACE_END(1);
         return;
@@ -768,6 +835,10 @@
         return;
     }
     for (int i = threadIdx.x; i < CO::total; i += blockDim.x) cst[i] = A.consts[i];
+    if (LEAN) {
+        const int ncb = conv_block_groups(A.Tp, A.Tp) * 64;
+        for (int i = threadIdx.x; i < ncb; i += blockDim.x) cblk[i] = A.pool[i];
+    }
     if (threadIdx.x == 0) sq[0] = FUSE == 2 ? fb : (FUSE == 0 && A.persistent) ? atomicAdd(A.counter, 1) : FUSE ? fb : (int)blockIdx.x;
     if (FUSE == 1) {
         const int g0 = fb;
@@ -824,8 +895,8 @@
                 mlp_l12_b3<0, true>(st, slot, zslot, nullptr, A.A0x, ao, A.A0y, ao, acc2, lane);
                 mlp_l3_b3<1>(st, acc2, cst + CO::b2x, cst + CO::b3x, xo, h);
             } else {
-                mlp_l12<0>(st, slot, zslot, nullptr, A.A0x, ao, A.A0y, ao, acc2, lane);
-                mlp_l3<1, 3>(st, acc2, cst + CO::b2x, cst + CO::b3x, xo, h);
+                mlp_l12<0, LEAN>(st, slot, zslot, nullptr, A.A0x, ao, A.A0y, ao, acc2, lane);
+                mlp_l3<1, 3, LEAN>(st, acc2, cst + CO::b2x, cst + CO::b3x, xo, h);
             }
             agent = opaque(agent);
             const float* xp = A.xpad + (size_t)agent * A.ldx;
@@ -847,8 +918,8 @@
                 mlp_l12_b3<0, true>(st, slot, zslot, nullptr, A.A0y, ao, A.A1y, ao, acc2, lane);
                 mlp_l3_b3<NY>(st, acc2, cst + CO::b2y, cst + CO::b3y, yo, h);
             } else {
-                mlp_l12<0>(st, slot, zslot, nullptr, A.A0y, ao, A.A1y, ao, acc2, lane);
-                mlp_l3<NY, 1>(st, acc2, cst + CO::b2y, cst + CO::b3y, yo, h);
+                mlp_l12<0, LEAN>(st, slot, zslot, nullptr, A.A0y, ao, A.A1y, ao, acc2, lane);
+                mlp_l3<NY, LEAN ? 3 : 1, LEAN>(st, acc2, cst + CO::b2y, cst + CO::b3y, yo, h);
             }
             if (live) {
                 float* prow = A.park + (size_t)opaque(col) * A.Tf2;
@@ -876,7 +947,7 @@
 #pragma unroll
             for (int j = 0; j < 3; ++j) hs[j] = splat16(0.f);
             if (B3M) gru32_steps_b3(st, cst + CO::gb, cst + CO::cb, d, hs, A.Tp, h);
-            else gru32_steps<ZS>(st, cst + CO::gb, cst + CO::cb, d, hs, A.Tp, h);
+            else gru32_steps<ZS, LEAN>(st, cst + CO::gb, cst + CO::cb, d, hs, A.Tp, h, cblk + lane);
         }
         STT_FENCE();
         C32_STAMP(3);
@@ -886,11 +957,11 @@
             const int cnx = col_of(gnext < ngroups ? gnext : g);
             const unsigned ao = row_off(agent, 512, h), an = row_off(cnx / A.K, 512, h);
             if (B3M) mlp_l12_b3<3, false>(st, slot, zslot, hs, A.A1y, ao, A.A0x, an, acc2, lane);
-            else mlp_l12<3>(st, slot, zslot, hs, A.A1y, ao, A.A0x, an, acc2, lane);
+            else mlp_l12<3, LEAN>(st, slot, zslot, hs, A.A1y, ao, A.A0x, an, acc2, lane);
             gather_rows(A.z, row_off(opaque(cnx), 32, h), zslot_addr);
             f32x16 yo[NY];
             if (B3M) mlp_l3_b3<NY>(st, acc2, cst + CO::b2m, cst + CO::b3m, yo, h);
-            else mlp_l3<NY, 3>(st, acc2, cst + CO::b2m, cst + CO::b3m, yo, h);
+            else mlp_l3<NY, 3, LEAN>(st, acc2, cst + CO::b2m, cst + CO::b3m, yo, h);
             {
                 agent = opaque(agent);
                 const float cx = A.cur[2 * agent], cy = A.cur[2 * agent + 1];
@@ -971,6 +1042,10 @@
     }
     C32_TRACE_END(0);
 }
+template <int NY, int FUSE, bool B3M, bool ZS>
+__global__ __launch_bounds__(256, 2) void traj_chain_kernel(ChainArgs A) { traj_chain_body<NY, FUSE, B3M, ZS, false>(A); }
+template <int NY, int FUSE>
+__global__ __launch_bounds__(256, 2) void traj_chain_lean_kernel(ChainArgs A) { traj_chain_body<NY, FUSE, false, true, true>(A); }
 
 struct Gru32Args {
     const float* xin; int ldx;
@@ -979,14 +1054,19 @@
     float* state;
     int ncols, Tp;
 };
-template <bool ZS>
+template <bool ZS, bool LEAN = false>
 __global__ __launch_bounds__(256, 2) void gru32_kernel(Gru32Args A) {
     extern __shared__ __attribute__((aligned(16))) char smem[];
     f32x4* ring = reinterpret_cast<f32x4*>(smem);
     float* cst = reinterpret_cast<float*>(ring + C32_RING);
+    f32x4* cblk = reinterpret_cast<f32x4*>(cst + 416);
     const int lane = threadIdx.x & 63, c = lane & 31, h = lane >> 5;
     const int wave = __builtin_amdgcn_readfirstlane(threadIdx.x >> 6);
     for (int i = threadIdx.x; i < 416; i += blockDim.x) cst[i] = A.consts[i];
+    if (LEAN) {
+        const int ncb = conv_block_groups(A.Tp, A.Tp) * 64;
+        for (int i = threadIdx.x; i < ncb; i += blockDim.x) cblk[i] = A.pool[i];
+    }
     __syncthreads();
     ChainStream st;
     st.init(A.pool, A.prog, A.prog_len, ring);
@@ -1008,7 +1088,7 @@
     f32x16 hs[3];
 #pragma unroll
     for (int j = 0; j < 3; ++j) hs[j] = splat16(0.f);
-    gru32_steps<ZS>(st, cst, cst + 384, d, hs, A.Tp, h);
+    gru32_steps<ZS, LEAN>(st, cst, cst + 384, d, hs, A.Tp, h, cblk + lane);
     if (col < A.ncols) {
 #pragma unroll
         for (int j = 0; j < 3; ++j)
@@ -1034,6 +1114,8 @@
     static const int v = getenv("STTODE_GRU_ZERO_SKIP") ? atoi(getenv("STTODE_GRU_ZERO_SKIP")) != 0 : 1;
     return v;
 }
+bool stt_chain_lean_available() { return gru_zero_skip() != 0; }
+static int conv_block_bytes(int Tp) { return conv_block_groups(Tp, Tp) * 1024; }
 static int chain_lds(int NY, bool b3 = false) { return ((b3 ? 2 * C32_BUF_B3 : C32_RING) + 8 * C32_SLOT) * 16 + (1216 + 64 * NY) * 4 + 16; }
 
 static int role_lds(int Tp) {
@@ -1043,9 +1125,17 @@
 
 static int role32_lds() { return C32_RING * 16 + R32C::total * 4; }
 
-template <int NY, int FUSE, bool B3M = false> static int chain_launch(ChainArgs a, int wgs_per_cu, hipStream_t s) {
-    void (*kern)(ChainArgs) = gru_zero_skip() ? traj_chain_kernel<NY, FUSE, B3M, true> : traj_chain_kernel<NY, FUSE, B3M, false>;
-    STT_SET_LDS_ONCE(kern, 96 * 1024);
+template <int NY, int FUSE, bool B3M = false> static int chain_launch(ChainArgs a, int wgs_per_cu, hipStream_t s, bool lean = false) {
+    STT_REQUIRE(!lean || (!B3M && gru_zero_skip()), "sttode_traj_chain: a lean program needs the fp32 stream with the zero products skipped");
+    if (!B3M && lean) {
+        STT_SET_LDS_ONCE((traj_chain_lean_kernel<NY, FUSE>), 96 * 1024);
+    } else if (gru_zero_skip()) {
+        STT_SET_LDS_ONCE((traj_chain_kernel<NY, FUSE, B3M, true>), 96 * 1024);
+    } else {
+        STT_SET_LDS_ONCE((traj_chain_kernel<NY, FUSE, B3M, false>), 96 * 1024);
+    }
+    void (*kern)(ChainArgs) = (!B3M && lean) ? traj_chain_lean_kernel<NY, FUSE>
+                              : gru_zero_skip() ? traj_chain_kernel<NY, FUSE, B3M, true> : traj_chain_kernel<NY, FUSE, B3M, false>;
     const int ngroups = (a.ncols + 127) / 128;
     int grid = ngroups;
     if (FUSE == 1) grid = a.R.ntiles + ngroups;
@@ -1056,9 +1146,10 @@
         a.nworkers = workers;
         if (workers < ngroups) a.xcd_map = 0;
     }
-    int lds = chain_lds(NY, B3M);
+    const int cbb = lean ? conv_block_bytes(a.Tp) : 0;
+    int lds = chain_lds(NY, B3M) + cbb;
     if (FUSE == 1 && lds < role_lds(a.Tp)) lds = role_lds(a.Tp);
-    if (FUSE == 2 && a.R32.nwg > 0 && lds < role32_lds()) lds = role32_lds();
+    if (FUSE == 2 && a.R32.nwg > 0 && lds < role32_lds() + cbb) lds = role32_lds() + cbb;
     if (wgs_per_cu == 1 && lds < 84 * 1024) lds = 84 * 1024;
     STT_REQUIRE(lds <= 96 * 1024, "sttode_traj_chain: dynamic LDS beyond the 96 KiB the kernel is registered for");
     STT_REQUIRE((long)a.ncols * 128 <= 0xffffffffL && (long)((a.ncols + a.K - 1) / a.K) * 2048 <= 0xffffffffL,
@@ -1073,12 +1164,16 @@
                                  float* state, int ncols, int Tp, void* stream) {
     STT_REQUIRE(xin && pool && prog && consts && state, "sttode_gru_cols32: null pointer");
     STT_REQUIRE(ncols > 0 && Tp >= 1 && (ldx == 16 || ldx == 32) && 2 * Tp <= ldx, "sttode_gru_cols32: bad ncols/Tp/ldx");
-    STT_REQUIRE(prog_len == 13 * Tp, "sttode_gru_cols32: chunk program must hold 13 entries per step");
+    const bool lean = prog_len == stt_lean_gru_len(Tp);
+    STT_REQUIRE(prog_len == 13 * Tp || lean, "sttode_gru_cols32: chunk program must hold 13 entries per step (lean: 3 + 12 (Tp - 1))");
+    STT_REQUIRE(!lean || gru_zero_skip(), "sttode_gru_cols32: a lean program needs the zero products skipped");
     Gru32Args a;
     a.xin = xin; a.ldx = ldx; a.pool = (const f32x4*)pool; a.prog = (const int2*)prog; a.prog_len = prog_len; a.consts = consts;
     a.state = state; a.ncols = ncols; a.Tp = Tp;
-    const int lds = C32_RING * 16 + 416 * 4;
-    hipLaunchKernelGGL(gru_zero_skip() ? gru32_kernel<true> : gru32_kernel<false>, dim3((ncols + 127) / 128), dim3(256), lds, (hipStream_t)stream, a);
+    const int lds = C32_RING * 16 + 416 * 4 + (lean ? conv_block_bytes(Tp) : 0);
+    void (*kern)(Gru32Args) = gru_zero_skip() ? gru32_kernel<true> : gru32_kernel<false>;
+    if (lean) kern = gru32_kernel<true, true>;
+    hipLaunchKernelGGL(kern, dim3((ncols + 127) / 128), dim3(256), lds, (hipStream_t)stream, a);
     STT_HIP(hipGetLastError());
     return 0;
 }
@@ -1150,6 +1245,7 @@
     const int l3y = (8 * NY + 2) / 3;
     return (48 + 3) + (48 + l3y) + 13 * Tp + (64 + l3y);
 }
+static int chain_prog_len_lean(int Tp, int Tf) { return sttode_chain_prog_len(Tp, Tf) - 13 * Tp + stt_lean_gru_len(Tp); }
 
 static int traj_chain_impl(const float* A0x, const float* A0y, const float* A1y, const float* pool, const int* prog, int prog_len,
                            const float* consts, const float* z, const float* xpad, int ldx, const float* cur, const float* orig,
@@ -1159,7 +1255,8 @@
     STT_REQUIRE(ldx == 16 || ldx == 32, "sttode_traj_chain: ldx must be 16 or 32");
     STT_REQUIRE(wgs_per_cu == 1 || wgs_per_cu == 2, "sttode_traj_chain: wgs_per_cu must be 1 or 2");
     STT_REQUIRE(2 * Tp <= ldx, "sttode_traj_chain: xpad rows shorter than 2*Tp");
-    STT_REQUIRE(prog_len == sttode_chain_prog_len(Tp, Tf), "sttode_traj_chain: chunk program length does not match (Tp, Tf)");
+    const bool lean = !b3 && prog_len == chain_prog_len_lean(Tp, Tf);
+    STT_REQUIRE(prog_len == sttode_chain_prog_len(Tp, Tf) || lean, "sttode_traj_chain: chunk program length does not match (Tp, Tf)");
     ChainArgs a;
     a.A0x = A0x; a.A0y = A0y; a.A1y = A1y; a.pool = (const f32x4*)pool; a.prog = (const int2*)prog; a.prog_len = prog_len;
     a.consts = consts; a.z = z; a.xpad = xpad; a.ldx = ldx; a.cur = cur; a.orig = orig; a.pred = pred; a.park = pred; a.counter = counter;
@@ -1182,9 +1279,9 @@
         }
     }
     switch (NY) {
-        case 1: return chain_launch<1, 0>(a, wgs_per_cu, s);
-        case 2: return chain_launch<2, 0>(a, wgs_per_cu, s);
-        case 3: return chain_launch<3, 0>(a, wgs_per_cu, s);
+        case 1: return chain_launch<1, 0>(a, wgs_per_cu, s, lean);
+        case 2: return chain_launch<2, 0>(a, wgs_per_cu, s, lean);
+        case 3: return chain_launch<3, 0>(a, wgs_per_cu, s, lean);
         default: STT_REQUIRE(false, "sttode_traj_chain: future length beyond the built instantiations (2*Tf <= 96)");
     }
     return 0;
@@ -1206,7 +1303,8 @@
     STT_REQUIRE(W && ws && off && z && pred, "stt_chain_fused: null pointer");
     STT_REQUIRE(n > 0 && K > 0 && stt_chain_fused_covers(Tp) && Tf >= 1, "stt_chain_fused: shape outside the fused launch");
     STT_REQUIRE(!attn || (ld_attn >= 64 && ld_attn % 4 == 0), "stt_chain_fused: bad attention leading dimension");
-    STT_REQUIRE(prog_len == sttode_chain_prog_len(Tp, Tf), "stt_chain_fused: chunk program length does not match (Tp, Tf)");
+    const bool lean = !b3 && prog_len == chain_prog_len_lean(Tp, Tf);
+    STT_REQUIRE(prog_len == sttode_chain_prog_len(Tp, Tf) || lean, "stt_chain_fused: chunk program length does not match (Tp, Tf)");
     STT_REQUIRE((long)n * K <= 0x7fffffffL, "stt_chain_fused: too many trajectories");
     ChainArgs a;
     a.A0x = ws + off[STT_B_A0X]; a.A0y = ws + off[STT_B_A0Y]; a.A1y = ws + off[STT_B_A1Y];
@@ -1231,9 +1329,9 @@
     const int NY = (2 * Tf + 31) / 32;
     hipStream_t s = (hipStream_t)stream;
     switch (NY) {
-        case 1: return b3 ? chain_launch<1, 1, true>(a, wgs_per_cu, s) : chain_launch<1, 1>(a, wgs_per_cu, s);
-        case 2: return b3 ? chain_launch<2, 1, true>(a, wgs_per_cu, s) : chain_launch<2, 1>(a, wgs_per_cu, s);
-        case 3: return b3 ? chain_launch<3, 1, true>(a, wgs_per_cu, s) : chain_launch<3, 1>(a, wgs_per_cu, s);
+        case 1: return b3 ? chain_launch<1, 1, true>(a, wgs_per_cu, s) : chain_launch<1, 1>(a, wgs_per_cu, s, lean);
+        case 2: return b3 ? chain_launch<2, 1, true>(a, wgs_per_cu, s) : chain_launch<2, 1>(a, wgs_per_cu, s, lean);
+        case 3: return b3 ? chain_launch<3, 1, true>(a, wgs_per_cu, s) : chain_launch<3, 1>(a, wgs_per_cu, s, lean);
         default: STT_REQUIRE(false, "stt_chain_fused: future length beyond the built instantiations (2*Tf <= 96)");
     }
     return 0;
@@ -1248,6 +1346,8 @@
     const float* g_gt = lg.gt; float* g_ade = lg.ade; float* g_fde = lg.fde; const float g_scale = lg.scale; const int lag_workers_ok = lg.workers;
     STT_REQUIRE(W && (ws_r || ws_g), "stt_chain_lagged: nothing to launch");
     STT_REQUIRE(K > 0 && stt_chain_lagged_covers(Tp) && Tf >= 1, "stt_chain_lagged: shape outside the lagged launch");
+    const bool lean = !b3 && prog_len == chain_prog_len_lean(Tp, Tf);
+    STT_REQUIRE(prog_len == sttode_chain_prog_len(Tp, Tf) || lean, "stt_chain_lagged: chunk program length does not match (Tp, Tf)");
     ChainArgs a;
     a.R = RoleArgs();
     a.R32 = Role32Args();
@@ -1263,7 +1363,6 @@
     }
     if (ws_g) {
         STT_REQUIRE(off_g && z && pred && n_g > 0 && (long)n_g * K <= 0x7fffffffL, "stt_chain_lagged: bad group arguments");
-        STT_REQUIRE(prog_len == sttode_chain_prog_len(Tp, Tf), "stt_chain_lagged: chunk program length does not match (Tp, Tf)");
         a.A0x = ws_g + off_g[STT_B_A0X]; a.A0y = ws_g + off_g[STT_B_A0Y]; a.A1y = ws_g + off_g[STT_B_A1Y];
         a.z = z; a.xpad = ws_g + off_g[STT_B_XPAD]; a.cur = ws_g + off_g[STT_B_CUR]; a.orig = ws_g + off_g[STT_B_ORIG]; a.pred = pred;
         a.park = ws_g + off_g[STT_B_YBUF];
@@ -1281,7 +1380,8 @@
         r.consts = W[attn ? STT_W_ROLE32_CONSTS_NBA : STT_W_ROLE32_CONSTS_SCENES];
         r.kte = (4 * Tp + 31) / 32;
         const int e = attn ? 8 : 2 * r.kte + 8;
-        r.prog_len = attn ? 13 * Tp + (e + 2) / 3 + (128 + 288 + 2) / 3 : 13 * Tp + (e + 128 + 288 + 2) / 3;
+        const int gl = lean ? stt_lean_gru_len(Tp) : 13 * Tp;
+        r.prog_len = attn ? gl + (e + 2) / 3 + (128 + 288 + 2) / 3 : gl + (e + 128 + 288 + 2) / 3;
         r.enc_in = ws_r + off_r[STT_B_ENC_IN]; r.last = (const int*)(ws_r + off_r[STT_B_LAST]);
         r.g_in = ws_r + off_r[STT_B_G]; r.attn = attn; r.ld_attn = ld_attn;
         r.xpad = ws_r + off_r[STT_B_XPAD]; r.ldx = a.ldx;
@@ -1305,9 +1405,9 @@
     const int NY = (2 * Tf + 31) / 32;
     hipStream_t s = (hipStream_t)stream;
     switch (NY) {
-        case 1: return b3 ? chain_launch<1, 2, true>(a, 2, s) : chain_launch<1, 2>(a, 2, s);
-        case 2: return b3 ? chain_launch<2, 2, true>(a, 2, s) : chain_launch<2, 2>(a, 2, s);
-        case 3: return b3 ? chain_launch<3, 2, true>(a, 2, s) : chain_launch<3, 2>(a, 2, s);
+        case 1: return b3 ? chain_launch<1, 2, true>(a, 2, s) : chain_launch<1, 2>(a, 2, s, lean);
+        case 2: return b3 ? chain_launch<2, 2, true>(a, 2, s) : chain_launch<2, 2>(a, 2, s, lean);
+        case 3: return b3 ? chain_launch<3, 2, true>(a, 2, s) : chain_launch<3, 2>(a, 2, s, lean);
         default: STT_REQUIRE(false, "stt_chain_lagged: future length beyond the built instantiations (2*Tf <= 96)");
     }
     return 0;
diff --git a/sttode_amd/csrc/pipeline.hip b/sttode_amd/csrc/pipeline.hip
--- a/sttode_amd/csrc/pipeline.hip
+++ b/sttode_amd/csrc/pipeline.hip
@@ -30,6 +30,7 @@
     int b3;
     int ode_method, ode_steps;
     int prog_len;
+    int lean;
     hipStream_t sA, sB, sB2;
     std::mutex mu;
     unsigned* tmo_host;
@@ -111,6 +112,7 @@
     if (const char* e = getenv("STTODE_LAGGED")) m->lag_streams = atoi(e) >= 2 && atoi(e) <= 4 ? atoi(e) : 0;
     m->scene_launch = 128;
     m->prog_len = sttode_chain_prog_len(Tp, Tf);
+    m->lean = 0;
     m->side = nullptr;
     bool ok = hipEventCreateWithFlags(&m->ev_fork, hipEventDisableTiming) == hipSuccess &&
               hipEventCreateWithFlags(&m->ev_join, hipEventDisableTiming) == hipSuccess;
@@ -205,6 +207,17 @@
     return 0;
 }
 
+extern "C" int sttode_set_chain_program(SttodeModel* m, int lean) {
+    STT_REQUIRE(m, "sttode_set_chain_program: null model");
+    STT_REQUIRE(lean == 0 || lean == 1, "sttode_set_chain_program: lean must be 0 or 1");
+    STT_REQUIRE(!lean || !m->b3, "sttode_set_chain_program: the bf16-split mode runs beside the full programs only");
+    STT_REQUIRE(!lean || stt_chain_lean_available(),"sttode_set_chain_program: the lean program needs the zero products skipped (STTODE_GRU_ZERO_SKIP)");
+    std::lock_guard<std::mutex> lk(m->mu);
+    m->lean = lean;
+    m->prog_len = sttode_chain_prog_len(m->Tp, m->Tf) - (lean ? 13 * m->Tp - stt_lean_gru_len(m->Tp) : 0);
+    return 0;
+}
+
 extern "C" int sttode_set_fused(SttodeModel* m, int mode) {
     STT_REQUIRE(m, "sttode_set_fused: null model");
     STT_REQUIRE(mode == 0 || mode == 1, "sttode_set_fused: mode must be 0 or 1 (modes 2-4 were retired)");
@@ -241,6 +254,7 @@
     STT_REQUIRE(mode == 0 || mode == 1, "sttode_set_mfma_mode: mode must be 0 (fp32) or 1 (three-way bf16 split, exploratory)");
     STT_REQUIRE(mode == 0 || (m->w[STT_W_CHAINB3_POOL] && m->w[STT_W_CHAINB3_PROG]),
                 "sttode_set_mfma_mode: the bf16-split weight stream has not been handed over (sttode_model_set_weight)");
+    STT_REQUIRE(mode == 0 || !m->lean, "sttode_set_mfma_mode: the bf16-split mode runs beside the full programs only (sttode_set_chain_program)");
     m->b3 = mode;
     return 0;
 }
@@ -364,7 +378,8 @@
     }
     if (TPX == 2) {
         RUN(STT_STAGE_GRU0, gs,
-            sttode_gru_cols32(xpad, 16 * TPX, W[STT_W_G0_POOL], (const int*)W[STT_W_G0_PROG], 13 * Tp, W[STT_W_G0_CONSTS], state0, n, Tp, gs));
+            sttode_gru_cols32(xpad, 16 * TPX, W[STT_W_G0_POOL], (const int*)W[STT_W_G0_PROG], m->lean ? stt_lean_gru_len(Tp) : 13 * Tp,
+                              W[STT_W_G0_CONSTS], state0, n, Tp, gs));
     } else
         RUN(STT_STAGE_GRU0, gs,
             stt_gru_cols_form(xpad, W[STT_W_B0_CONVP], W[STT_W_B0_CONVB], W[STT_W_B0_WIHP], W[STT_W_B0_WHHP], W[STT_W_B0_GBIAS], state0, n,
diff --git a/sttode_amd/csrc/role32.hpp b/sttode_amd/csrc/role32.hpp
--- a/sttode_amd/csrc/role32.hpp
+++ b/sttode_amd/csrc/role32.hpp
@@ -124,10 +124,11 @@
     }
 }
 
-template <bool ZS>
+template <bool ZS, bool LEAN = false>
 __device__ __forceinline__ void role32_body(KRole32Args& R, int wg, char* smem) {
     f32x4* ring = reinterpret_cast<f32x4*>(smem);
     float* cst = reinterpret_cast<float*>(ring + C32_RING);
+    f32x4* cblk = reinterpret_cast<f32x4*>(cst + R32C::total);
     const int lane = threadIdx.x & 63, c = lane & 31, h = lane >> 5;
     const int wave = __builtin_amdgcn_readfirstlane(threadIdx.x >> 6);
     if (R.prio > 0) __builtin_amdgcn_s_setprio(3);
@@ -144,6 +145,10 @@
         __builtin_amdgcn_fence(__ATOMIC_ACQUIRE, "workgroup");
     }
     for (int i = threadIdx.x; i < R32C::total; i += blockDim.x) cst[i] = R.consts[i];
+    if (LEAN) {
+        const int ncb = conv_block_groups(R.Tp, R.Tp) * 64;
+        for (int i = threadIdx.x; i < ncb; i += blockDim.x) cblk[i] = R.pool[i];
+    }
     __syncthreads();
     ChainStream st;
     st.init(R.pool, R.prog, R.prog_len, ring);
@@ -168,7 +173,7 @@
     f32x16 hs[3];
 #pragma unroll
     for (int j = 0; j < 3; ++j) hs[j] = splat16(0.f);
-    gru32_steps<ZS>(st, cst + R32C::gb, cst + R32C::cb, d, hs, Tp, h);
+    gru32_steps<ZS, LEAN>(st, cst + R32C::gb, cst + R32C::cb, d, hs, Tp, h, cblk + lane);
     if (live) {
 #pragma unroll
         for (int j = 0; j < 3; ++j) strows(R.state0 + (size_t)col * 96 + 32 * j, hs[j], h);
@@ -227,7 +232,7 @@
             f32x16 hid = ldrows(cst + R32C::l1b + 32 * ht, h);
             fd.mma(hid, XR[0]);
             fd.mma(hid, XR[1]);
-            hid = relu16(hid);
+            hid = relu16<LEAN>(hid);
             fd.mma(FF[0], hid);
             fd.mma(FF[1], hid);
         }
@@ -242,7 +247,7 @@
 #pragma unroll
     for (int j = 0; j < 2; ++j) {
         B7[j] = G[j];
-        B7[2 + j] = relu16(G[j] + XR[j] * R.ode_time);
+        B7[2 + j] = relu16<LEAN>(G[j] + XR[j] * R.ode_time);
     }
 #pragma unroll
     for (int j = 0; j < 3; ++j) B7[4 + j] = hs[j];
diff --git a/sttode_amd/model.py b/sttode_amd/model.py
--- a/sttode_amd/model.py
+++ b/sttode_amd/model.py
@@ -235,18 +235,22 @@
                 torch.cuda.synchronize(self.device)
             sd = {k: v.detach().cpu().numpy() for k, v in self.state_dict().items()}
             a = self.args
+            lean = (self.device.type == 'cuda' and self.mfma_mode != 'bf16x3' and capi.has_lean_program()
+                    and packing.lean_program_wanted(a.past_length))
+            chain_stream, gru32_stream, role_stream = ((packing.chain_stream_lean, packing.gru32_stream_lean, packing.role_stream_lean) if lean
+                                                       else (packing.chain_stream, packing.gru32_stream, packing.role_stream))
             host = {'past': packing.pack_trunk(sd, 'past_encoder.', a.past_length),
                     'blk0': packing.pack_block(sd, 0, a.past_length, a.future_length, first=True),
                     'blk1': packing.pack_block(sd, 1, a.past_length, a.future_length, first=False),
                     'future': packing.pack_trunk(sd, 'future_encoder.', a.future_length),
                     'post': packing.pack_posterior(sd),
-                    'chain': packing.chain_stream(sd, a.past_length, a.future_length),
-                    'gru0s': packing.gru32_stream(sd, 0, a.past_length),
-                    'role32': packing.role_stream(sd, a.past_length)}
+                    'chain': chain_stream(sd, a.past_length, a.future_length),
+                    'gru0s': gru32_stream(sd, 0, a.past_length),
+                    'role32': role_stream(sd, a.past_length)}
             self._packed = {g: {k: (torch.from_numpy(np.ascontiguousarray(v)).to(self.device) if isinstance(v, np.ndarray) else v)
                                 for k, v in d.items()} for g, d in host.items()}
             self._packed_key = key
-            self._native = capi.NativeModel(self._packed, a.past_length, a.future_length, a.sample_k) if self.device.type == 'cuda' else None
+            self._native = capi.NativeModel(self._packed, a.past_length, a.future_length, a.sample_k, lean=lean) if self.device.type == 'cuda' else None
             self._wscache = {}
             self._async_bufs = {}
         return self._packed
@@ -264,6 +268,9 @@
             raise capi.SttodeError('the native pipeline (fused launches, packed weight streams) is built for the reference widths hidden_dim 64, '
                                    'zdim 32, num_decompose 2, 2 Tp <= 32, 2 Tf <= 96; this model runs the generic form (sttode_amd/generic.py)')
         if check_weights or self._packed is None or self._native is None:
+            self.packed()
+        if self._native is not None and self.mfma_mode == 'bf16x3' and self._native.lean:
+            self._packed = None
             self.packed()
         ode = (self.ODE_METHODS[self.ode_method], int(self.ode_steps))
         if self._native is not None and getattr(self._native, '_ode', (0, 1)) != ode:
diff --git a/sttode_amd/packing.py b/sttode_amd/packing.py
--- a/sttode_amd/packing.py
+++ b/sttode_amd/packing.py
@@ -340,6 +340,92 @@
             'consts': np.ascontiguousarray(consts), 'prog_len': len(prog)}
 
 
+def conv_groups(t, Tp):
+    return max(2 * t - 2, 0) >> 3, min(2 * t + 3, 2 * Tp - 1) >> 3
+
+
+def conv_block_offset(t, Tp):
+    return sum(g1 - g0 + 1 for g0, g1 in (conv_groups(s, Tp) for s in range(t)))
+
+
+def conv_block_tiles(Tp):
+    return (conv_block_offset(Tp, Tp) + 3) // 4
+
+
+def lean_gru_len(Tp):
+    return 3 + 12 * (Tp - 1)
+
+
+def chain_prog_len_lean(Tp, Tf):
+    return chain_prog_len(Tp, Tf) - 13 * Tp + lean_gru_len(Tp)
+
+
+def role_prog_len_lean(Tp, nba):
+    return role_prog_len(Tp, nba) - 13 * Tp + lean_gru_len(Tp)
+
+
+def _lean(pool, progs, p0, gru_base, conv_base, Tp):
+    blk = [pool[conv_base + t].reshape(4, 256)[g] for t in range(Tp) for g in range(conv_groups(t, Tp)[0], conv_groups(t, Tp)[1] + 1)]
+    nct = conv_block_tiles(Tp)
+    head = np.zeros((nct, 1024), np.float32)
+    head.reshape(-1)[: 256 * len(blk)] = np.concatenate(blk)
+    step0 = np.stack([pool[gru_base + 12 * j + o] for j in range(3) for o in (0, 4, 11)])
+    shift = nct + 9
+    out = []
+    for prog in progs:
+        prog = [(int(a), int(b)) for a, b in prog]
+        assert all(e == (conv_base + t, 1) for t, e in zip(range(Tp), prog[p0:p0 + 13 * Tp:13]))
+        lean = [(a + shift, b) for a, b in prog[:p0]] + [(nct + 3 * j, 3) for j in range(3)]
+        for t in range(1, Tp):
+            lean += [(a + shift, b) for a, b in prog[p0 + 13 * t + 1: p0 + 13 * t + 13]]
+        lean += [(a + shift, b) for a, b in prog[p0 + 13 * Tp:]]
+        out.append(np.ascontiguousarray(np.asarray(lean, np.int32)))
+    return np.ascontiguousarray(np.concatenate([head, step0, pool])), out
+
+
+def chain_stream_lean(sd, Tp, Tf):
+    f = chain_stream(sd, Tp, Tf)
+    p0 = chain_prog_len(Tp, Tf) - 13 * Tp - (64 + (8 * tiles_y32(Tf) + 2) // 3)
+    gru_base = int(f['prog'][p0 + 1][0])
+    pool, (prog,) = _lean(f['pool'], [f['prog']], p0, gru_base, gru_base + 36, Tp)
+    assert len(prog) == chain_prog_len_lean(Tp, Tf)
+    return {'pool': pool, 'prog': prog, 'consts': f['consts'], 'prog_len': len(prog)}
+
+
+def gru32_stream_lean(sd, block, Tp):
+    f = gru32_stream(sd, block, Tp)
+    pool, (prog,) = _lean(f['pool'], [f['prog']], 0, 0, 36, Tp)
+    assert len(prog) == lean_gru_len(Tp)
+    return {'pool': pool, 'prog': prog, 'consts': f['consts'], 'prog_len': len(prog)}
+
+
+def role_stream_lean(sd, Tp):
+    f = role_stream(sd, Tp)
+    pool, (ps, pn) = _lean(f['pool'], [f['prog_scenes'], f['prog_nba']], 0, 0, 36, Tp)
+    out = dict(f, pool=pool, prog_scenes=ps, prog_nba=pn, prog_len_scenes=len(ps), prog_len_nba=len(pn))
+    assert len(ps) == role_prog_len_lean(Tp, False) and len(pn) == role_prog_len_lean(Tp, True)
+    return out
+
+
+LEAN_MAX_CONV_KIB = 16
+
+
+def lean_program_wanted(Tp, env=None):
+    import os
+    env = os.environ if env is None else env
+    zs = env.get('STTODE_GRU_ZERO_SKIP')
+    if zs is not None:
+        try:
+            if int(zs.strip() or 0) == 0:
+                return False
+        except ValueError:
+            return False
+    how = env.get('STTODE_CHAIN_PROGRAM', '')
+    if how == 'full':
+        return False
+    return how == 'lean' or conv_block_offset(Tp, Tp) <= LEAN_MAX_CONV_KIB
+
+
 R32_CONSTS = dict(bc=0, wlast=64, bi=128, bg=192, ln1w=256, ln1b=320, l1b=384, l2b=1408, ln2w=1472, ln2b=1536, gbias=1600, convb=1984,
                   b1x=2016, b1y=2528, b11=3040, total=3552)
 
```

Result: no change. 87.31 million, median of 6 (+0.6%).
